# shiv-vignesh/T5-Resnet-VQA

Measured on AMD Instinct MI355X. Metric: question-image pairs/sec, ResNet50+T5-base+SGA train step, 1/2/4/8 MI355X, higher is better.
Workload: dtype bf16; 1 GPU; ResNet50 + t5-base + 3xSGA train step (BASELINE configs[1]; configs[2] at N=8); model=resnet50+t5-base+3xSGA, global_batch=64, per_gpu_batch=64, seq_len=32, image_size=224, answers=170, parallelism=dp1, world_size=1, graph=True, resnet_pipelined=True

## Files before the change

include/vqa_hip.h:

```cpp
#ifndef VQA_HIP_H
#define VQA_HIP_H

#include <hip/hip_runtime.h>

#ifdef __cplusplus
extern "C" {
#endif

#define VQA_ABI_VERSION 20
#define VQA_OK 0
#define VQA_ERR_INVALID 1000

int vqa_abi_version(void);
const char* vqa_last_error(void);

typedef struct vqa_dropout {
  float p;
  unsigned site;
  const unsigned* rng;
} vqa_dropout;

int vqa_rng_advance(unsigned* rng, hipStream_t stream);
int vqa_dropout_mask(const vqa_dropout* d, float* out, long long n, hipStream_t stream);

typedef struct vqa_conv_geom {
  int n, h, w, c;
  int oh, ow;
  int kh, kw, stride, pad;
} vqa_conv_geom;

typedef struct vqa_gemm_desc {
  const void* a; long long lda; int a_trans;
  const void* b; long long ldb; int b_trans;
  int m, n, k;
  float* c32; long long ldc32;
  void* c16; long long ldc16;
  const float* bias;
  const float* res32; const void* res16; long long ldres;
  const void* mask16; long long ldmask;
  float alpha, beta; int relu;
  int a_conv; vqa_conv_geom ga;
  int b_conv; vqa_conv_geom gb;
  int batch; long long stride_a, stride_b, stride_c32, stride_c16, stride_res;
  int config;
  vqa_dropout drop;
  int splitk;
  void* workspace;
  long long workspace_bytes;
  long long stride_bias;
  int drop_site_stride;
  int fp8;
  const float* scale_a;
  const float* scale_b;
  long long stride_scale_a, stride_scale_b;
  int norm;
  const float* norm_w;
  const float* norm_b;
  float norm_eps;
  float* norm_y32;
  void* norm_y16;
  float* norm_mean;
  float* norm_rstd;
  long long stride_norm_w, stride_norm_y, stride_norm_stat;
  vqa_dropout norm_drop;
} vqa_gemm_desc;

#define VQA_GEMM_CONFIGS 28
#define VQA_GEMM_PATCH_FIRST 17
#define VQA_GEMM_PATCH_LAST 20
#define VQA_GEMM_PATCH_WIDE 25
int vqa_gemm(const vqa_gemm_desc* d, hipStream_t stream);
int vqa_quant_rows_fp8(const void* x, int x_bf16, long long ldx, int rows, int cols, void* q, long long ldq,
                       float* scale, hipStream_t stream);
int vqa_gemm_select(const vqa_gemm_desc* d);
long long vqa_gemm_workspace_bytes(const vqa_gemm_desc* d);
int vqa_gemm_pair(const vqa_gemm_desc* dx, const vqa_gemm_desc* dw, hipStream_t stream);

typedef struct vqa_attn_desc {
  const void* q; long long ldq;
  const void* k; long long ldk;
  const void* v; long long ldv;
  void* o; long long ldo;
  float* p;
  const float* bias;
  const long long* key_mask;
  int batch, heads, lq, lk, dh;
  float scale;
  const void* dout; long long lddo;
  void* dq; long long lddq;
  void* dk; long long lddk;
  void* dv; long long lddv;
  float* dbias;
  vqa_dropout drop;
  int groups;
  long long gstride_qkv, gstride_o, gstride_p, gstride_dout;
  int gdrop_site_stride;
} vqa_attn_desc;

int vqa_attn_fwd(const vqa_attn_desc* d, hipStream_t stream);
int vqa_attn_bwd(const vqa_attn_desc* d, hipStream_t stream);
#define VQA_ATTN_MFMA 0
#define VQA_ATTN_LONG 1
#define VQA_ATTN_VALU 2
int vqa_attn_path(const vqa_attn_desc* d, int backward);
int vqa_attn_probs(const vqa_attn_desc* d, hipStream_t stream);

int vqa_rmsnorm_fwd(const float* x, const float* w, float* y32, void* y16, float* rstd, int rows, int d, float eps,
                    const vqa_dropout* drop, hipStream_t stream);
int vqa_rmsnorm_bwd(const float* dy, const float* x, const float* rstd, const float* w, const float* dres,
                    float* dx32, void* dx16, float* dw, float dw_beta, float* ws, int rows, int d,
                    const vqa_dropout* drop_dy, const vqa_dropout* drop_dx32, const vqa_dropout* drop_dx16,
                    hipStream_t stream);
int vqa_layernorm_fwd(const float* x, const float* gamma, const float* beta, float* y32, void* y16, float* mean,
                      float* rstd, int rows, int d, float eps, hipStream_t stream);
int vqa_layernorm_bwd(const float* dy, const float* x, const float* mean, const float* rstd, const float* gamma,
                      const float* dres, float* dx32, void* dx16, float* dgamma, float* dbeta, float* ws, int rows,
                      int d, const vqa_dropout* drop_dx16, float* dsum, hipStream_t stream);
int vqa_norm_bwd_workspace_floats(int rows, int d);
int vqa_colsum_partials(const float* ws, int parts, long long stride, int cols, float* out, float beta,
                        hipStream_t stream);
typedef struct vqa_colsum_job {
  const float* ws; float* out; long long stride; int parts; int cols; float beta; int first_block;
} vqa_colsum_job;
int vqa_norm_bwd_parts(int rows);
int vqa_colsum_parts(int rows);
int vqa_colsum_batched(const vqa_colsum_job* jobs, int njobs, int nblocks, hipStream_t stream);

int vqa_image_to_nhwc8(const float* img, void* out, int n, int h, int w, hipStream_t stream);
int vqa_image_to_s2d16(const float* img, void* out, int n, int h, int w, hipStream_t stream);
int vqa_maxpool3x3s2_nhwc(const void* x, void* y, int n, int h, int w, int c, int oh, int ow, hipStream_t stream);
int vqa_subsample_nhwc(const void* x, int n, int h, int w, int c, int stride, void* y, long long ldy,
                       hipStream_t stream);
int vqa_stem_s2d_conv(const void* z, const void* w, const float* bias, void* y, int n, int hz, int oh,
                      hipStream_t stream);
int vqa_stem_pool_s2d(const void* z, const void* w, const float* bias, void* y, int n, int hz, int oh,
                      hipStream_t stream);
int vqa_stem_pool_img(const float* img, const void* w, const float* bias, void* y, int n, int h, hipStream_t stream);
int vqa_colsum(const void* x, int x_bf16, int rows, int cols, long long ld, float* out, float beta, float* ws,
               hipStream_t stream);
int vqa_colsum_workspace_floats(int rows, int cols);
int vqa_embedding_fwd(const long long* ids, const float* table, float* out, int tokens, int d, int vocab,
                      const vqa_dropout* drop, hipStream_t stream);
typedef struct {
  long long offset;
  int h, w;
} vqa_image_desc;
int vqa_resize_linear_u8(const void* src, const vqa_image_desc* desc, int batch, int oh, int ow, float* out,
                         hipStream_t stream);
int vqa_embedding_bwd(const long long* ids, const float* dh, float* dtable, int tokens, int d, int vocab, int* ws,
                      hipStream_t stream);
int vqa_embedding_zero_rows(long long* ids_prev, const long long* ids_cur, int tokens, float* dtable, int d,
                            int vocab, hipStream_t stream);
int vqa_t5_relbias_fwd(const float* table, const int* bucket, float* out, int heads, int lq, int lk,
                       hipStream_t stream);
int vqa_t5_relbias_bwd(const float* dbias, const int* bucket, float* dtable, int heads, int lq, int lk,
                       int nbuckets, hipStream_t stream);
int vqa_batch_sum(const float* x, int batch, long long n, float* out, float beta, hipStream_t stream);
int vqa_cast_f32_bf16(const float* x, void* y, long long n, hipStream_t stream);
int vqa_zero(void* p, long long bytes, hipStream_t stream);
int vqa_copy(void* dst, const void* src, long long bytes, hipStream_t stream);
int vqa_tap_shift(const void* in, void* out, int n, int h, int w, int c, int kh, int kw, int pad,
                  hipStream_t stream);

int vqa_vit_patchify(const float* img, void* out, int n, int h, int w, int patch, hipStream_t stream);
int vqa_gather_rows(const void* src, long long lds, const long long* idx, long long stride, long long offset,
                    void* dst, long long ldd, int rows, int cols, int esz, hipStream_t stream);
int vqa_scatter_rows(const void* src, long long lds, const long long* idx, long long stride, long long offset,
                     void* dst, long long ldd, int rows, int cols, int esz, hipStream_t stream);
int vqa_last_index(const long long* mask, int batch, int len, long long* out, hipStream_t stream);
int vqa_xattn1_fwd(const void* v, long long ldv, void* out, long long ldo, int batch, int len, int heads, int dh,
                   const vqa_dropout* drop, hipStream_t stream);
int vqa_xattn1_bwd(const void* dctx, long long ldd, float* dv32, void* dv16, long long lddv, int batch, int len,
                   int heads, int dh, const vqa_dropout* drop, hipStream_t stream);

int vqa_head_fwd(const float* x, const float* wp, const float* bp, const float* wc, const float* bc,
                 const long long* targets, float* att, float* pooled, float* logp, float* nll, float* loss,
                 int batch, int seq, int d, int answers, hipStream_t stream);
int vqa_head_bwd(const float* x, const float* att, const float* pooled, const float* logp, const long long* targets,
                 const float* wp, const float* wc, float* dx32, void* dx16, float* dwp, float* dbp, float* dwc,
                 float* dbc, float* ws, int batch, int seq, int d, int answers, const float* nll, float* loss,
                 const float* row_total, float row_scale, hipStream_t stream);
int vqa_head_workspace_floats(int batch, int seq, int d, int answers);
int vqa_count_targets(const long long* targets, int batch, float* out, hipStream_t stream);

typedef struct vqa_eval_desc {
  const float* logp;
  const long long* targets;
  const float* nll;
  const float* loss;
  const float* similarity;
  int batch, answers, k;
  int* topk_idx;
  float* topk_logp;
  void* acc;
  int* pred_log; int* tgt_log;
  long long capacity;
} vqa_eval_desc;

int vqa_eval_rows(const vqa_eval_desc* d, hipStream_t stream);

#define VQA_MAX_GROUPS 8
#define VQA_ST_STEP 0
#define VQA_ST_GRAD_NORM 1
#define VQA_ST_CLIP_COEF 2
#define VQA_ST_LR_SCALE 3
#define VQA_ST_BC1 4
#define VQA_ST_BC2_SQRT 5
#define VQA_ST_PENDING 8

typedef struct vqa_adamw_desc {
  float* param; const float* grad;
  float* exp_avg; float* exp_avg_sq; float* max_exp_avg_sq;
  void* param16;
  long long n;
  int ngroups;
  long long group_end[VQA_MAX_GROUPS];
  float group_lr[VQA_MAX_GROUPS];
  float beta1, beta2, eps, weight_decay, grad_scale;
  const float* state;
} vqa_adamw_desc;

int vqa_grad_sqnorm(const float* g, long long n, double* ws, int parts, hipStream_t stream);
int vqa_optim_finalize(const double* ws, int parts, float grad_scale, float max_norm, int warmup, int total,
                       float beta1, float beta2, float* state, hipStream_t stream);
int vqa_adamw_amsgrad(const vqa_adamw_desc* d, hipStream_t stream);
int vqa_embed_mark(const long long* ids, int n, int rows, int* mark, const float* state, hipStream_t stream);
int vqa_adamw_rows(const vqa_adamw_desc* d, const int* mark, int rows, int cols, int touched, int warmup, int total,
                   hipStream_t stream);

#ifdef __cplusplus
}
#endif
#endif
```

t5-resnet-vqa_amd/csrc/elementwise.hip:

```cpp
#include "common.h"

namespace {

__global__ __launch_bounds__(256) void image_to_nhwc8_kernel(const float* __restrict__ img, bf16_t* __restrict__ out,
                                                             int n, int hw) {
  const long i = (long)blockIdx.x * 256 + threadIdx.x;
  if (i >= (long)n * hw) return;
  const long b = i / hw, p = i - b * hw;
  const float* src = img + b * 3 * hw + p;
  uint4 u;
  u.x = (uint32_t)f2bf(src[0]) | ((uint32_t)f2bf(src[hw]) << 16);
  u.y = (uint32_t)f2bf(src[2 * hw]);
  u.z = 0; u.w = 0;
  reinterpret_cast<uint4*>(out)[i] = u;
}

__global__ __launch_bounds__(256) void image_to_s2d16_kernel(const float* __restrict__ img, bf16_t* __restrict__ out,
                                                             int n, int h, int w, int hz, int wz) {
  const long i = (long)blockIdx.x * 256 + threadIdx.x;
  if (i >= (long)n * hz * wz) return;
  const int v = (int)(i % wz);
  const long t = i / wz;
  const int u = (int)(t % hz), b = (int)(t / hz);
  const float* src = img + (long)b * 3 * h * w;
  float z[16];
#pragma unroll
  for (int p = 0; p < 2; ++p)
#pragma unroll
    for (int q = 0; q < 2; ++q) {
      const int y = 2 * u + p - 1, x = 2 * v + q - 1;
      const bool ok = y >= 0 && y < h && x >= 0 && x < w;
      const long o = ok ? (long)y * w + x : 0;
#pragma unroll
      for (int c = 0; c < 3; ++c) z[(2 * p + q) * 3 + c] = ok ? src[(long)c * h * w + o] : 0.f;
    }
#pragma unroll
  for (int c = 12; c < 16; ++c) z[c] = 0.f;
  uint4 lo, hi;
  lo.x = (uint32_t)f2bf(z[0]) | ((uint32_t)f2bf(z[1]) << 16);
  lo.y = (uint32_t)f2bf(z[2]) | ((uint32_t)f2bf(z[3]) << 16);
  lo.z = (uint32_t)f2bf(z[4]) | ((uint32_t)f2bf(z[5]) << 16);
  lo.w = (uint32_t)f2bf(z[6]) | ((uint32_t)f2bf(z[7]) << 16);
  hi.x = (uint32_t)f2bf(z[8]) | ((uint32_t)f2bf(z[9]) << 16);
  hi.y = (uint32_t)f2bf(z[10]) | ((uint32_t)f2bf(z[11]) << 16);
  hi.z = 0; hi.w = 0;
  reinterpret_cast<uint4*>(out)[2 * i] = lo;
  reinterpret_cast<uint4*>(out)[2 * i + 1] = hi;
}

__global__ __launch_bounds__(256) void maxpool3s2_kernel(const bf16_t* __restrict__ x, bf16_t* __restrict__ y, int n,
                                                         int h, int w, int c, int oh, int ow) {
  const int c8 = c / 8;
  const long i = (long)blockIdx.x * 256 + threadIdx.x;
  if (i >= (long)n * oh * ow * c8) return;
  const int cc = (int)(i % c8);
  long t = i / c8;
  const int ox = (int)(t % ow); t /= ow;
  const int oy = (int)(t % oh);
  const int b = (int)(t / oh);
  float m[8];
#pragma unroll
  for (int j = 0; j < 8; ++j) m[j] = -INFINITY;
  for (int dy = 0; dy < 3; ++dy) {
    const int iy = oy * 2 - 1 + dy;
    if (iy < 0 || iy >= h) continue;
    for (int dx = 0; dx < 3; ++dx) {
      const int ix = ox * 2 - 1 + dx;
      if (ix < 0 || ix >= w) continue;
      uint4 u = reinterpret_cast<const uint4*>(x + (((long)b * h + iy) * w + ix) * c)[cc];
      const uint32_t wds[4] = {u.x, u.y, u.z, u.w};
#pragma unroll
      for (int j = 0; j < 4; ++j) {
        m[2 * j] = fmaxf(m[2 * j], bf2f((bf16_t)(wds[j] & 0xffff)));
        m[2 * j + 1] = fmaxf(m[2 * j + 1], bf2f((bf16_t)(wds[j] >> 16)));
      }
    }
  }
  uint4 o;
  o.x = (uint32_t)f2bf(m[0]) | ((uint32_t)f2bf(m[1]) << 16);
  o.y = (uint32_t)f2bf(m[2]) | ((uint32_t)f2bf(m[3]) << 16);
  o.z = (uint32_t)f2bf(m[4]) | ((uint32_t)f2bf(m[5]) << 16);
  o.w = (uint32_t)f2bf(m[6]) | ((uint32_t)f2bf(m[7]) << 16);
  reinterpret_cast<uint4*>(y)[i] = o;
}

constexpr int COLSUM_ROWS = 64;
template <bool BF16>
__global__ __launch_bounds__(256) void colsum_part_kernel(const void* __restrict__ xv, int rows, int cols, long ld,
                                                          float* __restrict__ ws) {
  const int tx = threadIdx.x & 63, ty = threadIdx.x >> 6;
  const int c = blockIdx.x * 256 + tx * 4;
  const int r0 = blockIdx.y * COLSUM_ROWS;
  float s[4] = {0.f, 0.f, 0.f, 0.f};
  constexpr int RPT = COLSUM_ROWS / 4;
  const int cl = min(c, cols - 4);
  float4 v[RPT];
#pragma unroll
  for (int q = 0; q < RPT; ++q) {
    const int r = min(r0 + ty + 4 * q, rows - 1);
    if constexpr (BF16) {
      const uint2 u = *reinterpret_cast<const uint2*>((const bf16_t*)xv + (long)r * ld + cl);
      v[q] = make_float4(bf2f(u.x & 0xffff), bf2f(u.x >> 16), bf2f(u.y & 0xffff), bf2f(u.y >> 16));
    } else {
      v[q] = *reinterpret_cast<const float4*>((const float*)xv + (long)r * ld + cl);
    }
  }
#pragma unroll
  for (int q = 0; q < RPT; ++q) {
    const float m = (c < cols && r0 + ty + 4 * q < rows) ? 1.f : 0.f;
    s[0] += v[q].x * m; s[1] += v[q].y * m; s[2] += v[q].z * m; s[3] += v[q].w * m;
  }
  __shared__ float red[4][256];
#pragma unroll
  for (int j = 0; j < 4; ++j) red[ty][tx * 4 + j] = s[j];
  __syncthreads();
  const int cc = blockIdx.x * 256 + threadIdx.x;
  if (cc < cols)
    ws[(long)blockIdx.y * cols + cc] = red[0][threadIdx.x] + red[1][threadIdx.x] + red[2][threadIdx.x] +
                                       red[3][threadIdx.x];
}

__global__ __launch_bounds__(256) void embedding_fwd_kernel(const long long* __restrict__ ids,
                                                            const float* __restrict__ table, float* __restrict__ out,
                                                            int tokens, int d4, int vocab, vqa_dropout drop) {
  const long i = (long)blockIdx.x * 256 + threadIdx.x;
  if (i >= (long)tokens * d4) return;
  const int t = (int)(i / d4), j = (int)(i - (long)t * d4);
  long long id = ids[t];
  id = id < 0 ? 0 : (id >= vocab ? vocab - 1 : id);
  float4 v = reinterpret_cast<const float4*>(table + id * (long)d4 * 4)[j];
  const DropK dk = drop_init(drop);
  if (dk.on) {
    const uint32_t e = (uint32_t)i * 4u;
    v.x *= drop_mul(dk, e); v.y *= drop_mul(dk, e + 1); v.z *= drop_mul(dk, e + 2); v.w *= drop_mul(dk, e + 3);
  }
  reinterpret_cast<float4*>(out)[i] = v;
}

__global__ void rng_advance_kernel(unsigned* rng) { rng[1] += 1u; }

__global__ __launch_bounds__(256) void dropout_mask_kernel(vqa_dropout d, float* __restrict__ out, long n) {
  const long i = (long)blockIdx.x * 256 + threadIdx.x;
  if (i >= n) return;
  const DropK dk = drop_init(d);
  out[i] = drop_mul(dk, (uint32_t)i);
}

__global__ __launch_bounds__(256) void embedding_zero_rows_kernel(long long* __restrict__ prev,
                                                                  const long long* __restrict__ cur,
                                                                  float* __restrict__ dtable, int d, int vocab) {
  const int t = blockIdx.x;
  long long id = prev[t];
  id = id < 0 ? 0 : (id >= vocab ? vocab - 1 : id);
  float4* row = reinterpret_cast<float4*>(dtable + id * (long long)d);
  for (int c = threadIdx.x; c < d / 4; c += 256) row[c] = make_float4(0.f, 0.f, 0.f, 0.f);
  __syncthreads();
  if (cur && threadIdx.x == 0) prev[t] = cur[t];
}

__device__ __forceinline__ unsigned long long shfl_xor64(unsigned long long v, int m) {
  const int lo = __shfl_xor((int)(unsigned)(v & 0xffffffffu), m, 64);
  const int hi = __shfl_xor((int)(unsigned)(v >> 32), m, 64);
  return ((unsigned long long)(unsigned)hi << 32) | (unsigned)lo;
}
template <int E>
__global__ __launch_bounds__(1024) void embedding_sort_kernel(const long long* __restrict__ ids, int tokens, int vocab,
                                                              int* __restrict__ ws) {
  __shared__ unsigned long long key[E * 1024];
  constexpr int n = E * 1024;
  const int t = threadIdx.x;
  unsigned long long v[E];
#pragma unroll
  for (int q = 0; q < E; ++q) {
    const int i = q * 1024 + t;
    long long id = ids[min(i, tokens - 1)];
    id = id < 0 ? 0 : (id >= vocab ? vocab - 1 : id);
    v[q] = i < tokens ? (((unsigned long long)id << 16) | (unsigned long long)i) : ~0ull;
  }
  for (int k = 2; k <= n; k <<= 1) {
    for (int j = k >> 1; j > 0; j >>= 1) {
      if (j >= 1024) {
        const int qj = j >> 10;
#pragma unroll
        for (int q = 0; q < E; ++q) {
          if (q & qj) continue;
          const int i = q * 1024 + t;
          const bool up = (i & k) == 0;
          const unsigned long long a = v[q], c = v[q | qj];
          v[q] = up ? (a < c ? a : c) : (a < c ? c : a);
          v[q | qj] = up ? (a < c ? c : a) : (a < c ? a : c);
        }
      } else if (j >= 64) {
#pragma unroll
        for (int q = 0; q < E; ++q) key[q * 1024 + t] = v[q];
        __syncthreads();
#pragma unroll
        for (int q = 0; q < E; ++q) {
          const int i = q * 1024 + t;
          const unsigned long long c = key[i ^ j];
          const bool keep_min = ((i & j) == 0) == ((i & k) == 0);
          v[q] = keep_min ? (v[q] < c ? v[q] : c) : (v[q] < c ? c : v[q]);
        }
        __syncthreads();
      } else {
#pragma unroll
        for (int q = 0; q < E; ++q) {
          const int i = q * 1024 + t;
          const unsigned long long c = shfl_xor64(v[q], j);
          const bool keep_min = ((i & j) == 0) == ((i & k) == 0);
          v[q] = keep_min ? (v[q] < c ? v[q] : c) : (v[q] < c ? c : v[q]);
        }
      }
    }
  }
#pragma unroll
  for (int q = 0; q < E; ++q) key[q * 1024 + t] = v[q];
  __syncthreads();
#pragma unroll
  for (int q = 0; q < E; ++q) {
    const int i = q * 1024 + t;
    if (i >= tokens) continue;
    const unsigned long long kt = v[q];
    const unsigned id = (unsigned)(kt >> 16);
    ws[i] = (int)(kt & 0xffff);
    ws[tokens + i] = (int)id;
    if (i == 0 || (unsigned)(key[i - 1] >> 16) != id) {
      int lo = i + 1, hi = tokens;
      while (lo < hi) {
        const int mid = (lo + hi) >> 1;
        if ((unsigned)(key[mid] >> 16) == id) lo = mid + 1; else hi = mid;
      }
      ws[2 * tokens + i] = lo;
    }
  }
}

constexpr int EMB_RL = 16, EMB_CL = 32;
__global__ __launch_bounds__(EMB_RL * EMB_CL) void embedding_bwd_kernel(const float* __restrict__ dh,
                                                                        float* __restrict__ dtable,
                                                                        const int* __restrict__ ws, int tokens,
                                                                        int d) {
  const int s0 = blockIdx.x;
  const int* pos = ws;
  const int* sid = ws + tokens;
  const int id = sid[s0];
  if (s0 > 0 && sid[s0 - 1] == id) return;
  const int s1 = ws[2 * tokens + s0];
  const int tx = threadIdx.x % EMB_CL, ty = threadIdx.x / EMB_CL;
  const int c4 = blockIdx.y * EMB_CL + tx;
  const bool act = c4 * 4 < d;
  float4 acc = make_float4(0.f, 0.f, 0.f, 0.f);
  if (act) {
    constexpr int U = 8;
    for (int u0 = s0 + ty; u0 < s1; u0 += EMB_RL * U) {
      int pp[U];
#pragma unroll
      for (int q = 0; q < U; ++q) pp[q] = pos[min(u0 + q * EMB_RL, s1 - 1)];
      float4 v[U];
#pragma unroll
      for (int q = 0; q < U; ++q) v[q] = reinterpret_cast<const float4*>(dh + (long)pp[q] * d)[c4];
#pragma unroll
      for (int q = 0; q < U; ++q) {
        if (u0 + q * EMB_RL < s1) { acc.x += v[q].x; acc.y += v[q].y; acc.z += v[q].z; acc.w += v[q].w; }
      }
    }
  }
  __shared__ float4 red[EMB_RL][EMB_CL];
  red[ty][tx] = acc;
  __syncthreads();
  if (ty == 0 && act) {
    float4 t = red[0][tx];
#pragma unroll
    for (int r = 1; r < EMB_RL; ++r) {
      const float4 v = red[r][tx];
      t.x += v.x; t.y += v.y; t.z += v.z; t.w += v.w;
    }
    float4* dst = reinterpret_cast<float4*>(dtable + (long)id * d) + c4;
    const float4 o = *dst;
    t.x += o.x; t.y += o.y; t.z += o.z; t.w += o.w;
    *dst = t;
  }
}

__global__ __launch_bounds__(256) void relbias_fwd_kernel(const float* __restrict__ table,
                                                          const int* __restrict__ bucket, float* __restrict__ out,
                                                          int heads, int lqk) {
  const int i = blockIdx.x * 256 + threadIdx.x;
  if (i >= heads * lqk) return;
  const int h = i / lqk, p = i - h * lqk;
  const int bk = bucket[p];
  out[i] = bk < 0 ? -3.4028234663852886e38f : table[bk * heads + h];
}

__global__ __launch_bounds__(256) void relbias_bwd_kernel(const float* __restrict__ dbias,
                                                          const int* __restrict__ bucket, float* __restrict__ dtable,
                                                          int heads, int lqk) {
  __shared__ float red[4];
  const int bk = blockIdx.x / heads, h = blockIdx.x - bk * heads;
  float s = 0.f;
  for (int p = threadIdx.x; p < lqk; p += 256)
    if (bucket[p] == bk) s += dbias[(long)h * lqk + p];
  s = block_sum<256>(s, red);
  if (threadIdx.x == 0) dtable[bk * heads + h] = s;
}

__global__ __launch_bounds__(256) void cast_f32_bf16_kernel(const float* __restrict__ x, bf16_t* __restrict__ y,
                                                            long n) {
  const long i = ((long)blockIdx.x * 256 + threadIdx.x) * 4;
  if (i + 3 < n) {
    float4 v = *reinterpret_cast<const float4*>(x + i);
    uint2 u;
    u.x = (uint32_t)f2bf(v.x) | ((uint32_t)f2bf(v.y) << 16);
    u.y = (uint32_t)f2bf(v.z) | ((uint32_t)f2bf(v.w) << 16);
    *reinterpret_cast<uint2*>(y + i) = u;
  } else {
    for (long j = i; j < n; ++j) y[j] = f2bf(x[j]);
  }
}

__global__ __launch_bounds__(256) void zero_kernel(uint4* __restrict__ p, long n16) {
  for (long i = (long)blockIdx.x * 256 + threadIdx.x; i < n16; i += (long)gridDim.x * 256)
    p[i] = make_uint4(0, 0, 0, 0);
}

__global__ __launch_bounds__(256) void copy_kernel(uint4* __restrict__ dst, const uint4* __restrict__ src, long n16) {
  for (long i = (long)blockIdx.x * 256 + threadIdx.x; i < n16; i += (long)gridDim.x * 256) dst[i] = src[i];
}

}

extern "C" int vqa_image_to_s2d16(const float* img, void* out, int n, int h, int w, hipStream_t s) {
  VQA_REQUIRE(img && out && n > 0 && h > 1 && w > 1 && h % 2 == 0 && w % 2 == 0,
              "vqa_image_to_s2d16: bad arguments (H and W must be even)");
  const int hz = h / 2 + 1, wz = w / 2 + 1;
  const long total = (long)n * hz * wz;
  hipLaunchKernelGGL(image_to_s2d16_kernel, dim3(vqa::cdiv(total, 256)), dim3(256), 0, s, img, (bf16_t*)out, n, h, w,
                     hz, wz);
  return vqa::check_launch("vqa_image_to_s2d16");
}

extern "C" int vqa_image_to_nhwc8(const float* img, void* out, int n, int h, int w, hipStream_t s) {
  VQA_REQUIRE(img && out && n > 0 && h > 0 && w > 0, "vqa_image_to_nhwc8: bad arguments");
  const long total = (long)n * h * w;
  hipLaunchKernelGGL(image_to_nhwc8_kernel, dim3(vqa::cdiv(total, 256)), dim3(256), 0, s, img, (bf16_t*)out, n, h * w);
  return vqa::check_launch("vqa_image_to_nhwc8");
}

extern "C" int vqa_maxpool3x3s2_nhwc(const void* x, void* y, int n, int h, int w, int c, int oh, int ow,
                                     hipStream_t s) {
  VQA_REQUIRE(x && y && c % 8 == 0, "vqa_maxpool3x3s2_nhwc: bad arguments");
  const long total = (long)n * oh * ow * (c / 8);
  hipLaunchKernelGGL(maxpool3s2_kernel, dim3(vqa::cdiv(total, 256)), dim3(256), 0, s, (const bf16_t*)x, (bf16_t*)y, n,
                     h, w, c, oh, ow);
  return vqa::check_launch("vqa_maxpool3x3s2_nhwc");
}

namespace {
__global__ __launch_bounds__(256) void subsample_kernel(const uint4* __restrict__ x, uint4* __restrict__ y, int h,
                                                        int w, int c8, int s, int oh, int ow, long ldy8, long total) {
  const long i = (long)blockIdx.x * 256 + threadIdx.x;
  if (i >= total) return;
  const int cc = (int)(i % c8);
  const long r = i / c8;
  const int ox = (int)(r % ow);
  const long t = r / ow;
  const int oy = (int)(t % oh);
  const long b = t / oh;
  y[r * ldy8 + cc] = x[((b * h + (long)oy * s) * w + (long)ox * s) * c8 + cc];
}
}

extern "C" int vqa_subsample_nhwc(const void* x, int n, int h, int w, int c, int stride, void* y, long long ldy,
                                  hipStream_t s) {
  VQA_REQUIRE(x && y && n > 0 && h > 0 && w > 0 && stride >= 1 && c % 8 == 0 && ldy % 8 == 0 && ldy >= c &&
                  ((uintptr_t)y & 15) == 0 && ((uintptr_t)x & 15) == 0,
              "vqa_subsample_nhwc: bad arguments (c, ldy multiples of 8, 16-B aligned buffers)");
  const int oh = (h - 1) / stride + 1, ow = (w - 1) / stride + 1;
  const long total = (long)n * oh * ow * (c / 8);
  hipLaunchKernelGGL(subsample_kernel, dim3(vqa::cdiv(total, 256)), dim3(256), 0, s, (const uint4*)x, (uint4*)y, h, w,
                     c / 8, stride, oh, ow, (long)(ldy / 8), total);
  return vqa::check_launch("vqa_subsample_nhwc");
}

extern "C" int vqa_colsum_workspace_floats(int rows, int cols) { return vqa::cdiv(rows, COLSUM_ROWS) * cols; }
extern "C" int vqa_colsum_parts(int rows) { return vqa::cdiv(rows, COLSUM_ROWS); }

extern "C" int vqa_colsum(const void* x, int x_bf16, int rows, int cols, long long ld, float* out, float beta,
                          float* ws, hipStream_t s) {
  VQA_REQUIRE(x && ws && cols % 4 == 0 && ld % 4 == 0, "vqa_colsum: bad arguments");
  const int parts = vqa::cdiv(rows, COLSUM_ROWS);
  dim3 grid(vqa::cdiv(cols, 256), parts);
  if (x_bf16)
    hipLaunchKernelGGL(colsum_part_kernel<true>, grid, dim3(256), 0, s, x, rows, cols, (long)ld, ws);
  else
    hipLaunchKernelGGL(colsum_part_kernel<false>, grid, dim3(256), 0, s, x, rows, cols, (long)ld, ws);
  if (int rc = vqa::check_launch("vqa_colsum")) return rc;
  if (!out) return VQA_OK;
  return vqa_colsum_partials(ws, parts, cols, cols, out, beta, s);
}

extern "C" int vqa_embedding_fwd(const long long* ids, const float* table, float* out, int tokens, int d, int vocab,
                                 const vqa_dropout* drop, hipStream_t s) {
  VQA_REQUIRE(ids && table && out && d % 4 == 0, "vqa_embedding_fwd: bad arguments");
  VQA_REQUIRE(!drop || (drop->p >= 0.f && drop->p < 1.f), "vqa_embedding_fwd: dropout p must be in [0, 1)");
  const vqa_dropout dr = drop ? *drop : vqa_dropout{0.f, 0u, nullptr};
  const long total = (long)tokens * (d / 4);
  hipLaunchKernelGGL(embedding_fwd_kernel, dim3(vqa::cdiv(total, 256)), dim3(256), 0, s, ids, table, out, tokens,
                     d / 4, vocab, dr);
  return vqa::check_launch("vqa_embedding_fwd");
}

extern "C" int vqa_rng_advance(unsigned* rng, hipStream_t s) {
  VQA_REQUIRE(rng, "vqa_rng_advance: null state");
  hipLaunchKernelGGL(rng_advance_kernel, dim3(1), dim3(1), 0, s, rng);
  return vqa::check_launch("vqa_rng_advance");
}

extern "C" int vqa_dropout_mask(const vqa_dropout* d, float* out, long long n, hipStream_t s) {
  VQA_REQUIRE(d && out && n > 0 && n <= (1ll << 32), "vqa_dropout_mask: bad arguments");
  VQA_REQUIRE(d->p >= 0.f && d->p < 1.f, "vqa_dropout_mask: p must be in [0, 1)");
  hipLaunchKernelGGL(dropout_mask_kernel, dim3(vqa::cdiv(n, 256)), dim3(256), 0, s, *d, out, (long)n);
  return vqa::check_launch("vqa_dropout_mask");
}

extern "C" int vqa_embedding_zero_rows(long long* ids_prev, const long long* ids_cur, int tokens, float* dtable,
                                       int d, int vocab, hipStream_t s) {
  VQA_REQUIRE(ids_prev && dtable && tokens > 0 && d % 4 == 0 && vocab > 0, "vqa_embedding_zero_rows: bad arguments");
  hipLaunchKernelGGL(embedding_zero_rows_kernel, dim3(tokens), dim3(256), 0, s, ids_prev, ids_cur, dtable, d, vocab);
  return vqa::check_launch("vqa_embedding_zero_rows");
}

extern "C" int vqa_embedding_bwd(const long long* ids, const float* dh, float* dtable, int tokens, int d, int vocab,
                                 int* ws, hipStream_t s) {
  VQA_REQUIRE(ids && dh && dtable && ws && tokens > 0 && d % 4 == 0, "vqa_embedding_bwd: bad arguments");
  constexpr int SLICE = 16384;
  for (int t0 = 0; t0 < tokens; t0 += SLICE) {
    const int n = tokens - t0 < SLICE ? tokens - t0 : SLICE;
    const long long* sid = ids + t0;
    if (n <= 1024)
      hipLaunchKernelGGL(embedding_sort_kernel<1>, dim3(1), dim3(1024), 0, s, sid, n, vocab, ws);
    else if (n <= 2048)
      hipLaunchKernelGGL(embedding_sort_kernel<2>, dim3(1), dim3(1024), 0, s, sid, n, vocab, ws);
    else if (n <= 4096)
      hipLaunchKernelGGL(embedding_sort_kernel<4>, dim3(1), dim3(1024), 0, s, sid, n, vocab, ws);
    else if (n <= 8192)
      hipLaunchKernelGGL(embedding_sort_kernel<8>, dim3(1), dim3(1024), 0, s, sid, n, vocab, ws);
    else
      hipLaunchKernelGGL(embedding_sort_kernel<16>, dim3(1), dim3(1024), 0, s, sid, n, vocab, ws);
    if (int rc = vqa::check_launch("vqa_embedding_bwd/sort")) return rc;
    hipLaunchKernelGGL(embedding_bwd_kernel, dim3(n, vqa::cdiv(d, 4 * EMB_CL)), dim3(EMB_RL * EMB_CL), 0, s,
                       dh + (long long)t0 * d, dtable, ws, n, d);
    if (int rc = vqa::check_launch("vqa_embedding_bwd")) return rc;
  }
  return VQA_OK;
}

extern "C" int vqa_batch_sum(const float* x, int batch, long long n, float* out, float beta, hipStream_t s) {
  VQA_REQUIRE(x && out && batch > 0 && n > 0 && n < (1ll << 31), "vqa_batch_sum: bad arguments");
  return vqa_colsum_partials(x, batch, n, (int)n, out, beta, s);
}

extern "C" int vqa_t5_relbias_fwd(const float* table, const int* bucket, float* out, int heads, int lq, int lk,
                                  hipStream_t s) {
  VQA_REQUIRE(table && bucket && out, "vqa_t5_relbias_fwd: bad arguments");
  hipLaunchKernelGGL(relbias_fwd_kernel, dim3(vqa::cdiv(heads * lq * lk, 256)), dim3(256), 0, s, table, bucket, out,
                     heads, lq * lk);
  return vqa::check_launch("vqa_t5_relbias_fwd");
}

extern "C" int vqa_t5_relbias_bwd(const float* dbias, const int* bucket, float* dtable, int heads, int lq, int lk,
                                  int nbuckets, hipStream_t s) {
  VQA_REQUIRE(dbias && bucket && dtable, "vqa_t5_relbias_bwd: bad arguments");
  hipLaunchKernelGGL(relbias_bwd_kernel, dim3(heads * nbuckets), dim3(256), 0, s, dbias, bucket, dtable, heads,
                     lq * lk);
  return vqa::check_launch("vqa_t5_relbias_bwd");
}

extern "C" int vqa_cast_f32_bf16(const float* x, void* y, long long n, hipStream_t s) {
  VQA_REQUIRE(x && y && n >= 0, "vqa_cast_f32_bf16: bad arguments");
  if (n == 0) return VQA_OK;
  hipLaunchKernelGGL(cast_f32_bf16_kernel, dim3(vqa::cdiv(vqa::cdiv(n, 4), 256)), dim3(256), 0, s, x, (bf16_t*)y,
                     (long)n);
  return vqa::check_launch("vqa_cast_f32_bf16");
}

extern "C" int vqa_zero(void* p, long long bytes, hipStream_t s) {
  VQA_REQUIRE(p && bytes >= 0 && ((uintptr_t)p & 15) == 0 && bytes % 16 == 0,
              "vqa_zero: pointer and size must be 16-byte aligned");
  if (bytes == 0) return VQA_OK;
  const long n16 = (long)(bytes / 16);
  const int grid = (int)((n16 + 255) / 256 < 8192 ? (n16 + 255) / 256 : 8192);
  hipLaunchKernelGGL(zero_kernel, dim3(grid), dim3(256), 0, s, (uint4*)p, n16);
  return vqa::check_launch("vqa_zero");
}

extern "C" int vqa_copy(void* dst, const void* src, long long bytes, hipStream_t s) {
  VQA_REQUIRE(dst && src && bytes >= 0 && ((uintptr_t)dst & 15) == 0 && ((uintptr_t)src & 15) == 0 && bytes % 16 == 0,
              "vqa_copy: pointers and size must be 16-byte aligned");
  if (bytes == 0) return VQA_OK;
  const long n16 = (long)(bytes / 16);
  const int grid = (int)((n16 + 255) / 256 < 8192 ? (n16 + 255) / 256 : 8192);
  hipLaunchKernelGGL(copy_kernel, dim3(grid), dim3(256), 0, s, (uint4*)dst, (const uint4*)src, n16);
  return vqa::check_launch("vqa_copy");
}

__global__ __launch_bounds__(256) void tap_shift_kernel(const uint4* __restrict__ in, uint4* __restrict__ out, int h,
                                                        int w, int c8, int kw, int pad, int per_tap) {
  const int i = blockIdx.x * 256 + threadIdx.x;
  if (i >= per_tap) return;
  const int t = blockIdx.y, ky = t / kw, kx = t - ky * kw;
  const int pos = i / c8, ch = i - pos * c8;
  const int hw = h * w, b = pos / hw, yx = pos - b * hw;
  const int y = yx / w, x = yx - y * w;
  const int sy = y - ky + pad, sx = x - kx + pad;
  uint4 v = make_uint4(0u, 0u, 0u, 0u);
  if (sy >= 0 && sy < h && sx >= 0 && sx < w) v = in[(b * hw + sy * w + sx) * c8 + ch];
  out[(long)t * per_tap + i] = v;
}

extern "C" int vqa_tap_shift(const void* in, void* out, int n, int h, int w, int c, int kh, int kw, int pad,
                             hipStream_t s) {
  VQA_REQUIRE(in && out && n > 0 && h > 0 && w > 0 && c > 0 && kh > 0 && kw > 0 && pad >= 0 && c % 8 == 0 &&
                  ((uintptr_t)in & 15) == 0 && ((uintptr_t)out & 15) == 0,
              "vqa_tap_shift: bad arguments (c a multiple of 8, 16-byte aligned maps)");
  const long per_tap = (long)n * h * w * (c / 8);
  VQA_REQUIRE(per_tap < (1l << 31) && kh * kw <= 65535, "vqa_tap_shift: map too large");
  hipLaunchKernelGGL(tap_shift_kernel, dim3((unsigned)((per_tap + 255) / 256), (unsigned)(kh * kw)), dim3(256), 0, s,
                     (const uint4*)in, (uint4*)out, h, w, c / 8, kw, pad, (int)per_tap);
  return vqa::check_launch("vqa_tap_shift");
}
```

t5-resnet-vqa_amd/csrc/optim.hip:

```cpp
#include "adamw.h"

namespace {

__global__ __launch_bounds__(256) void sqnorm_kernel(const float* __restrict__ g, long n4, double* __restrict__ ws) {
  const float4* g4 = reinterpret_cast<const float4*>(g);
  const long st = (long)gridDim.x * 256;
  double s = 0.0;
  long i = (long)blockIdx.x * 256 + threadIdx.x;
  for (; i + 3 * st < n4; i += 4 * st) {
    float4 v[4];
#pragma unroll
    for (int u = 0; u < 4; ++u) v[u] = g4[i + u * st];
#pragma unroll
    for (int u = 0; u < 4; ++u)
      s += (double)v[u].x * v[u].x + (double)v[u].y * v[u].y + (double)v[u].z * v[u].z + (double)v[u].w * v[u].w;
  }
  for (; i < n4; i += st) {
    const float4 v = g4[i];
    s += (double)v.x * v.x + (double)v.y * v.y + (double)v.z * v.z + (double)v.w * v.w;
  }
#pragma unroll
  for (int o = 32; o > 0; o >>= 1) s += __shfl_xor(s, o, 64);
  __shared__ double red[4];
  if ((threadIdx.x & 63) == 0) red[threadIdx.x >> 6] = s;
  __syncthreads();
  if (threadIdx.x == 0) ws[blockIdx.x] = red[0] + red[1] + red[2] + red[3];
}

__device__ __forceinline__ void schedule_at(double step, int warmup, int total, float beta1, float beta2,
                                            float& lam_f, float& bc1, float& bc2s) {
  double lam;
  if (step < warmup) lam = step / (double)(warmup > 1 ? warmup : 1);
  else lam = fmax(0.0, (double)(total - step) / (double)((total - warmup) > 1 ? (total - warmup) : 1));
  const double t = step + 1.0;
  lam_f = (float)lam;
  bc1 = (float)(1.0 - pow((double)beta1, t));
  bc2s = (float)sqrt(1.0 - pow((double)beta2, t));
}

__global__ void finalize_kernel(const double* __restrict__ ws, int parts, float grad_scale, float max_norm,
                                int warmup, int total, float beta1, float beta2, float* __restrict__ st) {
  __shared__ double red[256];
  double part = 0.0;
  for (int i = threadIdx.x; i < parts; i += 256) part += ws[i];
  red[threadIdx.x] = part;
  __syncthreads();
  if (threadIdx.x != 0) return;
  double ss = 0.0;
  for (int i = 0; i < 256; ++i) ss += red[i];
  const float norm = (float)(sqrt(ss) * (double)grad_scale);
  float coef = 1.f;
  if (max_norm > 0.f) coef = fminf(1.f, max_norm / (norm + 1e-6f));
  const double step = (double)st[VQA_ST_STEP];
  float lam, bc1, bc2s;
  schedule_at(step, warmup, total, beta1, beta2, lam, bc1, bc2s);
  st[VQA_ST_GRAD_NORM] = norm;
  st[VQA_ST_CLIP_COEF] = coef;
  st[VQA_ST_LR_SCALE] = lam;
  st[VQA_ST_BC1] = bc1;
  st[VQA_ST_BC2_SQRT] = bc2s;
  st[VQA_ST_STEP] = (float)(step + 1.0);
  st[VQA_ST_PENDING] = 1.f;
}

__global__ __launch_bounds__(256) void embed_mark_kernel(const long long* __restrict__ ids, int n, int rows,
                                                         int* __restrict__ mark, const float* __restrict__ st) {
  const int i = blockIdx.x * 256 + threadIdx.x;
  if (i >= n) return;
  const long long id = ids[i];
  if (id >= 0 && id < rows) mark[id] = (int)st[VQA_ST_STEP];
}

template <int MODE>
__global__ __launch_bounds__(192) void adamw_rows_kernel(AdamArgs A, const int* __restrict__ mark, int rows, int d4,
                                                         int warmup, int total) {
  const int step = (int)A.st[VQA_ST_STEP];
  float coef, lam, bc1, bc2s;
  if (MODE == 0) {
    coef = 1.f;
    schedule_at((double)A.st[VQA_ST_STEP], warmup, total, A.b1, A.b2, lam, bc1, bc2s);
  } else {
    if (A.st[VQA_ST_PENDING] == 0.f) return;
    coef = A.st[VQA_ST_CLIP_COEF];
    lam = A.st[VQA_ST_LR_SCALE];
    bc1 = A.st[VQA_ST_BC1];
    bc2s = A.st[VQA_ST_BC2_SQRT];
  }
  for (int row = blockIdx.x; row < rows; row += gridDim.x) {
  const bool touched = mark[row] == (MODE == 0 ? step : step - 1);
  if (MODE == 0 ? touched : !touched) continue;
  for (int c = threadIdx.x; c < d4; c += 192) {
    const long i = (long)row * d4 + c;
    f32x4_t p = __builtin_nontemporal_load(reinterpret_cast<const f32x4_t*>(A.p) + i);
    f32x4_t g4 = {0.f, 0.f, 0.f, 0.f};
    if (MODE == 1) g4 = __builtin_nontemporal_load(reinterpret_cast<const f32x4_t*>(A.g) + i);
    f32x4_t m = __builtin_nontemporal_load(reinterpret_cast<const f32x4_t*>(A.m) + i);
    f32x4_t v = __builtin_nontemporal_load(reinterpret_cast<const f32x4_t*>(A.v) + i);
    f32x4_t vm = __builtin_nontemporal_load(reinterpret_cast<const f32x4_t*>(A.vm) + i);
    adamw_update4_with(A, i, p, g4, m, v, vm, coef, lam, bc1, bc2s);
    __builtin_nontemporal_store(p, reinterpret_cast<f32x4_t*>(A.p) + i);
    __builtin_nontemporal_store(m, reinterpret_cast<f32x4_t*>(A.m) + i);
    __builtin_nontemporal_store(v, reinterpret_cast<f32x4_t*>(A.v) + i);
    __builtin_nontemporal_store(vm, reinterpret_cast<f32x4_t*>(A.vm) + i);
    if (A.p16) {
      uint2 u;
      u.x = (uint32_t)f2bf(p[0]) | ((uint32_t)f2bf(p[1]) << 16);
      u.y = (uint32_t)f2bf(p[2]) | ((uint32_t)f2bf(p[3]) << 16);
      reinterpret_cast<uint2*>(A.p16)[i] = u;
    }
  }
  }
}

__global__ __launch_bounds__(256) void adamw_kernel(AdamArgs A) {
  const long i = (long)blockIdx.x * 256 + threadIdx.x;
  if (i >= A.n4 || A.st[VQA_ST_PENDING] == 0.f) return;
  f32x4_t p = __builtin_nontemporal_load(reinterpret_cast<const f32x4_t*>(A.p) + i);
  const f32x4_t g4 = __builtin_nontemporal_load(reinterpret_cast<const f32x4_t*>(A.g) + i);
  f32x4_t m = __builtin_nontemporal_load(reinterpret_cast<const f32x4_t*>(A.m) + i);
  f32x4_t v = __builtin_nontemporal_load(reinterpret_cast<const f32x4_t*>(A.v) + i);
  f32x4_t vm = __builtin_nontemporal_load(reinterpret_cast<const f32x4_t*>(A.vm) + i);
  adamw_update4(A, i, p, g4, m, v, vm);
  __builtin_nontemporal_store(p, reinterpret_cast<f32x4_t*>(A.p) + i);
  __builtin_nontemporal_store(m, reinterpret_cast<f32x4_t*>(A.m) + i);
  __builtin_nontemporal_store(v, reinterpret_cast<f32x4_t*>(A.v) + i);
  __builtin_nontemporal_store(vm, reinterpret_cast<f32x4_t*>(A.vm) + i);
  if (A.p16) {
    uint2 u;
    u.x = (uint32_t)f2bf(p[0]) | ((uint32_t)f2bf(p[1]) << 16);
    u.y = (uint32_t)f2bf(p[2]) | ((uint32_t)f2bf(p[3]) << 16);
    reinterpret_cast<uint2*>(A.p16)[i] = u;
  }
}

int grid_for(long n4) {
  long b = (n4 + 255) / 256;
  return (int)(b < 4096 ? b : 4096);
}

}

extern "C" int vqa_grad_sqnorm(const float* g, long long n, double* ws, int parts, hipStream_t s) {
  VQA_REQUIRE(g && ws && n % 4 == 0 && parts > 0, "vqa_grad_sqnorm: bad arguments (n %% 4 == 0)");
  hipLaunchKernelGGL(sqnorm_kernel, dim3(parts), dim3(256), 0, s, g, (long)(n / 4), ws);
  return vqa::check_launch("vqa_grad_sqnorm");
}

extern "C" int vqa_optim_finalize(const double* ws, int parts, float grad_scale, float max_norm, int warmup, int total,
                                  float beta1, float beta2, float* state, hipStream_t s) {
  VQA_REQUIRE(ws && state && parts > 0, "vqa_optim_finalize: bad arguments");
  hipLaunchKernelGGL(finalize_kernel, dim3(1), dim3(256), 0, s, ws, parts, grad_scale, max_norm, warmup, total, beta1,
                     beta2, state);
  return vqa::check_launch("vqa_optim_finalize");
}

extern "C" int vqa_adamw_amsgrad(const vqa_adamw_desc* d, hipStream_t s) {
  AdamArgs A;
  if (int rc = adam_args(d, A)) return rc;
  hipLaunchKernelGGL(adamw_kernel, dim3(vqa::cdiv(A.n4, 256)), dim3(256), 0, s, A);
  return vqa::check_launch("vqa_adamw_amsgrad");
}

extern "C" int vqa_embed_mark(const long long* ids, int n, int rows, int* mark, const float* state, hipStream_t s) {
  VQA_REQUIRE(ids && mark && state && n > 0 && rows > 0, "vqa_embed_mark: bad arguments");
  hipLaunchKernelGGL(embed_mark_kernel, dim3(vqa::cdiv(n, 256)), dim3(256), 0, s, ids, n, rows, mark, state);
  return vqa::check_launch("vqa_embed_mark");
}

extern "C" int vqa_adamw_rows(const vqa_adamw_desc* d, const int* mark, int rows, int cols, int touched, int warmup,
                              int total, hipStream_t s) {
  AdamArgs A;
  if (int rc = adam_args(d, A)) return rc;
  VQA_REQUIRE(mark && rows > 0 && cols > 0 && cols % 4 == 0 && (long long)rows * cols == d->n,
              "vqa_adamw_rows: rows x cols must be the descriptor's n (cols %% 4 == 0)");
  const int grid = touched > 1 && touched < rows ? touched : rows;
  if (touched == 1)
    hipLaunchKernelGGL(adamw_rows_kernel<1>, dim3(rows), dim3(192), 0, s, A, mark, rows, cols / 4, warmup, total);
  else
    hipLaunchKernelGGL(adamw_rows_kernel<0>, dim3(grid), dim3(192), 0, s, A, mark, rows, cols / 4, warmup, total);
  return vqa::check_launch("vqa_adamw_rows");
}
```

t5-resnet-vqa_amd/dp.py:

```python
from __future__ import annotations

import os

import numpy as np
import torch

from . import lib as L
from . import ops
from . import synthetic as S
from .engine_base import _after, no_gc_capture


DP_T5_DW_GROUPS = (4, 4, 3, 1)


def dp_t5_dw_groups(layers=12):
    if layers == 12:
        return DP_T5_DW_GROUPS
    g = [layers // 3, layers // 3, layers // 4]
    return tuple(g + [layers - sum(g)])


def plan_buckets(ready_marks, end, min_bytes=24 << 20):
    out, start = [], 0
    for i, (ci, stop) in enumerate(ready_marks):
        stop = min(stop, end)
        last = i == len(ready_marks) - 1
        if stop - start >= min_bytes // 4 or (last and stop > start):
            if last and out and stop - start < min_bytes // 32:
                out[-1] = (ci, out[-1][1], stop)
            else:
                out.append((ci, start, stop))
            start = stop
    return out


def plan_shards(buckets, world, align=64):
    out = []
    for _, a, b in buckets:
        chunk = (b - a) // (world * align) * align
        out.append((a, chunk, b))
    return out


def _wait_only(w):
    return w.wait_only() if hasattr(w, "wait_only") else w.wait()


COMM_ON_STREAM = True


class _OnStream:
    def __init__(self):
        self.ev = torch.cuda.Event()
        self.ev.record(torch.cuda.current_stream())

    def wait(self):
        torch.cuda.current_stream().wait_event(self.ev)
        return True

    wait_only = wait


class _Done:
    def wait(self):
        return True

    wait_only = wait


class _Then:
    def __init__(self, work, then):
        self.work, self.then = work, then

    def wait(self):
        self.work.wait()
        self.then()
        return True

    def wait_only(self):
        return self.work.wait()


class _All:
    def __init__(self, works):
        self.works = works

    def wait(self):
        for w in self.works:
            w.wait()
        return True

    def wait_only(self):
        for w in self.works:
            _wait_only(w)
        return True


def _staged(t, group):
    import torch.distributed as dist
    return t.is_cuda and dist.get_backend(group) == "gloo"


def allreduce_buckets(flat, buckets, group=None):
    import torch.distributed as dist
    if _staged(flat, group):
        for _, a, b in buckets:
            h = flat[a:b].cpu()
            dist.all_reduce(h, group=group)
            flat[a:b].copy_(h)
        return [_Done() for _ in buckets]
    if COMM_ON_STREAM and flat.is_cuda:
        for _, a, b in buckets:
            dist.all_reduce(flat[a:b], group=group, async_op=False)
        return [_OnStream()]
    return [dist.all_reduce(flat[a:b], group=group, async_op=True) for _, a, b in buckets]


def gather_rows(ids, rows, out_ids, out_rows, group=None):
    import torch.distributed as dist
    if dist.get_backend(group) == "gloo":
        w = dist.get_world_size(group)
        if _staged(rows, group):
            hi, hr = torch.empty(out_ids.shape, dtype=out_ids.dtype), torch.empty(out_rows.shape, dtype=out_rows.dtype)
            dist.all_gather(list(hi.chunk(w)), ids.reshape(-1).cpu(), group=group)
            dist.all_gather(list(hr.chunk(w)), rows.cpu(), group=group)
            out_ids.copy_(hi)
            out_rows.copy_(hr)
            return [_Done(), _Done()]
        w1 = dist.all_gather(list(out_ids.chunk(w)), ids.reshape(-1), group=group, async_op=True)
        w2 = dist.all_gather(list(out_rows.chunk(w)), rows, group=group, async_op=True)
        return [w1, w2]
    if COMM_ON_STREAM:
        dist.all_gather_into_tensor(out_ids, ids.reshape(-1), group=group, async_op=False)
        dist.all_gather_into_tensor(out_rows, rows, group=group, async_op=False)
        return [_OnStream()]
    w1 = dist.all_gather_into_tensor(out_ids, ids.reshape(-1), group=group, async_op=True)
    w2 = dist.all_gather_into_tensor(out_rows, rows, group=group, async_op=True)
    return [w1, w2]


def gather_tensor(x, out, group=None):
    import torch.distributed as dist
    w = dist.get_world_size(group)
    if dist.get_backend(group) == "gloo":
        if x.is_cuda:
            h = torch.empty(out.shape, dtype=out.dtype)
            dist.all_gather(list(h.chunk(w)), x.reshape(-1, *out.shape[1:]).cpu(), group=group)
            out.copy_(h)
            return [_Done()]
        dist.all_gather(list(out.chunk(w)), x.reshape(-1, *out.shape[1:]), group=group)
        return [_Done()]
    if COMM_ON_STREAM:
        dist.all_gather_into_tensor(out, x.reshape(-1, *out.shape[1:]), group=group, async_op=False)
        return [_OnStream()]
    return [dist.all_gather_into_tensor(out, x.reshape(-1, *out.shape[1:]), group=group, async_op=True)]


RES_SPLIT = 1.0


def plan_stages(segments, scaler, dw_stream=True):
    stages, ops, fin, pend, pend_b, prev = [], [], [], [], [], 0
    for k, seg in enumerate(segments):
        lo, hi = prev, prev + len(seg)
        prev = hi
        if (lo, hi) == tuple(scaler):
            chain, dw = [], list(seg)
        elif dw_stream:
            chain, dw = [c for c in seg if not c.side], [c for c in seg if c.side]
        else:
            chain, dw = list(seg), []
        if chain:
            if pend:
                ops.append(("fork", pend))
                fin, pend, pend_b = fin + pend_b, [], []
            ops.append(("main", chain))
        if dw:
            pend, pend_b = pend + dw, pend_b + [k]
        else:
            fin = fin + [k]
        if chain and fin:
            stages.append({"ops": ops, "final": fin})
            ops, fin = [], []
    if pend:
        if ops or not stages:
            ops.append(("fork", pend))
            fin = fin + pend_b
        else:
            stages[-1]["ops"].append(("fork", pend))
            stages[-1]["final"] = stages[-1]["final"] + pend_b
    if ops or fin:
        stages.append({"ops": ops, "final": fin})
    rows = max(j for j, st in enumerate(stages) if any(kd == "main" for kd, _ in st["ops"]))
    return stages, rows


class DataParallelStep:
    def __init__(self, engine, group=None, bucket_mb=24, use_graph=True, shard_optimizer=False, res_split=RES_SPLIT):
        import torch.distributed as dist
        self.eng, self.group = engine, group
        self.world = dist.get_world_size(group)
        self.rank = dist.get_rank(group)
        self.shard = bool(shard_optimizer)
        e = engine
        e.set_grad_scale(1.0 / self.world)
        e.use_global_rows(self.world)
        emb = e.lay["t5.embed"]
        self.buckets = plan_buckets(e.ready_marks, emb.offset, bucket_mb << 20)
        calls = e.bwd_calls[:-1]
        assert e.bwd_calls[-1] is e.emb_call
        T, D = e.T, e.D
        dev = e.dev
        self.GIDS = torch.zeros(self.world * T, dtype=torch.int64, device=dev)
        self.GIDS_PREV = torch.zeros(self.world * T, dtype=torch.int64, device=dev)
        assert calls[0] is e.zero_calls[0]
        g = e.g32["t5.embed"]
        calls = [ops.Call("vqa_embedding_zero_rows", self.GIDS_PREV.data_ptr(), self.GIDS.data_ptr(), self.world * T,
                          g.data_ptr(), D, S.T5_VOCAB, keep=(self.GIDS_PREV, self.GIDS, g))] + calls[1:]
        self.segments, prev = [], 0
        for ci, _, _ in self.buckets:
            self.segments.append(calls[prev:ci])
            prev = ci
        self.tail = calls[prev:]
        self.GDH = torch.zeros(self.world * T, D, dtype=torch.float32, device=dev)
        self.WS = torch.empty(3 * min(self.world * T, 16384), dtype=torch.int32, device=dev)
        self.emb_call = ops.Call("vqa_embedding_bwd", self.GIDS.data_ptr(), self.GDH.data_ptr(),
                                 e.g32["t5.embed"].data_ptr(), self.world * T, D, S.T5_VOCAB, self.WS.data_ptr(),
                                 keep=(self.GIDS, self.GDH, self.WS, e.g32["t5.embed"]))
        if self.shard:
            self._plan_sharded_optimizer()
        self._plan_schedule()
        r1 = int(round(len(e.res_calls) * float(res_split))) if e.pipeline else 0
        self._res_a = list(e.res_calls[:r1]) if e.pipeline else []
        if e.pipeline and r1 < len(e.res_calls):
            self.stages[0]["ops"].insert(0, ("res", list(e.res_calls[r1:])))
        self.graphs = None
        self.timing = False
        self._ev = []
        if use_graph:
            self.capture()
        e.g32["t5.embed"].zero_()

    def _plan_sharded_optimizer(self):
        e = self.eng
        self.shards = plan_shards(self.buckets, self.world)
        n, emb = e.lay.total, e.lay["t5.embed"].offset
        r, N = self.rank, self.world
        own = [(a + r * c, a + (r + 1) * c) for a, c, b in self.shards if c > 0]
        rep = [(a + N * c, b) for a, c, b in self.shards if b > a + N * c] + [(emb, n)]
        K = e.SQ_PARTS
        ranges = own + rep
        self.WS_SQN = torch.zeros(len(ranges) * K, dtype=torch.float64, device=e.dev)
        sq = []
        for i, (lo, hi) in enumerate(ranges):
            if i < len(own) or r == 0:
                sq.append(ops.Call("vqa_grad_sqnorm", ops.addr(e.G32, lo), hi - lo, ops.addr(self.WS_SQN, i * K), K,
                                   keep=(e.G32, self.WS_SQN)))
        self.sq_calls = sq
        fin = []
        e._call(fin, "vqa_optim_finalize", self.WS_SQN, len(ranges) * K, float(e.grad_scale), float(e.max_norm),
                int(e.warmup), int(e.total), float(e.betas[0]), float(e.betas[1]), e.opt_state)
        self.finalize_call = fin[0]
        self.adam_calls = [e.adam_range_call(lo, hi) for lo, hi in ranges]
        offs = np.concatenate([[0], np.cumsum([c for _, c, _ in self.shards])]).astype(np.int64)
        self.rs_off = [int(o) for o in offs[:-1]]
        self.RS_OUT = torch.empty(max(int(offs[-1]), 1), dtype=torch.float32, device=e.dev)

    def _sharded_collectives_after(self, bk_index):
        import torch.distributed as dist
        e = self.eng
        a, c, b = self.shards[bk_index]
        N, r = self.world, self.rank
        works = []
        if c > 0:
            full, mine = e.G32[a:a + N * c], e.G32[a + r * c:a + (r + 1) * c]
            if _staged(full, self.group) or dist.get_backend(self.group) == "gloo":
                h = full.cpu()
                dist.all_reduce(h, group=self.group)
                mine.copy_(h[r * c:(r + 1) * c])
                works.append(_Done())
            else:
                out = self.RS_OUT[self.rs_off[bk_index]:self.rs_off[bk_index] + c]
                if COMM_ON_STREAM:
                    dist.reduce_scatter_tensor(out, full, group=self.group, async_op=False)
                    mine.copy_(out)
                    works.append(_OnStream())
                else:
                    works.append(_Then(dist.reduce_scatter_tensor(out, full, group=self.group, async_op=True),
                                       lambda out=out, mine=mine: mine.copy_(out)))
        if b > a + N * c:
            works += allreduce_buckets(e.G32, [(None, a + N * c, b)], self.group)
        return [_All(works)]

    def _sharded_optimizer(self):
        import torch.distributed as dist
        e = self.eng
        s = L.stream_handle()
        self.WS_SQN.zero_()
        for c in self.sq_calls:
            c(s)
        if _staged(self.WS_SQN, self.group):
            h = self.WS_SQN.cpu()
            dist.all_reduce(h, group=self.group)
            self.WS_SQN.copy_(h)
        else:
            dist.all_reduce(self.WS_SQN, group=self.group)
        self.finalize_call(s)
        for c in self.adam_calls:
            c(s)
        e.clear_pending(s)
        N, r = self.world, self.rank
        for a, c, b in self.shards:
            if c == 0:
                continue
            for t in (e.P32, e.P16):
                full, mine = t[a:a + N * c], t[a + r * c:a + (r + 1) * c]
                if _staged(full, self.group):
                    parts = [torch.empty(c, dtype=t.dtype) for _ in range(N)]
                    dist.all_gather(parts, mine.cpu(), group=self.group)
                    full.copy_(torch.cat(parts))
                else:
                    dist.all_gather_into_tensor(full, mine.clone(), group=self.group)
        if e.fp8 and not e.defer_opt:
            self._run(e.quant_all)

    def sync_optimizer_state(self):
        import torch.distributed as dist
        if not self.shard:
            return
        e = self.eng
        N, r = self.world, self.rank
        for a, c, b in self.shards:
            if c == 0:
                continue
            for t in (e.M, e.V, e.VMAX):
                full, mine = t[a:a + N * c], t[a + r * c:a + (r + 1) * c]
                if _staged(full, self.group):
                    parts = [torch.empty(c, dtype=t.dtype) for _ in range(N)]
                    dist.all_gather(parts, mine.cpu(), group=self.group)
                    full.copy_(torch.cat(parts))
                else:
                    dist.all_gather_into_tensor(full, mine.clone(), group=self.group)

    def _run(self, calls):
        s = L.stream_handle()
        for c in calls:
            c(s)

    def _plan_schedule(self):
        e = self.eng
        self.stages, self.rows_stage = plan_stages(self.segments, e._bsplit, e.dw_stream)
        assert sorted(k for st in self.stages for k in st["final"]) == list(range(len(self.buckets)))
        self.emb_pre = []
        self._sq0_stage = None
        opt = list(e.opt_calls)
        if not self.shard:
            if e.embed_split:
                self.emb_pre = [ops.Call("vqa_embed_mark", self.GIDS.data_ptr(), self.world * e.T, S.T5_VOCAB,
                                         e.EMB_MARK.data_ptr(), e.opt_state.data_ptr(),
                                         keep=(self.GIDS, e.EMB_MARK, e.opt_state)), e.emb_pre[1]]
                self.stages[0]["ops"].insert(0, ("emb", self.emb_pre))
                opt = opt[:2] + list(e.tail_calls)
            a = e._sq_split[1] if e._sq_split is not None else None
            if a is not None:
                done = 0
                for j, st in enumerate(self.stages):
                    if st["final"]:
                        done = max(done, max(self.buckets[k][2] for k in st["final"]))
                    if done >= a and st["final"]:
                        self._sq0_stage = j
                        break
            if self._sq0_stage is not None:
                assert opt[0].name == "vqa_grad_sqnorm"
                self._sq0_call = opt[0]
                opt = opt[1:]
        self.finish_calls = self.tail + [self.emb_call] + ([] if self.shard else opt)
        comm = os.environ.get("VQA_DP_COMM", "wside")
        self._comm = {"own": None, "side": e._side, "wside": e._wside}[comm] or torch.cuda.Stream(e.dev)
        self._tstream = torch.cuda.Stream(e.dev)

    def stage_plan(self):
        return [{"ops": [({"main": "chain", "fork": "dw_fork", "res": "resnet_fork", "emb": "embedding_rows_fork"}[kd],
                          len(c)) for kd, c in st["ops"]],
                 "final_buckets": st["final"]} for st in self.stages]

    def _run_stage(self, st):
        e = self.eng
        main = torch.cuda.current_stream(e.dev)
        forked = set()
        for kind, calls in st["ops"]:
            if kind == "main":
                self._run(calls)
            else:
                side = {"fork": e._wside, "res": e._rstream, "emb": e._side}[kind]
                _after(side, main)
                with torch.cuda.stream(side):
                    self._run(calls)
                forked.add(side)
        for side in forked:
            _after(main, side)

    def _backward_exchange(self):
        e = self.eng
        g = self.graphs
        main = torch.cuda.current_stream(e.dev)
        exchange = lambda i, bk: self._sharded_collectives_after(i)
        comm = self._comm
        tm = {"stage": {}, "done": {}} if self.timing else None
        works = {}

        def mark_done(key, ws):
            if tm is not None:
                with torch.cuda.stream(self._tstream):
                    for w in ws:
                        _wait_only(w)
                    tm["done"][key] = torch.cuda.Event(enable_timing=True)
                    tm["done"][key].record(self._tstream)
        for j, st in enumerate(self.stages):
            if g is not None:
                g[f"stage{j}"].replay()
            else:
                self._run_stage(st)
            if not (st["final"] or j == self.rows_stage):
                continue
            if tm is not None:
                tm["stage"][j] = torch.cuda.Event(enable_timing=True)
                tm["stage"][j].record(main)
            _after(comm, main)
            with torch.cuda.stream(comm):
                if j == self.rows_stage:
                    works["rows"] = gather_tensor(e.dH32, self.GDH, self.group)
                    mark_done("rows", works["rows"])
                if self.shard:
                    for k in st["final"]:
                        works[k] = exchange(k, self.buckets[k])
                        mark_done(k, works[k])
                else:
                    ks = st["final"]
                    assert ks == list(range(ks[0], ks[-1] + 1))
                    ws = allreduce_buckets(e.G32, [(None, self.buckets[ks[0]][1], self.buckets[ks[-1]][2])], self.group)
                    for k in ks:
                        works[k] = ws if k == ks[-1] else []
                        mark_done(k, ws)
                    if j == self._sq0_stage and (COMM_ON_STREAM or _staged(e.G32, self.group)):
                        self._sq0_call(L.stream_handle(comm))
        if tm is not None:
            tm["wait"] = (torch.cuda.Event(enable_timing=True), torch.cuda.Event(enable_timing=True))
            tm["wait"][0].record(main)
        for key, ws in works.items():
            for w in ws:
                w.wait()
        _after(main, comm)
        if tm is not None:
            tm["wait"][1].record(main)
        self._play("finish", self.finish_calls)
        return tm

    def _play(self, name, calls):
        if self.graphs is not None:
            self.graphs[name].replay()
        else:
            self._run(calls)

    def capture(self):
        e = self.eng
        e.flush_optimizer()
        e.ROWTOT.fill_(float(e.B * self.world))
        s = torch.cuda.Stream(e.dev)
        s.wait_stream(torch.cuda.current_stream(e.dev))
        saved_rng = e.RNG.clone()
        with torch.cuda.stream(s):
            e._run(e.fwd_calls)
            e.backward()
        torch.cuda.current_stream(e.dev).wait_stream(s)
        torch.cuda.synchronize(e.dev)
        e.RNG.copy_(saved_rng)
        with no_gc_capture():
            self.graphs = self._capture_all(s)

    def _capture_all(self, s):
        e = self.eng
        gs = {}

        def cap(name, fn):
            g = torch.cuda.CUDAGraph()
            with torch.cuda.graph(g, stream=s):
                fn()
            gs[name] = g
        cap("fwd", self._fwd)
        for j, st in enumerate(self.stages):
            cap(f"stage{j}", lambda st=st: self._run_stage(st))
        cap("finish", lambda: self._run(self.finish_calls))
        return gs

    def _fwd(self):
        e = self.eng
        main = torch.cuda.current_stream(e.dev)
        if self._res_a:
            _after(e._rstream, main)
            with torch.cuda.stream(e._rstream):
                self._run(self._res_a)
        e.run_forward_streams()
        if self._res_a:
            _after(main, e._rstream)

    def _exchange_step_start(self):
        e = self.eng
        main = torch.cuda.current_stream(e.dev)
        e.count_call(L.stream_handle(main))
        _after(self._comm, main)
        with torch.cuda.stream(self._comm):
            ws = allreduce_buckets(e.ROWTOT, [(None, 0, 1)], self.group)
            return ws + gather_tensor(e.IDS, self.GIDS, self.group)

    def step(self):
        e = self.eng
        rows = self._exchange_step_start()
        if e.pipeline:
            e.copy_f4(L.stream_handle(torch.cuda.current_stream(e.dev)))
        if self.graphs is not None:
            self.graphs["fwd"].replay()
        else:
            self._fwd()
        for w in rows:
            w.wait()
        _after(torch.cuda.current_stream(e.dev), self._comm)
        tev = self._backward_exchange()
        if self.shard:
            self._sharded_optimizer()
        if self.timing:
            self._ev.append(tev)

    def timing_report(self):
        torch.cuda.synchronize()
        if not self._ev:
            return None
        e = self.eng
        stage_of = {k: j for j, st in enumerate(self.stages) for k in st["final"]}
        stage_of["rows"] = self.rows_stage

        def mean(f):
            return round(float(np.mean([f(t) for t in self._ev])), 1)
        lag = {k: mean(lambda t, k=k: t["stage"][stage_of[k]].elapsed_time(t["done"][k]) * 1e3) for k in stage_of}
        return {"world_size": self.world, "steps": len(self._ev), "stages": self.stage_plan(),
                "embedding_rows_gather": {"bytes": int(self.world * e.T * (e.D * 4 + 8)),
                                          "done_us_after_stage": lag["rows"]},
                "buckets": [{"start": int(a), "stop": int(b), "bytes": int(4 * (b - a)), "stage": stage_of[k],
                             "done_us_after_stage": lag[k]} for k, (_, a, b) in enumerate(self.buckets)],
                "exposed_wait_us_total": mean(lambda t: t["wait"][0].elapsed_time(t["wait"][1]) * 1e3)}
```

t5-resnet-vqa_amd/engine.py:

```python
from __future__ import annotations

import ctypes
import os
import math

import numpy as np
import torch

from . import lib as L
from . import ops
from . import synthetic as S
from .engine_base import (BF16, F32, I64, IGNORE_INDEX, SITE_EMBED, SITE_FINAL, EngineBase, _after,
                          _check_attn_path, _h2d, _Seq, batch_rows, load_rows, no_gc_capture, t5_site)
from .layout import ParamLayout, fold_bn, t5_bucket_map


def sga_site(block, kind):
    return 128 + 8 * block + kind


def stem_s2d_weight(wf):
    co, kh, kw, ci = wf.shape
    w8 = np.zeros((co, 8, 8, ci), np.float32)
    w8[:, :kh, :kw] = wf
    w = w8.reshape(co, 4, 2, 4, 2, ci).transpose(0, 1, 3, 2, 4, 5).reshape(co, 4, 4, 4 * ci)
    return np.concatenate([w, np.zeros((co, 4, 4, 16 - 4 * ci), np.float32)], 3)


class VQAEngine(EngineBase):
    def __init__(self, state_dict, vision="resnet50", batch=64, seq_len=32, image_size=224, device="cuda:0",
                 warmup=10, total=100, num_blocks=3, answer_spaces=170, grad_scale=1.0, max_norm=1.0,
                 betas=(0.9, 0.999), eps=1e-8, weight_decay=0.1, dropout=0.1, seed=0, pipeline=False,
                 t5_dw_group=None, defer_optimizer=True, dw_stream=None, sga_dw_batch=True, pair_bwd=True,
                 language_model="t5-base", fp8=False, sga_attn_group=True, fuse_norm=None):
        super().__init__(device, dropout, seed, warmup, total, max_norm, betas, eps, weight_decay, grad_scale)
        self.fuse_norm = (os.environ.get("VQA_FUSE_NORM", "0") == "1") if fuse_norm is None else bool(fuse_norm)
        self.fuse_norm_kept = []
        self.pipeline = bool(pipeline)
        self.res_order, self.res_head = "first", 4
        self._res_feed = None
        self._keep_graph = False
        self._rstream_handle = None
        self._rstream_plain = None
        self.EMB_MARK = None
        self.vision, self.B, self.L, self.H = vision, batch, seq_len, image_size
        assert image_size % 2 == 0, "the space-to-depth stem needs an even image size"
        self.NB, self.A = num_blocks, answer_spaces
        self.dims = dm = S.lm_dims(language_model)
        self.D, self.nl, self.h5, self.dkv, self.dff = dm.d_model, dm.t5_layers, dm.t5_heads, dm.t5_dkv, dm.t5_dff
        self.sga_heads, self.sga_dh = dm.sga_heads, dm.sga_dhead
        assert self.h5 * self.dkv == self.D and self.sga_heads * self.sga_dh == self.D
        self.fp8 = bool(fp8)
        if not 1 <= answer_spaces <= 1024:
            raise ValueError(f"answer_spaces={answer_spaces}: the fused answer head supports 1..1024 answers")
        if not 1 <= seq_len <= 64:
            raise ValueError(f"seq_len={seq_len}: the attention / pooler kernels support 1..64 question tokens")
        self.pair_bwd = bool(pair_bwd)
        if t5_dw_group is None:
            t5_dw_group = (3 * self.nl // 4, self.nl - 3 * self.nl // 4)
        if isinstance(t5_dw_group, (list, tuple)):
            self.t5_dw_groups = [int(x) for x in t5_dw_group]
            self.t5_dw_group = self.nl
            assert sum(self.t5_dw_groups) == self.nl and min(self.t5_dw_groups) >= 1
        else:
            self.t5_dw_groups = None
            self.t5_dw_group = int(t5_dw_group)
        self.sga_dw_batch = bool(sga_dw_batch)
        self.sga_attn_group = bool(sga_attn_group)
        self.defer_opt = bool(defer_optimizer)
        self.dw_stream = True if dw_stream is None else bool(dw_stream)
        self.T = batch * seq_len
        self.rows = batch
        self.lay = ParamLayout(vision, answer_spaces, num_blocks, dm)
        sd = {k: np.asarray(v) for k, v in state_dict.items()}
        self._frozen = {k: v for k, v in sd.items() if k not in set(self.lay.trainable_keys)}
        with torch.cuda.device(self.dev):
            self._alloc_params(sd)
            self._plan_resnet(sd)
            self._alloc_activations()
            self.fwd_calls, self.bwd_calls, self.opt_calls, self.zero_calls = [], [], [], []
            self._plan_forward()
            self._plan_backward()
            self._plan_optimizer()
            self._run(self.quant_all)
        self.eval_call = None
        self.allreduce = None
        self._side = torch.cuda.Stream(self.dev)
        self._wside = torch.cuda.Stream(self.dev)
        self._rstream = torch.cuda.Stream(self.dev)
        self.res_external = False
        self.allow_empty_rows = False
        self._img_rows_next = None
        self.count_call = None

    @classmethod
    def from_state_dict(cls, sd, **kw):
        return cls(sd, **kw)

    def _alloc_params(self, sd):
        self._alloc_arenas(sd)
        self.bucket = torch.from_numpy(t5_bucket_map(self.L, self.L)).reshape(-1).to(self.dev)

    def _alloc_shadow_arenas(self):
        if self.fp8:
            self.W8 = torch.empty(self.lay.total, dtype=torch.uint8, device=self.dev)
            self.WSC = torch.ones(self.lay.total, dtype=F32, device=self.dev)
            self._xq = {}

    def _plan_resnet(self, sd):
        B, H = self.B, self.H
        vm = "vision_model."
        self.res_calls = []
        self._res_keep = []
        convs = []

        def conv_w(cname, bname, s2d=False):
            w = sd[vm + cname + ".weight"].astype(np.float32)
            wf, bf = fold_bn(w, sd[vm + bname + ".weight"], sd[vm + bname + ".bias"],
                             sd[vm + bname + ".running_mean"], sd[vm + bname + ".running_var"])
            wf = wf.transpose(0, 2, 3, 1)
            if s2d:
                wf = stem_s2d_weight(wf)
            w16 = torch.from_numpy(np.ascontiguousarray(wf)).to(self.dev).to(BF16)
            b32 = torch.from_numpy(bf).to(self.dev)
            self._res_keep += [w16, b32]
            return w16, b32

        layers = S.RESNET_LAYERS[self.vision]
        bottleneck = self.vision == "resnet50"
        h1 = (H + 2 * 3 - 7) // 2 + 1
        h2 = (h1 + 2 - 3) // 2 + 1
        plan = []
        maxel = B * h1 * h1 * 64
        hh, cin = h2, 64
        for li, (planes, nblk) in enumerate(zip((64, 128, 256, 512), layers)):
            for bi in range(nblk):
                stride = (1 if li == 0 else 2) if bi == 0 else 1
                out = planes * 4 if bottleneck else planes
                ho = (hh + 2 - 3) // stride + 1
                maxel = max(maxel, B * hh * hh * planes, B * ho * ho * out)
                if bottleneck and bi == 0:
                    maxel = max(maxel, B * ho * ho * (planes + cin))
                plan.append((li, bi, stride, hh, ho, cin, planes, out))
                hh, cin = ho, out
        self.fh, self.fc = hh, cin
        self.V_TOK = B * hh * hh
        self.IMG = self._t((B, 3, H, H))
        hz = H // 2 + 1
        bufs = [self._t(maxel, BF16) for _ in range(5)]
        self.res_bufs = bufs
        self.F4 = self._t((B, hh, hh, cin), BF16)
        self.F4N = self._t((B, hh, hh, cin), BF16) if self.pipeline else self.F4
        self.copy_f4 = ops.Call("vqa_copy", self.F4.data_ptr(), self.F4N.data_ptr(), self.F4.numel() * 2,
                                keep=(self.F4, self.F4N))

        w16, b32 = conv_w("conv1", "bn1", s2d=True)
        g = ops.conv_geom(B, hz, hz, 16, h1, h1, 4, 4, 1, 1)
        fused_img = H % 32 == 0
        self.IMG8 = None if fused_img else self._t((B, hz, hz, 16), BF16)
        if fused_img:
            self.res_calls.append(ops.Call("vqa_stem_pool_img", self.IMG.data_ptr(), w16.data_ptr(), b32.data_ptr(),
                                           bufs[1].data_ptr(), B, H, keep=(self.IMG, w16, b32, bufs[1])))
        else:
            self.res_calls.append(ops.Call("vqa_image_to_s2d16", self.IMG.data_ptr(), self.IMG8.data_ptr(), B, H, H,
                                           keep=(self.IMG, self.IMG8)))
            self._gemm(self.res_calls, self.IMG8, w16, B * h1 * h1, 64, 256, lda=256, ldb=256, ga=g,
                       c16=bufs[0], ldc16=64, bias=b32, relu=True)
            self.res_calls.append(ops.Call("vqa_maxpool3x3s2_nhwc", bufs[0].data_ptr(), bufs[1].data_ptr(), B, h1,
                                           h1, 64, h2, h2, keep=(bufs[0], bufs[1])))
        x = bufs[1]
        free = [bufs[0], bufs[2], bufs[3], bufs[4]]
        nblocks_total = len(plan)
        for idx, (li, bi, stride, hi, ho, ci, planes, out) in enumerate(plan):
            p = f"layer{li + 1}.{bi}."
            t1, t2, ds, y = free[0], free[1], free[2], free[3]
            if idx == nblocks_total - 1:
                y = self.F4N
            if bottleneck and (vm + p + "downsample.0.weight") in sd:
                kc = planes + ci
                w, b = conv_w(p + "conv1", p + "bn1")
                self._conv(x, (B, hi, hi, ci), w, b, 1, 0, t1, relu=True)
                w, b = conv_w(p + "conv2", p + "bn2")
                self._conv(t1, (B, hi, hi, planes), w, b, stride, 1, ds, relu=True, ldc16=kc)
                self.res_calls.append(ops.Call("vqa_subsample_nhwc", x.data_ptr(), B, hi, hi, ci, stride,
                                               ops.addr(ds, planes), kc, keep=(x, ds)))
                w3, b3 = conv_w(p + "conv3", p + "bn3")
                wd, bd = conv_w(p + "downsample.0", p + "downsample.1")
                wcat = torch.cat([w3.reshape(out, planes), wd.reshape(out, ci)], dim=1).contiguous()
                bcat = b3 + bd
                self._res_keep += [wcat, bcat]
                assert B * ho * ho * kc <= ds.numel(), "fused downsample: the [conv2 | x] rows exceed the buffer"
                self._gemm(self.res_calls, ds, wcat, B * ho * ho, out, kc, lda=kc, ldb=kc, c16=y, ldc16=out,
                           bias=bcat, relu=True)
                if y is not self.F4N:
                    free = [x, t1, t2, ds]
                    x = y
                continue
            if bottleneck:
                w, b = conv_w(p + "conv1", p + "bn1")
                self._conv(x, (B, hi, hi, ci), w, b, 1, 0, t1, relu=True)
                w, b = conv_w(p + "conv2", p + "bn2")
                self._conv(t1, (B, hi, hi, planes), w, b, stride, 1, t2, relu=True)
                last_in, last_c, last_h = t2, planes, ho
                w3, b3 = conv_w(p + "conv3", p + "bn3")
            else:
                w, b = conv_w(p + "conv1", p + "bn1")
                self._conv(x, (B, hi, hi, ci), w, b, stride, 1, t1, relu=True)
                last_in, last_c, last_h = t1, planes, ho
                w3, b3 = conv_w(p + "conv2", p + "bn2")
            res = x
            if (vm + p + "downsample.0.weight") in sd:
                w, b = conv_w(p + "downsample.0", p + "downsample.1")
                self._conv(x, (B, hi, hi, ci), w, b, stride, 0, ds, relu=False)
                res = ds
            k3 = 1 if bottleneck else 3
            self._conv(last_in, (B, last_h, last_h, last_c), w3, b3, 1, 1 if k3 == 3 else 0, y, relu=True,
                       res16=res)
            if y is not self.F4N:
                free = [x, t1, t2, ds]
                x = y

    def _conv(self, x, shape, w16, b32, stride, pad, out, relu, res16=None, ldc16=None):
        n, h, w, c = shape
        cout, kh, kw, _ = w16.shape
        oh = (h + 2 * pad - kh) // stride + 1
        g = ops.conv_geom(n, h, w, c, oh, oh, kh, kw, stride, pad)
        if kh == 1 and kw == 1 and stride == 1 and pad == 0:
            g = None
        patch = kh == 3 and kw == 3 and stride == 1 and pad == 1 and c % 64 == 0 and 14 <= w <= 64
        if patch:
            w16 = w16.reshape(cout, 9, c // 64, 64).permute(0, 2, 1, 3).contiguous().reshape(cout, kh, kw, c)
            self._res_keep.append(w16)
        self._gemm(self.res_calls, x, w16, n * oh * oh, cout, kh * kw * c, lda=kh * kw * c, ldb=kh * kw * c, ga=g,
                   c16=out, ldc16=ldc16 or cout, bias=b32, relu=relu, res16=res16, ldres=cout, a_patch=patch)

    def _alloc_activations(self):
        D = self.D
        B, Lq, T, NB, V = self.B, self.L, self.T, self.NB, self.V_TOK
        t = self._t
        self.IDS = t((B, Lq), I64, zero=True)
        self.IDS_PREV = t((B, Lq), I64, zero=True)
        self.MASK = t((B, Lq), I64, zero=True)
        self.TGT = t((B,), I64, zero=True)
        self.VIS32, self.VIS16 = t((V, D)), t((V, D), BF16)
        nl = self.nl
        self.PB = t((self.h5, Lq, Lq))
        self.HS = [t((T, D)) for _ in range(nl + 1)]
        self.N0S, self.OS, self.N1S = t((nl, T, D), BF16), t((nl, T, D), BF16), t((nl, T, D), BF16)
        self.FFS = t((nl, T, self.dff), BF16)
        self.N0 = [self.N0S[nl - 1 - i] for i in range(nl)]
        self.QKV = [t((T, 3 * D), BF16) for _ in range(nl)]
        self.PT = [t((B, self.h5, Lq, Lq)) for _ in range(nl)]
        self.O = [self.OS[nl - 1 - i] for i in range(nl)]
        self.HM = [t((T, D)) for _ in range(nl)]
        self.N1 = [self.N1S[nl - 1 - i] for i in range(nl)]
        self.FF = [self.FFS[nl - 1 - i] for i in range(nl)]
        self.R0 = [t(T) for _ in range(nl)]
        self.R1 = [t(T) for _ in range(nl)]
        self.RF = t(T)
        self.TXT32, self.TXT16 = t((T, D)), t((T, D), BF16)
        self.QKV1A = t((T, NB * 3 * D), BF16)
        self.O1A, self.S1A = t((NB, T, D), BF16), t((NB, T, D))
        self.P1A = t((NB, B, self.sga_heads, Lq, Lq))
        self.X1hS, self.O2S, self.X2hS, self.FFhS = (t((NB, T, D), BF16) for _ in range(4))
        self.Q2S = t((NB, T, D), BF16)
        if self.fuse_norm:
            self.X1S, self.MU1S, self.RS1S = t((NB, T, D)), t((NB, T)), t((NB, T))
            self.NORM_WS = [torch.zeros(65536 // 4, dtype=torch.int32, device=self.dev) for _ in range(2)]
        self.sga = []
        for n in range(NB):
            ly = V if n == 0 else T
            lk = self.fh * self.fh if n == 0 else Lq
            self.sga.append(dict(
                ly=ly, lk=lk,
                P1=self.P1A[n], O1=self.O1A[n], S1=self.S1A[n],
                X1=self.X1S[NB - 1 - n] if self.fuse_norm else t((T, D)), X1h=self.X1hS[NB - 1 - n],
                MU1=self.MU1S[n] if self.fuse_norm else t(T), RS1=self.RS1S[n] if self.fuse_norm else t(T),
                Q2=self.Q2S[NB - 1 - n], KV2=t((ly, 2 * D), BF16), P2=t((B, self.sga_heads, Lq, lk)),
                O2=self.O2S[NB - 1 - n], S2=t((T, D)), X2=t((T, D)), X2h=self.X2hS[NB - 1 - n], MU2=t(T), RS2=t(T),
                FFh=self.FFhS[NB - 1 - n], S3=t((T, D)), OUT=t((T, D)), OUTh=t((T, D), BF16), MU3=t(T), RS3=t(T)))
        self.ATT, self.POOLED = t((B, Lq)), t((B, D))
        self.LOGP, self.NLL, self.LOSS = t((B, self.A)), t(B), t(1)
        self.ROWTOT = t(1, zero=True)
        mx = max(T, V)
        self.dY = [t((T, D)), t((T, D))]
        self.dA32 = t((T, D))
        self._gbufs = {}
        self.dC32 = t((T, D))
        self.dTA = [t((T, D)), t((T, D))]
        self.dA1A, self.dO1A = t((NB, T, D), BF16), t((NB, T, D), BF16)
        self.dQKV1A = t((T, NB * 3 * D), BF16)
        self.dO16 = t((T, D), BF16)
        self.dTXT = t((T, D))
        self.dVIS32, self.dVIS16 = t((V, D)), t((V, D), BF16)
        self.dVIS9 = t((9, V, D), BF16)
        self.dH32 = t((T, D))
        self.dHM32 = t((T, D))
        self.dPB = t((self.h5, Lq, Lq), zero=True)
        self.dSB = t((self.nl, B, self.h5, Lq, Lq))
        self.WS_EMB = t(3 * T, torch.int32)
        lib = L.load()
        self.WS_COL2 = t(lib.vqa_colsum_workspace_floats(V, D))
        self.WS_HEAD = t(lib.vqa_head_workspace_floats(B, Lq, D, self.A))
        self.SQ_PARTS = 1024
        self.WS_SQ = t(3 * self.SQ_PARTS, torch.float64)

    def _sga_self_keep(self):
        names = [f"sga{n}.{w}" for w in ("qkv1_w", "qkv1_b", "m1_w", "m1_b") for n in range(self.NB)]
        for w in ("qkv1_w", "qkv1_b", "m1_w", "m1_b"):
            segs = [self.lay[f"sga{n}.{w}"] for n in range(self.NB)]
            assert all(b.offset == a.offset + a.numel for a, b in zip(segs, segs[1:])), w
        return tuple(self.p16[k] for k in names if k in self.p16) + tuple(self.p32[k] for k in names) + \
            tuple(self.g32[k] for k in names)

    def _sga_groups(self):
        T, D = self.B * self.L, self.D
        if not self.sga_attn_group or self.NB == 1:
            return dict(groups=1)
        return dict(groups=self.NB, gstride_qkv=3 * D, gstride_o=T * D, gstride_dout=T * D,
                    gstride_p=self.P1A[0].numel(), gdrop_site_stride=sga_site(1, 0) - sga_site(0, 0))

    FP8_T5 = ("qkv_w", "o_w", "wi", "wo")
    FP8_SGA = ("qkv1_w", "m1_w", "q2_w", "kv2_w", "m2_w", "fc1_w", "fc2_w")

    def _is_fp8(self, wname):
        return self.fp8 and wname.rsplit(".", 1)[-1] in (self.FP8_T5 + self.FP8_SGA)

    def _w8(self, wname):
        sg = self.lay[wname]
        n, k = sg.shape
        return self.W8[sg.offset:sg.offset + n * k].view(n, k), self.WSC[sg.offset:sg.offset + n]

    def _quant_weight(self, lst, wname, rows=None):
        sg = self.lay[wname]
        k = sg.shape[1]
        rows = sg.shape[0] if rows is None else rows
        self._call(lst, "vqa_quant_rows_fp8", ops.addr(self.P32, sg.offset), 0, k, rows, k, ops.addr(self.W8, sg.offset),
                   k, ops.addr(self.WSC, sg.offset), extra=(self.P32, self.W8, self.WSC))

    def _quant_act(self, lst, key, x16, rows):
        k = x16.shape[-1]
        if key not in self._xq:
            self._xq[key] = (torch.empty(rows, k, dtype=torch.uint8, device=self.dev), self._t(rows))
        x8, xs = self._xq[key]
        self._call(lst, "vqa_quant_rows_fp8", x16, 1, k, rows, k, x8, k, xs)
        return x8, xs

    def _rms_kw(self, w, y16, rstd, ws, y32=None, drop=None):
        kw = dict(norm=L.NORM_RMS, norm_w=w, norm_eps=1e-6, norm_y32=y32, norm_y16=y16, norm_rstd=rstd, workspace=ws)
        d = self._drop(drop) if drop is not None else None
        if d is not None:
            kw.update(norm_drop=d, keep=(self.RNG,))
        return kw

    def _ln_kw(self, g, b, y32, y16, mean, rstd, ws, **strides):
        return dict(norm=L.NORM_LAYER, norm_w=g, norm_b=b, norm_eps=1e-5, norm_y32=y32, norm_y16=y16, norm_mean=mean,
                    norm_rstd=rstd, workspace=ws, **strides)

    def _dxdw(self, lst, dy16, x16, wname, rows, bias_from=None, **dxkw):
        tmp = []
        self._dx(tmp, dy16, wname, rows, **dxkw)
        self._dw(tmp, dy16, x16, wname, rows, bias_from=bias_from)
        if not self.pair_bwd:
            lst.extend(tmp)
            return
        gx, gw = tmp[0], tmp[1]
        lst.append(ops.Call("vqa_gemm_pair", ctypes.byref(gx.desc), ctypes.byref(gw.desc), keep=gx.keep + gw.keep,
                            desc=(gx.desc, gw.desc)))
        lst.extend(tmp[2:])

    def _gbuf(self, name, shape):
        if name not in self._gbufs:
            self._gbufs[name] = self._t(shape, BF16)
        return self._gbufs[name]

    def _plan_forward(self):
        D = self.D
        f = self.fwd_calls
        B, Lq, T = self.B, self.L, self.T
        fuse = self.fuse_norm
        wt5, wsga = self.NORM_WS if fuse else (None, None)
        if self.p_drop > 0.0:
            self._call(f, "vqa_rng_advance", self.RNG)
        self._fsplit = [len(f)]
        if not self.pipeline:
            f += self.res_calls
        self._fvis_param = len(f)
        cin, fh = self.fc, self.fh
        g = ops.conv_geom(B, fh, fh, cin, fh, fh, 3, 3, 1, 1)
        self._gemm(f, self.F4, self.p16["scaler_w"], self.V_TOK, D, 9 * cin, lda=9 * cin, ldb=9 * cin, ga=g,
                   c32=self.VIS32, ldc32=D, c16=self.VIS16, ldc16=D, bias=self.p32["scaler_b"])
        self._linear(f, self.VIS16, "sga0.kv2_w", self.sga[0]["ly"], out16=self.sga[0]["KV2"])
        self.sga_vision_calls = [f[-1]]
        self._fsplit.append(len(f))
        kp = []
        self._call(f, "vqa_embedding_fwd", self.IDS, self.p32["t5.embed"], self.HS[0], T, D, S.T5_VOCAB,
                   self._dptr(SITE_EMBED, kp), extra=kp + [self.RNG])
        self._call(f, "vqa_t5_relbias_fwd", self.p32["t5.relbias"], self.bucket, self.PB, self.h5, Lq, Lq)
        self._t5_layer_start = []
        for i in range(self.nl):
            self._t5_layer_start.append(len(f))
            if i == 0 or not fuse:
                self._call(f, "vqa_rmsnorm_fwd", self.HS[i], self.p32[f"t5.{i}.ln0"], None, self.N0[i], self.R0[i],
                           T, D, 1e-6, None)
            self._linear(f, self.N0[i], f"t5.{i}.qkv_w", T, out16=self.QKV[i], bias=False)
            q = self.QKV[i]
            self._attn(f, "vqa_attn_fwd", q=q, ldq=3 * D, k=ops.addr(q, D), ldk=3 * D, v=ops.addr(q, 2 * D),
                       ldv=3 * D, o=self.O[i], ldo=D, p=self.PT[i], bias=self.PB, key_mask=self.MASK, batch=B,
                       heads=self.h5, lq=Lq, lk=Lq, dh=self.dkv, scale=1.0, drop=t5_site(i, 0))
            self._linear(f, self.O[i], f"t5.{i}.o_w", T, out32=self.HM[i], bias=False, res32=self.HS[i],
                         drop=t5_site(i, 1),
                         norm=self._rms_kw(self.p32[f"t5.{i}.ln1"], self.N1[i], self.R1[i], wt5) if fuse else None)
            if not fuse:
                self._call(f, "vqa_rmsnorm_fwd", self.HM[i], self.p32[f"t5.{i}.ln1"], None, self.N1[i], self.R1[i],
                           T, D, 1e-6, None)
            self._linear(f, self.N1[i], f"t5.{i}.wi", T, out16=self.FF[i], bias=False, relu=True,
                         drop=t5_site(i, 2))
            nrm = None
            if fuse and i + 1 < self.nl:
                nrm = self._rms_kw(self.p32[f"t5.{i + 1}.ln0"], self.N0[i + 1], self.R0[i + 1], wt5)
            elif fuse:
                nrm = self._rms_kw(self.p32["t5.final_ln"], self.TXT16, self.RF, wt5, y32=self.TXT32, drop=SITE_FINAL)
            self._linear(f, self.FF[i], f"t5.{i}.wo", T, out32=self.HS[i + 1], bias=False, res32=self.HM[i],
                         drop=t5_site(i, 3), norm=nrm)
        if not fuse:
            kp = []
            self._call(f, "vqa_rmsnorm_fwd", self.HS[-1], self.p32["t5.final_ln"], self.TXT32, self.TXT16, self.RF, T,
                       D, 1e-6, self._dptr(SITE_FINAL, kp), extra=kp + [self.RNG])
        self._fsplit.append(len(f))
        y16 = self.VIS16
        sc = 1.0 / math.sqrt(self.sga_dh)
        NB, W3 = self.NB, 3 * D
        if self.fp8:
            x8, xs = self._quant_act(f, ("sga.qkv1", "x"), self.TXT16, T)
            w8 = self.W8[self.lay["sga0.qkv1_w"].offset:]
            self._gemm(f, x8, w8, T, NB * W3, D, lda=D, ldb=D, c16=self.QKV1A, ldc16=NB * W3,
                       bias=self.p32["sga0.qkv1_b"], fp8=True, scale_a=xs,
                       scale_b=ops.addr(self.WSC, self.lay["sga0.qkv1_w"].offset),
                       keep=self._sga_self_keep() + (self.W8, self.WSC))
        else:
            self._gemm(f, self.TXT16, self.p16["sga0.qkv1_w"], T, NB * W3, D, lda=D, ldb=D, c16=self.QKV1A,
                       ldc16=NB * W3, bias=self.p32["sga0.qkv1_b"], keep=self._sga_self_keep())
        grp = self._sga_groups()
        for n in range(0, NB, grp["groups"]):
            s, c0 = self.sga[n], n * W3
            q = self.QKV1A
            self._attn(f, "vqa_attn_fwd", q=ops.addr(q, c0), ldq=NB * W3, k=ops.addr(q, c0 + D), ldk=NB * W3,
                       v=ops.addr(q, c0 + 2 * D), ldv=NB * W3, o=s["O1"], ldo=D, p=s["P1"], batch=B,
                       heads=self.sga_heads, lq=Lq, lk=Lq, dh=self.sga_dh, scale=sc, drop=sga_site(n, 0),
                       keep=(q, self.O1A, self.P1A), **grp)
        m1kw = dict(c32=self.S1A, ldc32=D, bias=self.p32["sga0.m1_b"], res32=self.TXT32, ldres=D, batch=NB,
                    stride_a=T * D, stride_b=D * D, stride_c32=T * D, stride_res=0, stride_bias=D,
                    drop_site_stride=sga_site(1, 1) - sga_site(0, 1))
        fuse1 = fuse
        if fuse and NB > 1:
            gs = [self.lay[f"sga{n}.ln1_g"].offset for n in range(NB)]
            bs = [self.lay[f"sga{n}.ln1_b"].offset for n in range(NB)]
            gst = gs[1] - gs[0]
            fuse1 = all(b_ - a_ == gst for a_, b_ in zip(gs, gs[1:])) and \
                all(b_ - a_ == gst for a_, b_ in zip(bs, bs[1:])) and gst % 4 == 0
            if not fuse1:
                self.fuse_norm_kept.append("sga ln1: gamma / beta of the blocks are not at one constant stride")
        if fuse1:
            gst = (self.lay["sga1.ln1_g"].offset - self.lay["sga0.ln1_g"].offset) if NB > 1 else 0
            m1kw.update(self._ln_kw(self.p32["sga0.ln1_g"], self.p32["sga0.ln1_b"], self.X1S[NB - 1], self.X1hS[NB - 1],
                                    self.MU1S, self.RS1S, wsga, stride_norm_w=gst, stride_norm_y=-T * D,
                                    stride_norm_stat=T))
            m1keep = (self.P32, self.X1S, self.X1hS)
        else:
            m1keep = ()
        if self.fp8:
            x8, xs = self._quant_act(f, ("sga.m1", "x"), self.O1A.view(NB * T, D), NB * T)
            o0 = self.lay["sga0.m1_w"].offset
            self._gemm(f, x8, self.W8[o0:], T, D, D, lda=D, ldb=D, fp8=True, scale_a=xs, stride_scale_a=T,
                       scale_b=ops.addr(self.WSC, o0), stride_scale_b=D * D,
                       keep=self._sga_self_keep() + (self.W8, self.WSC) + m1keep, **m1kw)
        else:
            self._gemm(f, self.O1A, self.p16["sga0.m1_w"], T, D, D, lda=D, ldb=D,
                       keep=self._sga_self_keep() + m1keep, **m1kw)
        self._set_drop(f[-1], sga_site(0, 1))
        for n in range(NB if not fuse1 else 0):
            s, p = self.sga[n], f"sga{n}."
            self._call(f, "vqa_layernorm_fwd", s["S1"], self.p32[p + "ln1_g"], self.p32[p + "ln1_b"], s["X1"],
                       s["X1h"], s["MU1"], s["RS1"], T, D, 1e-5)
        segs = [self.lay[f"sga{n}.q2_w"] for n in reversed(range(NB))]
        bsegs = [self.lay[f"sga{n}.q2_b"] for n in reversed(range(NB))]
        wst = segs[1].offset - segs[0].offset if NB > 1 else 0
        assert all(b_.offset - a_.offset == wst for a_, b_ in zip(segs, segs[1:]))
        assert all(b_.offset - a_.offset == wst for a_, b_ in zip(bsegs, bsegs[1:]))
        q2kw = dict(c16=self.Q2S, ldc16=D, bias=self.p32[f"sga{NB - 1}.q2_b"], batch=NB, stride_a=T * D,
                    stride_b=wst, stride_c16=T * D, stride_bias=wst)
        if self.fp8:
            x8, xs = self._quant_act(f, ("sga.q2", "x"), self.X1hS.view(NB * T, D), NB * T)
            o0 = self.lay[f"sga{NB - 1}.q2_w"].offset
            self._gemm(f, x8, self.W8[o0:], T, D, D, lda=D, ldb=D, fp8=True, scale_a=xs, stride_scale_a=T,
                       scale_b=ops.addr(self.WSC, o0), stride_scale_b=wst, keep=(self.P16, self.P32, self.W8, self.WSC),
                       **q2kw)
        else:
            self._gemm(f, self.X1hS, self.p16[f"sga{NB - 1}.q2_w"], T, D, D, lda=D, ldb=D, keep=(self.P16, self.P32),
                       **q2kw)
        for n in range(NB):
            s, p = self.sga[n], f"sga{n}."
            if n > 0:
                self._linear(f, y16, p + "kv2_w", s["ly"], out16=s["KV2"])
            kv = s["KV2"]
            self._attn(f, "vqa_attn_fwd", q=s["Q2"], ldq=D, k=kv, ldk=2 * D, v=ops.addr(kv, D), ldv=2 * D,
                       o=s["O2"], ldo=D, p=s["P2"], batch=B, heads=self.sga_heads, lq=Lq, lk=s["lk"], dh=self.sga_dh,
                       scale=sc, drop=sga_site(n, 2))
            self._linear(f, s["O2"], p + "m2_w", T, out32=s["S2"], res32=s["X1"], drop=sga_site(n, 3),
                         norm=self._ln_kw(self.p32[p + "ln2_g"], self.p32[p + "ln2_b"], s["X2"], s["X2h"], s["MU2"],
                                          s["RS2"], wsga) if fuse else None)
            if not fuse:
                self._call(f, "vqa_layernorm_fwd", s["S2"], self.p32[p + "ln2_g"], self.p32[p + "ln2_b"], s["X2"],
                           s["X2h"], s["MU2"], s["RS2"], T, D, 1e-5)
            self._linear(f, s["X2h"], p + "fc1_w", T, out16=s["FFh"], relu=True, drop=sga_site(n, 4))
            self._linear(f, s["FFh"], p + "fc2_w", T, out32=s["S3"], res32=s["X2"], drop=sga_site(n, 5),
                         norm=self._ln_kw(self.p32[p + "ln3_g"], self.p32[p + "ln3_b"], s["OUT"], s["OUTh"], s["MU3"],
                                          s["RS3"], wsga) if fuse else None)
            if not fuse:
                self._call(f, "vqa_layernorm_fwd", s["S3"], self.p32[p + "ln3_g"], self.p32[p + "ln3_b"], s["OUT"],
                           s["OUTh"], s["MU3"], s["RS3"], T, D, 1e-5)
            y16 = s["OUTh"]
        last = self.sga[-1]["OUT"]
        self._call(f, "vqa_head_fwd", last, self.p32["pool_w"], self.p32["pool_b"], self.p32["cls_w"],
                   self.p32["cls_b"], self.TGT, self.ATT, self.POOLED, self.LOGP, self.NLL, self.LOSS, B, Lq, D, self.A)

    def _plan_backward(self):
        D = self.D
        b = self.bwd_calls
        B, Lq, T, NB = self.B, self.L, self.T, self.NB
        nparts = L.load().vqa_norm_bwd_parts(T)
        z = self.g32["t5.embed"]
        self._call(self.zero_calls, "vqa_embedding_zero_rows", self.IDS_PREV, self.IDS, T, z, D, S.T5_VOCAB)
        b += self.zero_calls
        last = self.sga[-1]["OUT"]
        self._call(b, "vqa_head_bwd", last, self.ATT, self.POOLED, self.LOGP, self.TGT, self.p32["pool_w"],
                   self.p32["cls_w"], self.dY[(NB - 1) & 1], None, self.g32["pool_w"], self.g32["pool_b"],
                   self.g32["cls_w"], self.g32["cls_b"], self.WS_HEAD, B, Lq, D, self.A, self.NLL, self.LOSS,
                   None, 1.0)
        self.ready_marks = []
        self._sq_split = None

        def mark(seg):
            self._flush(b)
            sg = self.lay[seg]
            self.ready_marks.append((len(b), sg.offset + (sg.numel + 63) // 64 * 64))
        mark("pool_b")
        sc = 1.0 / math.sqrt(self.sga_dh)
        ks = self.drop_scale if self.p_drop > 0.0 else 1.0
        self.dA3S, self.dBS, self.dA2S, self.dQS = (self._t((NB, T, D), BF16) for _ in range(4))
        batched = self.sga_dw_batch
        dxdw = (lambda lst, dy, x, w, rows, **kw: self._dx(lst, dy, w, rows, **kw)) if batched else self._dxdw
        for n in reversed(range(NB)):
            s, p = self.sga[n], f"sga{n}."
            dy = self.dY[n & 1]
            y16 = self.VIS16 if n == 0 else self.sga[n - 1]["OUTh"]
            g = lambda nm, shape: self._gbuf(f"{p}{nm}", shape)
            slot = NB - 1 - n
            dA3, dA2, dB, dQ = self.dA3S[slot], self.dA2S[slot], self.dBS[slot], self.dQS[slot]
            dKV = g("dKV", (s["ly"], 2 * D))
            kp = []
            ws = self._norm_ws()
            self._call(b, "vqa_layernorm_bwd", dy, s["S3"], s["MU3"], s["RS3"], self.p32[p + "ln3_g"], None,
                       self.dA32, dA3, None, None, ws, T, D,
                       self._dptr(sga_site(n, 5), kp), self.g32[p + "fc2_b"], extra=kp + [self.RNG])
            for j, nm in enumerate(("ln3_g", "ln3_b", "fc2_b")):
                self._defer(ws, nparts, 3 * D, D, self.g32[p + nm], offset=j * D)
            dxdw(b, dA3, s["FFh"], p + "fc2_w", T, out16=dB, mask16=s["FFh"], alpha=ks)
            if batched:
                self._dx(b, dB, p + "fc1_w", T, out32=self.dC32, res32=self.dA32)
                self._bias_colsum(b, dB, T, p + "fc1_b")
            else:
                self._dxdw(b, dB, s["X2h"], p + "fc1_w", T, bias_from=dB, out32=self.dC32, res32=self.dA32)
            kp = []
            ws = self._norm_ws()
            self._call(b, "vqa_layernorm_bwd", self.dC32, s["S2"], s["MU2"], s["RS2"], self.p32[p + "ln2_g"], None,
                       self.dA32, dA2, None, None, ws, T, D,
                       self._dptr(sga_site(n, 3), kp), self.g32[p + "m2_b"], extra=kp + [self.RNG])
            for j, nm in enumerate(("ln2_g", "ln2_b", "m2_b")):
                self._defer(ws, nparts, 3 * D, D, self.g32[p + nm], offset=j * D)
            dxdw(b, dA2, s["O2"], p + "m2_w", T, out16=self.dO16)
            kv = s["KV2"]
            self._attn(b, "vqa_attn_bwd", q=s["Q2"], ldq=D, k=kv, ldk=2 * D, v=ops.addr(kv, D), ldv=2 * D,
                       p=s["P2"], batch=B, heads=self.sga_heads, lq=Lq, lk=s["lk"], dh=self.sga_dh, scale=sc,
                       dout=self.dO16, lddo=D, dq=dQ, lddq=D, dk=dKV, lddk=2 * D,
                       dv=ops.addr(dKV, D), lddv=2 * D, drop=sga_site(n, 2))
            if batched:
                self._dx(b, dQ, p + "q2_w", T, out32=self.dC32, res32=self.dA32)
                self._bias_colsum(b, dQ, T, p + "q2_b")
            else:
                self._dxdw(b, dQ, s["X1h"], p + "q2_w", T, bias_from=dQ, out32=self.dC32, res32=self.dA32)
            if n == 0:
                self._dxdw(b, dKV, y16, p + "kv2_w", s["ly"], bias_from=dKV, out32=self.dVIS32, out16=self.dVIS16)
            else:
                self._dxdw(b, dKV, y16, p + "kv2_w", s["ly"], bias_from=dKV, out32=self.dY[(n - 1) & 1])
            kp = []
            ws = self._norm_ws()
            self._call(b, "vqa_layernorm_bwd", self.dC32, s["S1"], s["MU1"], s["RS1"], self.p32[p + "ln1_g"],
                       None if n == NB - 1 else self.dTA[(n + 1) & 1], self.dTA[n & 1], self.dA1A[n], None, None,
                       ws, T, D, self._dptr(sga_site(n, 1), kp), self.g32[p + "m1_b"], extra=kp + [self.RNG])
            for j, nm in enumerate(("ln1_g", "ln1_b", "m1_b")):
                self._defer(ws, nparts, 3 * D, D, self.g32[p + nm], offset=j * D)
            if not batched:
                mark(f"sga{n}.ln3_b")
        if batched:
            for w, dys, xs in (("fc2_w", self.dA3S, self.FFhS), ("fc1_w", self.dBS, self.X2hS),
                               ("m2_w", self.dA2S, self.O2S), ("q2_w", self.dQS, self.X1hS)):
                segs = [self.lay[f"sga{n}.{w}"] for n in reversed(range(NB))]
                lstride = segs[1].offset - segs[0].offset if NB > 1 else 0
                assert all(b_.offset - a_.offset == lstride for a_, b_ in zip(segs, segs[1:])), w
                self._gemm(b, dys, xs, D, D, T, lda=D, ldb=D, a_trans=True, b_trans=True,
                           c32=self.g32[f"sga{NB - 1}.{w}"], ldc32=D, batch=NB, stride_a=T * D, stride_b=T * D,
                           stride_c32=lstride, keep=(self.G32,))
                b[-1].side = True
        W3 = 3 * D
        keep = self._sga_self_keep()
        self._gemm(b, self.dA1A, self.p16["sga0.m1_w"], T, D, D, lda=D, ldb=D, b_trans=True, c16=self.dO1A,
                   ldc16=D, batch=NB, stride_a=T * D, stride_b=D * D, stride_c16=T * D, keep=keep)
        self._gemm(b, self.dA1A, self.O1A, D, D, T, lda=D, ldb=D, a_trans=True, b_trans=True,
                   c32=self.g32["sga0.m1_w"], ldc32=D, batch=NB, stride_a=T * D, stride_b=T * D,
                   stride_c32=D * D, keep=keep)
        b[-1].side = True
        dq = self.dQKV1A
        grp = self._sga_groups()
        for n in reversed(range(0, NB, grp["groups"])):
            s, c0 = self.sga[n], n * W3
            q = self.QKV1A
            self._attn(b, "vqa_attn_bwd", q=ops.addr(q, c0), ldq=NB * W3, k=ops.addr(q, c0 + D), ldk=NB * W3,
                       v=ops.addr(q, c0 + 2 * D), ldv=NB * W3, p=s["P1"], batch=B, heads=self.sga_heads, lq=Lq, lk=Lq,
                       dh=self.sga_dh, scale=sc, dout=self.dO1A[n], lddo=D, dq=ops.addr(dq, c0), lddq=NB * W3,
                       dk=ops.addr(dq, c0 + D), lddk=NB * W3, dv=ops.addr(dq, c0 + 2 * D), lddv=NB * W3,
                       drop=sga_site(n, 0), keep=(q, dq, self.P1A, self.dO1A), **grp)
        tmp = []
        self._gemm(tmp, dq, self.p16["sga0.qkv1_w"], T, D, NB * W3, lda=NB * W3, ldb=D, b_trans=True,
                   c32=self.dTXT, ldc32=D, res32=self.dTA[0], ldres=D, keep=keep)
        self._gemm(tmp, dq, self.TXT16, NB * W3, D, T, lda=NB * W3, ldb=D, a_trans=True, b_trans=True,
                   c32=self.g32["sga0.qkv1_w"], ldc32=D, keep=keep)
        tmp[1].side = True
        b.extend(tmp)
        lib = L.load()
        ws = self._t(lib.vqa_colsum_workspace_floats(T, NB * W3))
        self._call(b, "vqa_colsum", dq, 1, T, NB * W3, NB * W3, None, 0.0, ws)
        self._defer(ws, lib.vqa_colsum_parts(T), NB * W3, NB * W3, self.g32["sga0.qkv1_b"])
        self._jobs[-1] = self._jobs[-1][:-1] + (self._jobs[-1][-1] + keep,)
        mark(f"sga{NB - 1}.m1_b")
        self._bsplit = [len(b)]
        cin, fh = self.fc, self.fh
        self._call(b, "vqa_tap_shift", self.dVIS16, self.dVIS9, B, fh, fh, D, 3, 3, 1)
        self._gemm(b, self.dVIS9, self.F4, D, cin, self.V_TOK, lda=D, ldb=cin, a_trans=True, b_trans=True,
                   c32=self.g32["scaler_w"], ldc32=9 * cin, batch=9, stride_a=self.V_TOK * D, stride_b=0,
                   stride_c32=cin, keep=(self.G32,))
        self.scaler_dw_call = b[-1]
        self._call(b, "vqa_colsum", self.dVIS32, 0, self.V_TOK, D, D, self.g32["scaler_b"], 0.0, self.WS_COL2)
        mark("scaler_b")
        self._bsplit.append(len(b))
        nl = self.nl
        self.dH16S, self.dHMS = self._t((nl, T, D), BF16), self._t((nl, T, D), BF16)
        self.dFS, self.dQKVS = self._t((nl, T, self.dff), BF16), self._t((nl, T, 3 * D), BF16)
        dH16 = [self.dH16S[nl - 1 - i] for i in range(nl)]
        G = self.t5_dw_group
        kp = []
        ws = self._norm_ws()
        self._call(b, "vqa_rmsnorm_bwd", self.dTXT, self.HS[-1], self.RF, self.p32["t5.final_ln"], None, self.dH32,
                   dH16[-1], None, 0.0, ws, T, D,
                   self._dptr(SITE_FINAL, kp), None, self._dptr(t5_site(self.nl - 1, 3), kp),
                   extra=kp + [self.RNG])
        self._defer(ws, nparts, D, D, self.g32["t5.final_ln"])
        mark("t5.final_ln")
        dxdw = self._dxdw if (G == 1 and not self.t5_dw_groups) else \
            (lambda lst, dy, x, w, rows, **kw: self._dx(lst, dy, w, rows, **kw))
        for i in reversed(range(nl)):
            dF, dHM, dQKV = self.dFS[nl - 1 - i], self.dHMS[nl - 1 - i], self.dQKVS[nl - 1 - i]
            dxdw(b, dH16[i], self.FF[i], f"t5.{i}.wo", T, out16=dF, mask16=self.FF[i], alpha=ks)
            dxdw(b, dF, self.N1[i], f"t5.{i}.wi", T, out32=self.dC32)
            kp = []
            ws = self._norm_ws()
            self._call(b, "vqa_rmsnorm_bwd", self.dC32, self.HM[i], self.R1[i], self.p32[f"t5.{i}.ln1"], self.dH32,
                       self.dHM32, dHM, None, 0.0, ws, T, D,
                       None, None, self._dptr(t5_site(i, 1), kp), extra=kp + [self.RNG])
            self._defer(ws, nparts, D, D, self.g32[f"t5.{i}.ln1"])
            dxdw(b, dHM, self.O[i], f"t5.{i}.o_w", T, out16=self.dO16)
            q = self.QKV[i]
            dq = dQKV
            self._attn(b, "vqa_attn_bwd", q=q, ldq=3 * D, k=ops.addr(q, D), ldk=3 * D, v=ops.addr(q, 2 * D),
                       ldv=3 * D, p=self.PT[i], bias=self.PB, key_mask=self.MASK, batch=B, heads=self.h5, lq=Lq,
                       lk=Lq, dh=self.dkv, scale=1.0, dout=self.dO16, lddo=D, dq=dq, lddq=3 * D,
                       dk=ops.addr(dq, D), lddk=3 * D, dv=ops.addr(dq, 2 * D), lddv=3 * D, dbias=self.dSB[i],
                       drop=t5_site(i, 0))
            dxdw(b, dq, self.N0[i], f"t5.{i}.qkv_w", T, out32=self.dC32)
            kp = []
            d32 = self._dptr(SITE_EMBED, kp) if i == 0 else None
            d16 = self._dptr(t5_site(i - 1, 3), kp) if i > 0 else None
            ws = self._norm_ws()
            self._call(b, "vqa_rmsnorm_bwd", self.dC32, self.HS[i], self.R0[i], self.p32[f"t5.{i}.ln0"], self.dHM32,
                       self.dH32, dH16[i - 1] if i > 0 else None, None, 0.0, ws, T, D,
                       None, d32, d16, extra=kp + [self.RNG])
            self._defer(ws, nparts, D, D, self.g32[f"t5.{i}.ln0"])
            done = nl - i
            ends = (np.cumsum(self.t5_dw_groups) if self.t5_dw_groups else None)
            if G == 1 and ends is None:
                mark(f"t5.{i}.ln1")
            elif ends is not None and done in ends:
                k = int(np.searchsorted(ends, done))
                self._t5_group_dw(b, i + self.t5_dw_groups[k] - 1, i)
                mark(f"t5.{i}.ln1")
                if self._sq_split is None and i > 0:
                    self._sq_split = self.ready_marks[-1]
            elif ends is None and (done % G == 0 or i == 0):
                self._t5_group_dw(b, i + (done - 1) % G, i)
                mark(f"t5.{i}.ln1")
                if self._sq_split is None and i > 0:
                    self._sq_split = self.ready_marks[-1]
        self._call(b, "vqa_batch_sum", self.dSB, self.nl * B, self.h5 * Lq * Lq, self.dPB, 0.0)
        self._call(b, "vqa_t5_relbias_bwd", self.dPB, self.bucket, self.g32["t5.relbias"], self.h5, Lq, Lq,
                   S.T5_BUCKETS)
        mark("t5.relbias")
        self._flush(b)
        self._call(b, "vqa_embedding_bwd", self.IDS, self.dH32, self.g32["t5.embed"], T, D, S.T5_VOCAB, self.WS_EMB)
        self.emb_call = b[-1]

    def _t5_group_dw(self, lst, i_hi, i_lo):
        nl, T = self.nl, self.T
        cnt, s0 = i_hi - i_lo + 1, nl - 1 - i_hi
        for w, dys, xs in (("wo", self.dH16S, self.FFS), ("wi", self.dFS, self.N1S), ("o_w", self.dHMS, self.OS),
                           ("qkv_w", self.dQKVS, self.N0S)):
            nout, kin = self.g32[f"t5.{i_hi}.{w}"].shape
            segs = [self.lay[f"t5.{i}.{w}"] for i in range(i_hi, i_lo - 1, -1)]
            lstride = segs[1].offset - segs[0].offset if cnt > 1 else 0
            assert all(b.offset - a.offset == lstride for a, b in zip(segs, segs[1:])), w
            self._gemm(lst, ops.addr(dys, s0 * T * nout), ops.addr(xs, s0 * T * kin), nout, kin, T, lda=nout,
                       ldb=kin, a_trans=True, b_trans=True, c32=self.g32[f"t5.{i_hi}.{w}"], ldc32=kin, batch=cnt,
                       stride_a=T * nout, stride_b=T * kin, stride_c32=lstride, keep=(dys, xs, self.G32))
            lst[-1].side = True

    def _plan_optimizer(self):
        o = self.opt_calls
        n = self.lay.total
        e0 = self.lay["t5.relbias"].offset
        a = self._sq_split[1] if self._sq_split is not None else e0
        assert a % 4 == 0 and e0 % 4 == 0 and (n - e0) % 4 == 0 and a <= e0
        K = self.SQ_PARTS
        self._call(o, "vqa_grad_sqnorm", self.G32, a, self.WS_SQ, K)
        self._call(o, "vqa_grad_sqnorm", ops.addr(self.G32, a), e0 - a, ops.addr(self.WS_SQ, K), K,
                   extra=[self.G32, self.WS_SQ])
        self._call(o, "vqa_grad_sqnorm", ops.addr(self.G32, e0), n - e0, ops.addr(self.WS_SQ, 2 * K), K,
                   extra=[self.G32, self.WS_SQ])
        self._call(o, "vqa_optim_finalize", self.WS_SQ, 3 * K, float(self.grad_scale), float(self.max_norm),
                   int(self.warmup), int(self.total), float(self.betas[0]), float(self.betas[1]), self.opt_state)
        self._adam_desc = self._adam_desc_full()
        self.adam_full = self._adam_call(self._adam_desc)
        lay = self.lay
        cuts = [("embed", lay["t5.relbias"].offset, n)]
        for i in range(self.nl):
            lo = lay[f"t5.{i}.qkv_w"].offset if i < self.nl - 1 else lay["t5.final_ln"].offset
            hi = lay[f"t5.{i - 1}.qkv_w"].offset if i > 0 else lay["t5.relbias"].offset
            cuts.append((f"t5.{i}", lo, hi))
        cuts.append(("scaler", lay["scaler_w"].offset, lay["t5.final_ln"].offset))
        cuts.append(("head", 0, lay["scaler_w"].offset))
        assert sum(hi - lo for _, lo, hi in cuts) == n
        self.adam_cuts = {name: (lo, hi) for name, lo, hi in cuts}
        quant = {name: [] for name, _, _ in cuts}
        self.quant_all = []
        if self.fp8:
            jobs = [(f"t5.{i}.{w}", None) for i in range(self.nl) for w in self.FP8_T5]
            jobs.append(("sga0.qkv1_w", self.NB * 3 * self.D))
            jobs += [(f"sga{n}.{w}", None) for n in range(self.NB) for w in self.FP8_SGA if w != "qkv1_w"]
            for wname, rows in jobs:
                off = self.lay[wname].offset
                nm = next(name for name, lo, hi in cuts if lo <= off < hi)
                self._quant_weight(quant[nm], wname, rows)
                self.quant_all += quant[nm][-1:]
        self.adam_segs = []
        self.adam_embed = None
        for name, lo, hi in cuts:
            c = self.adam_range_call(lo, hi)
            if quant[name]:
                c = _Seq([c] + quant[name])
            if name == "embed":
                self.adam_embed = c
            else:
                self.adam_segs.append((name, c))
        lst = []
        self._call(lst, "vqa_zero", ops.addr(self.opt_state, L.ST_PENDING), 16, extra=[self.opt_state])
        self.clear_pending = lst[0]
        if not self.defer_opt:
            o.append(self.adam_full)
            o += self.quant_all
        elif self.adam_embed is not None:
            o.append(self.adam_embed)
        self.embed_split = self.defer_opt
        self.tail_calls = o[2:]
        self.emb_pre = []
        if self.embed_split:
            emb = lay["t5.embed"]
            assert emb.offset + emb.numel == n and self.adam_embed is o[-1]
            if self.EMB_MARK is None:
                self.EMB_MARK = torch.full((S.T5_VOCAB,), -1, dtype=torch.int32, device=self.dev)
            lo = emb.offset
            self._emb_desc = dt = self._adam_range_desc(lo, n)
            keep = self._adam_keep() + (self.EMB_MARK,)
            rows_call = lambda touched: ops.Call("vqa_adamw_rows", ctypes.byref(dt), self.EMB_MARK.data_ptr(),
                                                 S.T5_VOCAB, self.D, touched, int(self.warmup), int(self.total),
                                                 desc=dt, keep=keep)
            self.emb_pre = [ops.Call("vqa_embed_mark", self.IDS.data_ptr(), self.T, S.T5_VOCAB,
                                     self.EMB_MARK.data_ptr(), self.opt_state.data_ptr(),
                                     keep=(self.IDS, self.EMB_MARK, self.opt_state)),
                            rows_call(256)]
            self.tail_calls = o[2:-1] + [self.adam_range_call(lay["t5.relbias"].offset, lo), rows_call(1)]

    def _adam_groups(self):
        ends, lrs = self.lay.group_of_element()
        return ends, [self.group_lr.get(g, lr) for g, lr in zip(self.lay.groups, lrs)]

    def flush_optimizer(self):
        if self.defer_opt:
            self._run([c for _, c in self.adam_segs] + [self.clear_pending])

    def set_grad_scale(self, s):
        self.grad_scale = float(s)
        self.opt_calls = []
        self._plan_optimizer()
        self.graph = None

    def load_batch(self, batch, next_images=None):
        ae = self.allow_empty_rows
        n = batch_rows(batch, "question_input_ids", self.B, ae)
        if self.pipeline:
            if self._img_rows_next is not None and self._img_rows_next != n:
                raise ValueError(f"pipelined engine: this batch has {n} question rows but its images "
                                 f"(loaded one step earlier) had {self._img_rows_next}")
            if next_images is not None:
                ni = batch_rows({"image_tensors": next_images}, "image_tensors", self.B, ae)
                load_rows(self.IMG, next_images, ni)
                self._img_rows_next = ni
            else:
                self._img_rows_next = None
        else:
            load_rows(self.IMG, batch["image_tensors"], n)
        self.rows = n
        load_rows(self.IDS, batch["question_input_ids"], n)
        load_rows(self.MASK, batch["question_attention_masks"], n, empty_fill=1)
        load_rows(self.TGT, batch.get("annotation_ids"), n, fill=IGNORE_INDEX)

    def prime(self, images):
        assert self.pipeline, "prime() is for pipelined engines"
        ni = batch_rows({"image_tensors": images}, "image_tensors", self.B, self.allow_empty_rows)
        load_rows(self.IMG, images, ni)
        self._img_rows_next = ni
        self._run(self.res_calls)

    def use_global_rows(self, world):
        i = next(k for k, c in enumerate(self.bwd_calls) if c.name == "vqa_head_bwd")
        old = self.bwd_calls[i]
        if self.count_call is not None:
            assert old.args[-1] == float(world), "use_global_rows: already set for another world size"
            return
        new = ops.Call("vqa_head_bwd", *old.args[:-2], ops.addr(self.ROWTOT), float(world),
                       keep=tuple(old.keep) + (self.ROWTOT,))
        new.side = old.side
        self.bwd_calls[i] = new
        self.count_call = ops.Call("vqa_count_targets", ops.addr(self.TGT), self.B, ops.addr(self.ROWTOT),
                                   keep=(self.TGT, self.ROWTOT))
        self.allow_empty_rows = True
        self.graph = None

    def forward(self):
        self.flush_optimizer()
        super().forward()

    def _run_step_streams(self, optimizer=True):
        self.run_forward_streams()
        if optimizer:
            self.run_backward_streams(sq_overlap=True)
            self._run(self.tail_calls)
        else:
            self.run_backward_streams()

    def run_forward_streams(self):
        main = torch.cuda.current_stream(self.dev)
        side = self._side
        f = self.fwd_calls
        p0, p1, p2 = self._fsplit
        self._run(f[:p0])
        _after(side, main)
        vis, txt = f[p0:p1], f[p1:p2]
        if self.defer_opt:
            self._forward_branches_deferred(main, side, vis, txt)
        else:
            self._forward_branches(main, side, vis, txt)
        self._run(f[p2:])

    def _forward_branches(self, main, side, vis, txt):
        hm, hs = L.stream_handle(main), L.stream_handle(side)
        j = 0
        for i, c in enumerate(vis):
            c(hm)
            upto = (i + 1) * len(txt) // len(vis)
            while j < upto:
                txt[j](hs)
                j += 1
        for c in txt[j:]:
            c(hs)
        _after(main, side)

    def _t5_waits(self, i):
        w = [f"t5.{i}"]
        if self.fuse_norm and i + 1 < self.nl:
            w.append(f"t5.{i + 1}")
        return w

    def _forward_branches_deferred(self, main, side, vis, txt):
        hm, hs = L.stream_handle(main), L.stream_handle(side)
        ost = main
        hs_o = L.stream_handle(ost)
        segs = dict(self.adam_segs)
        order = [n for n, _ in self.adam_segs]
        ev = {}

        def issue(name):
            segs[name](hs_o)
            ev[name] = torch.cuda.Event()
            ev[name].record(ost)
        p0, p1 = self._fsplit[0], self._fsplit[1]
        starts = [at - p1 for at in self._t5_layer_start]
        nl = len(starts)
        ahead = 2
        for i in range(min(ahead, nl)):
            issue(f"t5.{i}")
        issue("scaler")
        issue("head")
        vpre = vis[:self._fvis_param - p0]
        vpost = vis[self._fvis_param - p0:]
        bounds = starts + [len(txt)]
        j = 0
        feed = self._res_feed
        nres = len(feed[0]) if feed else 0
        head = min(nres, self.res_head)

        def res_upto(n):
            while feed and feed[0] and nres - len(feed[0]) < n:
                feed[0].pop(0)(feed[1])
        res_upto(head)
        for t in range(bounds[0]):
            txt[t](hs)
        for i in range(nl):
            if i + ahead < nl:
                issue(f"t5.{i + ahead}")
            for name in self._t5_waits(i):
                side.wait_event(ev[name])
            for t in range(bounds[i], bounds[i + 1]):
                txt[t](hs)
            res_upto(head + (i + 1) * (nres - head) // nl)
            while j < (i + 1) * len(vpre) // nl:
                vpre[j](hm)
                j += 1
            if j == len(vpre) and vpost:
                main.wait_event(ev["scaler"])
                main.wait_event(ev["head"])
                for c in vpost:
                    c(hm)
                vpost = []
        _after(main, side)
        main.wait_event(ev[f"t5.{nl - 1}"])
        self.clear_pending(hm)
        assert set(ev) == set(order)

    def run_backward_streams(self, sq_overlap=False):
        main = torch.cuda.current_stream(self.dev)
        side, wside = self._side, self._wside
        b = self.bwd_calls
        q0, q1 = self._bsplit
        self._run_tagged(b[:q0], main, wside)
        _after(side, main)
        with torch.cuda.stream(side):
            self._run(b[q0:q1])
            if sq_overlap:
                self._run(self.emb_pre)
        if sq_overlap:
            assert b[-1] is self.emb_call

            def to_side(calls):
                for st in ((main, wside) if self.dw_stream else (main,)):
                    _after(side, st)
                with torch.cuda.stream(side):
                    self._run(calls)
            m1 = self._sq_split[0] if self._sq_split is not None else None
            if m1 is not None and q1 < m1 < len(b) - 1:
                self._run_tagged(b[q1:m1], main, wside)
                to_side(self.opt_calls[:1])
                self._run_tagged(b[m1:-1], main, wside)
                to_side(self.opt_calls[1:2])
            else:
                self._run_tagged(b[q1:-1], main, wside)
                to_side(self.opt_calls[:2])
            self._run(b[-1:])
        else:
            self._run_tagged(b[q1:], main, wside)
        for st in (side, wside):
            _after(main, st)

    def _run_tagged(self, calls, main, wside):
        if not self.dw_stream:
            self._run(calls)
            return
        i, n = 0, len(calls)
        while i < n:
            j = i
            while j < n and calls[j].side == calls[i].side:
                j += 1
            if calls[i].side:
                _after(wside, main)
                with torch.cuda.stream(wside):
                    self._run(calls[i:j])
            else:
                self._run(calls[i:j])
            i = j

    def set_res_cumask(self, words):
        hip = L.hip_runtime()
        s = ctypes.c_void_p()
        arr = (ctypes.c_uint32 * len(words))(*words)
        with torch.cuda.device(self.dev):
            rc = hip.hipExtStreamCreateWithCUMask(ctypes.byref(s), ctypes.c_uint32(len(words)), arr)
        if rc != 0:
            raise RuntimeError(f"hipExtStreamCreateWithCUMask failed ({rc})")
        self.reset_res_cumask()
        self._rstream_plain = self._rstream
        self._rstream_handle = s
        self._rstream = torch.cuda.ExternalStream(s.value, device=self.dev)
        self.res_external = True

    def reset_res_cumask(self, destroy=True):
        h = self._rstream_handle
        if h is None:
            return None
        torch.cuda.synchronize(self.dev)
        masked = self._rstream
        self._rstream = self._rstream_plain
        self._rstream_handle = None
        if self.res_external:
            self.res_external = False
            self.graph = None
        if destroy:
            rc = L.hip_runtime().hipStreamDestroy(h)
            if rc != 0:
                raise RuntimeError(f"hipStreamDestroy failed ({rc})")
            return None
        return masked, h

    def _res_external_step(self):
        main = torch.cuda.current_stream(self.dev)
        self.copy_f4(L.stream_handle(main))
        _after(self._rstream, main)
        for g in self.graph:
            g.replay()
        with torch.cuda.stream(self._rstream):
            self._run(self.res_calls)
        _after(main, self._rstream)

    def _step_pipelined(self):
        main = torch.cuda.current_stream(self.dev)
        if self.res_external:
            self.run_forward_streams()
            self.run_backward_streams(sq_overlap=True)
            self._run(self.tail_calls)
            return
        if not (torch.cuda.is_current_stream_capturing() and self.res_order == "root"):
            self.copy_f4(L.stream_handle(main))
        _after(self._rstream, main)

        last = self.res_order == "last"
        inter = self.res_order == "interleave"
        if inter:
            self._res_feed = [list(self.res_calls), L.stream_handle(self._rstream)]
        elif not last:
            with torch.cuda.stream(self._rstream):
                self._run(self.res_calls)
        self.run_forward_streams()
        if inter:
            assert not self._res_feed[0], "every ResNet call issued"
            self._res_feed = None
        self.run_backward_streams(sq_overlap=True)
        self._run(self.tail_calls)
        if last:
            with torch.cuda.stream(self._rstream):
                self._run(self.res_calls)
        _after(main, self._rstream)

    def train_step(self):
        if self.graph is not None and self.res_external:
            self._res_external_step()
            return
        if self.graph is not None and self.pipeline and self.res_order == "root":
            self.copy_f4(L.stream_handle(torch.cuda.current_stream(self.dev)))
        if self.graph is not None:
            for g in self.graph:
                if callable(g):
                    g()
                else:
                    g.replay()
            return
        if self.pipeline:
            assert self.allreduce is None, "pipelined DP steps go through dp.DataParallelStep"
            self._step_pipelined()
            return
        self.forward()
        self.backward()
        if self.allreduce is not None:
            self.allreduce(self.G32)
        self.optimizer_step()

    def capture(self, warm=True, keep_graph=False):
        self._keep_graph = bool(keep_graph)
        self.flush_optimizer()
        s = torch.cuda.Stream(self.dev)
        s.wait_stream(torch.cuda.current_stream(self.dev))
        saved, saved_rng = self.opt_state.clone(), self.RNG.clone()
        with torch.cuda.stream(s):
            if warm:
                self._run(self.fwd_calls)
                self.backward()
        torch.cuda.current_stream(self.dev).wait_stream(s)
        torch.cuda.synchronize(self.dev)
        with no_gc_capture():
            parts = self._capture_parts(s)
        self.opt_state.copy_(saved)
        self.RNG.copy_(saved_rng)
        for g in parts:
            if self._keep_graph and not callable(g):
                g.instantiate()
        self.graph = parts

    def _new_graph(self):
        return torch.cuda.CUDAGraph(keep_graph=self._keep_graph)

    def _capture_parts(self, s):
        if self.allreduce is None:
            g = self._new_graph()
            with torch.cuda.graph(g, stream=s):
                if self.pipeline:
                    self._step_pipelined()
                else:
                    self._run_step_streams()
            parts = [g]
        else:
            g1, g2 = self._new_graph(), self._new_graph()
            with torch.cuda.graph(g1, stream=s):
                self.forward()
                self.backward()
            with torch.cuda.graph(g2, stream=s):
                self.optimizer_step()
            ar = self.allreduce
            parts = [g1, lambda: ar(self.G32), g2]
        return parts

    EVAL_CAPACITY = 1 << 16

    def eval_plan(self, topk=5, similarity=None, capacity=None):
        if self.pipeline:
            raise ValueError("pipelined engines take their images a step early; evaluation has no next batch: "
                             "build the engine with pipeline=False to evaluate")
        if not 1 <= int(topk) <= L.EVAL_MAX_K:
            raise ValueError(f"topk={topk}: vqa_eval_rows supports 1..{L.EVAL_MAX_K}")
        capacity = self.EVAL_CAPACITY if capacity is None else int(capacity)
        if capacity < 0:
            raise ValueError(f"capacity={capacity} must be >= 0")
        from .metrics import check_similarity
        sim = check_similarity(similarity, self.A)
        k = int(topk)
        with torch.cuda.device(self.dev):
            self.TOPK_IDX, self.TOPK_LOGP = self._t((self.B, k), torch.int32, zero=True), self._t((self.B, k), zero=True)
            self.EVAL_BUF = self._t(16 + 2 * capacity, torch.int32, zero=True)
            self.EVAL_SIM = None if sim is None else torch.from_numpy(sim).to(self.dev)
        d = L.EvalDesc()
        d.logp, d.targets, d.nll, d.loss = (ops.addr(t) for t in (self.LOGP, self.TGT, self.NLL, self.LOSS))
        d.similarity = ops.addr(self.EVAL_SIM)
        d.batch, d.answers, d.k = self.B, self.A, k
        d.topk_idx, d.topk_logp = ops.addr(self.TOPK_IDX), ops.addr(self.TOPK_LOGP)
        d.acc = ops.addr(self.EVAL_BUF)
        d.pred_log, d.tgt_log = ops.addr(self.EVAL_BUF, 16), ops.addr(self.EVAL_BUF, 16 + capacity)
        d.capacity = capacity
        keep = (self.LOGP, self.TGT, self.NLL, self.LOSS, self.TOPK_IDX, self.TOPK_LOGP, self.EVAL_BUF) + \
            (() if self.EVAL_SIM is None else (self.EVAL_SIM,))
        self.eval_call = ops.Call("vqa_eval_rows", ctypes.byref(d), keep=keep, desc=d)
        self.eval_k, self.eval_capacity = k, capacity
        self.eval_graph = None

    def eval_prepare(self, topk=5, similarity=None, capacity=None, graph=True):
        from .metrics import check_similarity
        sim = check_similarity(similarity, self.A)
        if capacity is None:
            capacity = self.eval_capacity if self.eval_call is not None else self.EVAL_CAPACITY
        cap = int(capacity)
        same = (self.eval_call is not None and self.eval_k == int(topk) and self.eval_capacity == cap
                and (sim is None) == (self.EVAL_SIM is None))
        if not same:
            self.eval_plan(topk, sim, cap)
        elif sim is not None:
            _h2d(self.EVAL_SIM, sim)
        if graph and self.eval_graph is None:
            self.eval_capture_graph()

    def _run_eval_streams(self):
        main = torch.cuda.current_stream(self.dev)
        side = self._side
        f = self.fwd_calls
        p0, p1, p2 = self._fsplit
        _after(side, main)
        self._forward_branches(main, side, f[p0:p1], f[p1:p2])
        self._run(f[p2:])
        self.eval_call(L.stream_handle(main))

    def eval_capture(self, topk=5, similarity=None, capacity=None):
        self.eval_plan(topk, similarity, capacity)
        self.eval_capture_graph()

    def eval_capture_graph(self):
        self.flush_optimizer()
        s = torch.cuda.Stream(self.dev)
        s.wait_stream(torch.cuda.current_stream(self.dev))
        saved = (self.opt_state.clone(), self.RNG.clone(), self.EVAL_BUF.clone())
        with torch.cuda.stream(s):
            self._run_eval_streams()
        torch.cuda.current_stream(self.dev).wait_stream(s)
        torch.cuda.synchronize(self.dev)
        g = self._new_graph()
        with no_gc_capture():
            with torch.cuda.graph(g, stream=s):
                self._run_eval_streams()
        for dst, src in zip((self.opt_state, self.RNG, self.EVAL_BUF), saved):
            dst.copy_(src)
        if self._keep_graph:
            g.instantiate()
        self.eval_graph = g

    def eval_step(self, use_graph=True):
        if self.eval_call is None or (use_graph and self.eval_graph is None):
            raise RuntimeError("eval_step: call eval_capture() (or eval_plan() for use_graph=False) first")
        self.flush_optimizer()
        flag = self.RNG[2:3]
        was = flag.clone()
        flag.zero_()
        if use_graph:
            self.eval_graph.replay()
        else:
            self._run_eval_streams()
        flag.copy_(was)

    def eval_reset(self):
        self.EVAL_BUF[:16].zero_()

    def eval_result(self):
        h = self.EVAL_BUF.cpu().numpy()
        out = {n: int(v) for n, v in zip(L.EVAL_ACC_INTS, h[:10].view(np.int64))}
        out.update({n: float(v) for n, v in zip(L.EVAL_ACC_F64, h[10:16].view(np.float64))})
        n, cap = min(out["cursor"], self.eval_capacity), self.eval_capacity
        out["predictions"] = h[16:16 + n].tolist()
        out["targets"] = h[16 + cap:16 + cap + n].tolist()
        return out

    def _model_specs(self):
        return S.model_specs(self.vision, self.A, self.NB, self.dims)

    def _tune_calls(self):
        return (self.res_calls if self.pipeline else []) + super()._tune_calls()

    def log_probs(self):
        return self.LOGP[:self.rows]

    def loss(self):
        return self.LOSS

    def segment_grad(self, name):
        return self.g32[name]

    def refresh_shadow(self):
        super().refresh_shadow()
        self._run(self.quant_all)

    def layer4_features(self):
        return self.F4[:self.rows].permute(0, 3, 1, 2).float()
```

t5-resnet-vqa_amd/engine_base.py:

```python
from __future__ import annotations

import contextlib
import ctypes
import gc

import numpy as np
import torch

from . import lib as L
from . import ops
from . import tune

BF16, F32, I64 = torch.bfloat16, torch.float32, torch.int64

SITE_EMBED, SITE_FINAL = 1, 2


def t5_site(layer, kind):
    return 16 + 4 * layer + kind


class _Seq:
    def __init__(self, calls):
        self.calls = calls

    def __call__(self, stream):
        for c in self.calls:
            c(stream)


@contextlib.contextmanager
def no_gc_capture():
    was = gc.isenabled()
    gc.collect()
    gc.disable()
    try:
        yield
    finally:
        if was:
            gc.enable()


def _after(stream, other):
    if stream is other:
        return
    ev = torch.cuda.Event()
    ev.record(other)
    stream.wait_event(ev)


_WARNED_ATTN = set()


def _check_attn_path(d, fn):
    path = L.load().vqa_attn_path(ctypes.byref(d), int(fn == "vqa_attn_bwd"))
    if path == L.ATTN_VALU:
        key = (fn, d.lq, d.lk, d.dh, bool(d.key_mask))
        if key not in _WARNED_ATTN:
            _WARNED_ATTN.add(key)
            import warnings
            warnings.warn(f"{fn}: lq={d.lq} lk={d.lk} dh={d.dh} key_mask={bool(d.key_mask)} runs the scalar VALU "
                          "attention kernel (no MFMA kernel covers this shape)", RuntimeWarning, stacklevel=3)
    return path


def _h2d(dst, src):
    src = torch.as_tensor(src).to(dst.dtype).reshape(dst.shape)
    dst.copy_(src, non_blocking=src.is_cuda or src.is_pinned())


IGNORE_INDEX = -100


def batch_rows(batch, key, planned, allow_empty=False):
    n = int(torch.as_tensor(batch[key]).shape[0])
    if not (0 if allow_empty else 1) <= n <= planned:
        lo = 0 if allow_empty else 1
        raise ValueError(f"{key}: batch of {n} rows; this engine is planned for {lo}..{planned} rows")
    return n


def load_rows(dst, src, n, fill=None, empty_fill=0):
    if src is None:
        return
    B = dst.shape[0]
    if n == 0:
        dst.fill_(fill if fill is not None else empty_fill)
        return
    _h2d(dst[:n] if n < B else dst, src)
    if n == B:
        return
    if fill is not None:
        dst[n:].fill_(fill)
        return
    i = n
    while i < B:
        k = min(i, B - i)
        dst[i:i + k].copy_(dst[:k])
        i += k


class EngineBase:
    TIED = {}

    def __init__(self, device, dropout, seed, warmup, total, max_norm, betas, eps, weight_decay, grad_scale=1.0,
                 group_lr=None):
        L.load()
        self.dev = torch.device(device)
        self.p_drop, self.seed = float(dropout), int(seed)
        self.warmup, self.total, self.max_norm = warmup, total, max_norm
        self.betas, self.eps, self.wd = betas, eps, weight_decay
        self.grad_scale = grad_scale
        self.group_lr = dict(group_lr or {})
        self.fp8 = False
        self.graph = None
        self.eval_graph = None
        self._scratch = None
        self._jobs = []

    def _model_specs(self):
        raise NotImplementedError

    def _trainable_keys(self):
        return [k for s in self.lay.segments.values() for k in s.parts]

    def _adam_groups(self):
        raise NotImplementedError

    def _tune_calls(self):
        return self.fwd_calls + self.bwd_calls

    def _alloc_shadow_arenas(self):
        """Parameter shadows beyond the bf16 one, allocated between G32 and the AdamW moments."""

    def flush_optimizer(self):
        """Apply a deferred AdamW update now (nothing is deferred unless an engine says so)."""

    def _t(self, shape, dtype=F32, zero=False):
        f = torch.zeros if zero else torch.empty
        return f(shape, dtype=dtype, device=self.dev)

    def _alloc_arenas(self, sd):
        lay = self.lay
        self.P32 = torch.from_numpy(lay.pack(sd)).to(self.dev)
        self.P16 = self.P32.to(BF16)
        self.G32 = self._t(lay.total, zero=True)
        self._alloc_shadow_arenas()
        self.M, self.V, self.VMAX = (self._t(lay.total, zero=True) for _ in range(3))
        self.p32, self.p16, self.g32 = {}, {}, {}
        for s in lay.segments.values():
            sl = slice(s.offset, s.offset + s.numel)
            self.p32[s.name] = self.P32[sl].view(s.shape)
            self.p16[s.name] = self.P16[sl].view(s.shape)
            self.g32[s.name] = self.G32[sl].view(s.shape)
        self.opt_state = self._t(L.ST_FLOATS, zero=True)
        self.RNG = torch.from_numpy(np.array([self.seed & 0xFFFFFFFF, 0, 1, 0], np.uint32).view(np.int32)).to(self.dev)

    def _gemm(self, lst, a, b, m, n, k, keep=(), **kw):
        ts = [a, b] + [v for v in kw.values() if isinstance(v, torch.Tensor)] + list(keep)
        lst.append(ops.gemm_call(ops.gemm_desc(a, b, m, n, k, **kw), [t for t in ts if isinstance(t, torch.Tensor)]))

    def _call(self, lst, name, *args, extra=()):
        ts = tuple(a for a in args if isinstance(a, torch.Tensor)) + tuple(extra)
        lst.append(ops.Call(name, *[ops.addr(a) if isinstance(a, torch.Tensor) else a for a in args], keep=ts))

    def _attn(self, lst, fn, drop=None, keep=(), **kw):
        d = L.AttnDesc()
        for k, v in kw.items():
            setattr(d, k, ops.addr(v) if isinstance(v, torch.Tensor) else v)
        ts = tuple(v for v in kw.values() if isinstance(v, torch.Tensor)) + tuple(keep)
        dd = self._drop(drop) if drop is not None else None
        if dd is not None:
            d.drop = dd
            ts = ts + (self.RNG,)
        _check_attn_path(d, fn)
        lst.append(ops.Call(fn, ctypes.byref(d), keep=ts, desc=d))

    def _drop(self, site):
        if self.p_drop <= 0.0:
            return None
        return L.Dropout(self.p_drop, site, self.RNG.data_ptr())

    def _dptr(self, site, keep):
        d = self._drop(site)
        if d is None:
            return None
        keep.append(d)
        return ctypes.addressof(d)

    def _set_drop(self, call, site):
        d = self._drop(site) if site is not None else None
        if d is not None:
            call.desc.drop = d
            call.keep = call.keep + (self.RNG,)

    @property
    def drop_scale(self):
        p = np.float32(self.p_drop)
        return float(np.float32(1.0) / (np.float32(1.0) - p))

    def _linear(self, lst, x16, wname, m, out32=None, out16=None, bias=True, relu=False, res32=None, drop=None,
                norm=None):
        nkw = dict(norm or {})
        nkeep = tuple(nkw.pop("keep", ()))
        if self.fp8 and self._is_fp8(wname):
            x8, xs = self._quant_act(lst, (wname, "x"), x16, m)
            w8, ws = self._w8(wname)
            n, k = w8.shape
            self._gemm(lst, x8, w8, m, n, k, lda=k, ldb=k, c32=out32, ldc32=n, c16=out16, ldc16=n,
                       bias=self.p32[wname[:-1] + "b"] if bias else None, relu=relu, res32=res32, ldres=n, fp8=True,
                       scale_a=xs, scale_b=ws, keep=(self.W8, self.WSC) + nkeep, **nkw)
        else:
            w = self.p16[wname]
            n, k = w.shape
            self._gemm(lst, x16, w, m, n, k, lda=k, ldb=k, c32=out32, ldc32=n, c16=out16, ldc16=n,
                       bias=self.p32[wname[:-1] + "b"] if bias else None, relu=relu, res32=res32, ldres=n, keep=nkeep,
                       **nkw)
        self._set_drop(lst[-1], drop)

    def _dx(self, lst, dy16, wname, m, out32=None, out16=None, res32=None, mask16=None, beta=0.0, alpha=1.0):
        w = self.p16[wname]
        n, k = w.shape
        self._gemm(lst, dy16, w, m, k, n, lda=n, ldb=k, b_trans=True, c32=out32, ldc32=k, c16=out16, ldc16=k,
                   res32=res32, ldres=k, mask16=mask16, ldmask=k, beta=beta, alpha=alpha)

    def _dw(self, lst, dy16, x16, wname, rows, bias_from=None):
        g = self.g32[wname]
        n, k = g.shape
        self._gemm(lst, dy16, x16, n, k, rows, lda=n, ldb=k, a_trans=True, b_trans=True, c32=g, ldc32=k)
        lst[-1].side = True
        if bias_from is not None:
            assert bias_from.shape[-1] == n
            self._bias_colsum(lst, bias_from, rows, wname[:-1] + "b")

    def _bias_colsum(self, lst, dy16, rows, bname):
        lib = L.load()
        n = dy16.shape[-1]
        ws = self._t(lib.vqa_colsum_workspace_floats(rows, n))
        self._call(lst, "vqa_colsum", dy16, 1, rows, n, n, None, 0.0, ws)
        self._defer(ws, lib.vqa_colsum_parts(rows), n, n, self.g32[bname])

    def _defer(self, ws, parts, stride, cols, out, beta=0.0, offset=0):
        self._jobs.append((ops.addr(ws) + 4 * offset, ops.addr(out), stride, parts, cols, beta, (ws, out)))

    def _flush(self, lst):
        if not self._jobs:
            return
        arr = (L.ColsumJob * len(self._jobs))()
        blk = 0
        keep = []
        for j, (ws, out, stride, parts, cols, beta, k) in enumerate(self._jobs):
            arr[j] = L.ColsumJob(ws, out, stride, parts, cols, beta, blk)
            blk += -(-cols // 64)
            keep += list(k)
        raw = torch.frombuffer(bytearray(bytes(arr)), dtype=torch.uint8).to(self.dev)
        lst.append(ops.Call("vqa_colsum_batched", raw.data_ptr(), len(self._jobs), blk, keep=tuple(keep) + (raw,)))
        self._jobs = []

    def _norm_ws(self, rows=None):
        return self._t(L.load().vqa_norm_bwd_workspace_floats(self.T if rows is None else rows, self.D))

    def _run(self, calls):
        s = L.stream_handle()
        for c in calls:
            c(s)

    def _adam_desc_full(self):
        d = L.AdamWDesc()
        d.param, d.grad = self.P32.data_ptr(), self.G32.data_ptr()
        d.exp_avg, d.exp_avg_sq, d.max_exp_avg_sq = self.M.data_ptr(), self.V.data_ptr(), self.VMAX.data_ptr()
        d.param16 = self.P16.data_ptr()
        d.n = self.lay.total
        ends, lrs = self._adam_groups()
        d.ngroups = len(ends)
        for i, (e, lr) in enumerate(zip(ends, lrs)):
            d.group_end[i], d.group_lr[i] = e, lr
        d.beta1, d.beta2, d.eps, d.weight_decay = self.betas[0], self.betas[1], self.eps, self.wd
        d.grad_scale = self.grad_scale
        d.state = self.opt_state.data_ptr()
        return d

    def _adam_range_desc(self, lo, hi):
        d = self._adam_desc
        ds = L.AdamWDesc()
        ctypes.memmove(ctypes.addressof(ds), ctypes.addressof(d), ctypes.sizeof(d))
        ds.param, ds.grad = ops.addr(self.P32, lo), ops.addr(self.G32, lo)
        ds.exp_avg, ds.exp_avg_sq = ops.addr(self.M, lo), ops.addr(self.V, lo)
        ds.max_exp_avg_sq, ds.param16 = ops.addr(self.VMAX, lo), ops.addr(self.P16, lo)
        ds.n = hi - lo
        for i in range(d.ngroups):
            ds.group_end[i] = d.group_end[i] - lo
        return ds

    def _adam_keep(self):
        return (self.P32, self.G32, self.M, self.V, self.VMAX, self.P16, self.opt_state)

    def _adam_call(self, d):
        return ops.Call("vqa_adamw_amsgrad", ctypes.byref(d), desc=d, keep=self._adam_keep())

    def adam_range_call(self, lo, hi):
        return self._adam_call(self._adam_range_desc(lo, hi))

    def configure_optimizer(self, group_lr=None, warmup=None, total=None, max_norm=None, weight_decay=None,
                            betas=None, eps=None):
        if group_lr:
            self.group_lr.update(group_lr)
        if warmup is not None:
            self.warmup = int(warmup)
        if total is not None:
            self.total = int(total)
        if max_norm is not None:
            self.max_norm = float(max_norm)
        if weight_decay is not None:
            self.wd = float(weight_decay)
        if betas is not None:
            self.betas = tuple(betas)
        if eps is not None:
            self.eps = float(eps)
        self.opt_calls = []
        self._plan_optimizer()
        self.graph = None

    def set_training(self, mode=True):
        self.RNG[2].fill_(1 if mode else 0)

    def forward(self):
        self._run(self.fwd_calls)

    def backward(self):
        self._run(self.bwd_calls)

    def optimizer_step(self):
        self._run(self.opt_calls)

    def autotune(self, reps=5, table=None, save=None, cold=False):
        chosen = tune.autotune(self, self._tune_calls(), reps=reps, table=table, save=save, cold=cold)
        self.graph = None
        self.eval_graph = None
        return chosen

    def forward_backward(self, batch):
        self.load_batch(batch)
        self.forward()
        self.backward()
        torch.cuda.synchronize(self.dev)
        return self.LOGP[:self.rows].cpu().numpy(), float(self.LOSS.item())

    def grad_norm(self):
        return float(self.G32.double().norm()) * self.grad_scale

    def group_grad_norms(self):
        return {g: float(self.G32[a:e].double().norm()) * self.grad_scale for g, (a, e) in self.lay.groups.items()}

    def last_grad_norm(self):
        return float(self.opt_state[L.ST_GRAD_NORM].item())

    def state_dict(self):
        self.flush_optimizer()
        sd = dict(self._frozen)
        sd.update(self.lay.unpack(self.P32.cpu().numpy()))
        return {k: sd[k] for k in self._model_specs()}

    def optimizer_state(self):
        self.flush_optimizer()
        torch.cuda.synchronize(self.dev)
        unpack = lambda t: {k: v for k, v in self.lay.unpack(t.cpu().numpy()).items() if k not in self.TIED}
        return (unpack(self.M), unpack(self.V), unpack(self.VMAX), float(self.opt_state[L.ST_STEP].item()),
                self.RNG.cpu().numpy().copy())

    def load_optimizer_state(self, exp_avg, exp_avg_sq, max_exp_avg_sq, step, rng=None):
        self.flush_optimizer()
        specs = self._model_specs()
        zeros = {k: np.zeros(specs[k], np.float32) for k in self._trainable_keys()}
        for arena, st in ((self.M, exp_avg), (self.V, exp_avg_sq), (self.VMAX, max_exp_avg_sq)):
            full = dict(zeros)
            full.update({k: np.asarray(v, np.float32) for k, v in st.items() if k in full})
            arena.copy_(torch.from_numpy(self.lay.pack(full)))
        self.opt_state.zero_()
        self.opt_state[L.ST_STEP] = float(step)
        if rng is not None:
            self.RNG.copy_(torch.as_tensor(np.asarray(rng).astype(np.uint32).view(np.int32)))
        torch.cuda.synchronize(self.dev)

    def param_view(self, key):
        specs = self._model_specs()
        key = self.TIED.get(key, key)
        for sg in self.lay.segments.values():
            if key not in sg.parts:
                continue
            p32, g32 = self.p32[sg.name], self.g32[sg.name]
            if sg.kind == "convT":
                return p32, g32
            if sg.kind == "flat":
                return p32.view(specs[key]), g32.view(specs[key])
            row = 0
            for part in sg.parts:
                n = specs[part][0]
                if part == key:
                    return p32[row:row + n].view(specs[key]), g32[row:row + n].view(specs[key])
                row += n
        return None

    def refresh_shadow(self):
        self.P16.copy_(self.P32)
```

t5-resnet-vqa_amd/lib.py:

```python
from __future__ import annotations

import ctypes
import os
import re

import torch

PKG_DIR = os.path.dirname(os.path.abspath(__file__))
LIB_PATH = os.path.join(PKG_DIR, "lib", "libvqa_hip.so")
HEADER = os.path.join(os.path.dirname(PKG_DIR), "include", "vqa_hip.h")

c_void_p, c_int, c_float, c_ll = ctypes.c_void_p, ctypes.c_int, ctypes.c_float, ctypes.c_longlong


class ConvGeom(ctypes.Structure):
    _fields_ = [(n, c_int) for n in ("n", "h", "w", "c", "oh", "ow", "kh", "kw", "stride", "pad")]


class Dropout(ctypes.Structure):
    _fields_ = [("p", c_float), ("site", ctypes.c_uint), ("rng", c_void_p)]


class GemmDesc(ctypes.Structure):
    _fields_ = [
        ("a", c_void_p), ("lda", c_ll), ("a_trans", c_int),
        ("b", c_void_p), ("ldb", c_ll), ("b_trans", c_int),
        ("m", c_int), ("n", c_int), ("k", c_int),
        ("c32", c_void_p), ("ldc32", c_ll),
        ("c16", c_void_p), ("ldc16", c_ll),
        ("bias", c_void_p),
        ("res32", c_void_p), ("res16", c_void_p), ("ldres", c_ll),
        ("mask16", c_void_p), ("ldmask", c_ll),
        ("alpha", c_float), ("beta", c_float), ("relu", c_int),
        ("a_conv", c_int), ("ga", ConvGeom),
        ("b_conv", c_int), ("gb", ConvGeom),
        ("batch", c_int), ("stride_a", c_ll), ("stride_b", c_ll), ("stride_c32", c_ll),
        ("stride_c16", c_ll), ("stride_res", c_ll), ("config", c_int),
        ("drop", Dropout),
        ("splitk", c_int), ("workspace", c_void_p), ("workspace_bytes", c_ll),
        ("stride_bias", c_ll), ("drop_site_stride", c_int),
        ("fp8", c_int), ("scale_a", c_void_p), ("scale_b", c_void_p),
        ("stride_scale_a", c_ll), ("stride_scale_b", c_ll),
        ("norm", c_int), ("norm_w", c_void_p), ("norm_b", c_void_p), ("norm_eps", c_float),
        ("norm_y32", c_void_p), ("norm_y16", c_void_p), ("norm_mean", c_void_p), ("norm_rstd", c_void_p),
        ("stride_norm_w", c_ll), ("stride_norm_y", c_ll), ("stride_norm_stat", c_ll),
        ("norm_drop", Dropout),
    ]


class ImageDesc(ctypes.Structure):
    _fields_ = [("offset", c_ll), ("h", c_int), ("w", c_int)]


class ColsumJob(ctypes.Structure):
    _fields_ = [("ws", c_void_p), ("out", c_void_p), ("stride", c_ll), ("parts", c_int), ("cols", c_int),
                ("beta", c_float), ("first_block", c_int)]


class AttnDesc(ctypes.Structure):
    _fields_ = [
        ("q", c_void_p), ("ldq", c_ll), ("k", c_void_p), ("ldk", c_ll), ("v", c_void_p), ("ldv", c_ll),
        ("o", c_void_p), ("ldo", c_ll), ("p", c_void_p), ("bias", c_void_p), ("key_mask", c_void_p),
        ("batch", c_int), ("heads", c_int), ("lq", c_int), ("lk", c_int), ("dh", c_int), ("scale", c_float),
        ("dout", c_void_p), ("lddo", c_ll), ("dq", c_void_p), ("lddq", c_ll), ("dk", c_void_p), ("lddk", c_ll),
        ("dv", c_void_p), ("lddv", c_ll), ("dbias", c_void_p),
        ("drop", Dropout),
        ("groups", c_int), ("gstride_qkv", c_ll), ("gstride_o", c_ll), ("gstride_p", c_ll), ("gstride_dout", c_ll),
        ("gdrop_site_stride", c_int),
    ]


GEMM_TILES = {1: (128, 128, 3), 2: (128, 64, 4), 3: (64, 64, 4), 4: (64, 64, 2), 5: (64, 64, 3), 6: (128, 64, 2),
              7: (64, 128, 2), 8: (128, 128, 2), 9: (256, 128, 2), 10: (128, 256, 2), 11: (256, 256, 2),
              12: (256, 128, 3), 13: (64, 192, 2), 14: (128, 192, 2), 15: (64, 192, 3), 16: (128, 192, 3),
              17: (128, 64, 2), 18: (128, 128, 2), 19: (64, 64, 2), 20: (64, 128, 2),
              21: (64, 64, 2), 22: (64, 128, 2), 23: (128, 64, 2), 24: (64, 128, 2), 25: (128, 128, 3),
              26: (64, 128, 1), 27: (128, 64, 1), 28: (64, 64, 1)}
GEMM_PATCH_ONLY = (17, 18, 19, 20, 25)
GEMM_KC_B_ONLY = (13, 14, 15, 16)
GEMM_BK128 = (21, 22, 23, 24)
GEMM_K64_ONLY = (26, 27, 28)
GEMM_FP8 = (1, 2, 3, 4, 5, 6, 7, 8, 9, 10, 12, 21, 22, 23)
GEMM_WAVES = {c: ((4, 2) if c in (9, 12, 25) else (2, 4) if c in (10, 11, 24) else (2, 2)) for c in GEMM_TILES}

GEMM_NORM = (3, 4, 5, 6, 7, 21)
NORM_LAYER, NORM_RMS = 1, 2

ATTN_MFMA, ATTN_LONG, ATTN_VALU = 0, 1, 2
MAX_GROUPS = 8
ST_STEP, ST_GRAD_NORM, ST_CLIP_COEF, ST_LR_SCALE, ST_BC1, ST_BC2_SQRT = range(6)
ST_PENDING, ST_FLOATS = 8, 16


class AdamWDesc(ctypes.Structure):
    _fields_ = [
        ("param", c_void_p), ("grad", c_void_p), ("exp_avg", c_void_p), ("exp_avg_sq", c_void_p),
        ("max_exp_avg_sq", c_void_p), ("param16", c_void_p), ("n", c_ll), ("ngroups", c_int),
        ("group_end", c_ll * MAX_GROUPS), ("group_lr", c_float * MAX_GROUPS),
        ("beta1", c_float), ("beta2", c_float), ("eps", c_float), ("weight_decay", c_float),
        ("grad_scale", c_float), ("state", c_void_p),
    ]


class EvalDesc(ctypes.Structure):
    _fields_ = [
        ("logp", c_void_p), ("targets", c_void_p), ("nll", c_void_p), ("loss", c_void_p), ("similarity", c_void_p),
        ("batch", c_int), ("answers", c_int), ("k", c_int),
        ("topk_idx", c_void_p), ("topk_logp", c_void_p), ("acc", c_void_p),
        ("pred_log", c_void_p), ("tgt_log", c_void_p), ("capacity", c_ll),
    ]


EVAL_MAX_K = 16
EVAL_ACC_INTS = ("steps", "rows", "top1", "topk", "cursor")
EVAL_ACC_F64 = ("loss_sum", "nll_sum", "sim_sum")

_lib = None


def header_symbols():
    txt = open(HEADER).read()
    return sorted(set(re.findall(r"^\s*(?:int|long long|const char\*)\s+(vqa_\w+)\s*\(", txt, re.M)))


def abi_version():
    return int(re.search(r"#define VQA_ABI_VERSION (\d+)", open(HEADER).read()).group(1))


def load():
    global _lib
    if _lib is not None:
        return _lib
    if not os.path.exists(LIB_PATH):
        raise RuntimeError(f"libvqa_hip.so not built at {LIB_PATH}: run `python __graft_entry__.py` "
                           "(make -C t5-resnet-vqa_amd/csrc)")
    lib = ctypes.CDLL(LIB_PATH)
    missing = [s for s in header_symbols() if not hasattr(lib, s)]
    if missing:
        raise RuntimeError(f"libvqa_hip.so lacks exported symbols {missing}")
    lib.vqa_last_error.restype = ctypes.c_char_p
    if lib.vqa_abi_version() != abi_version():
        raise RuntimeError(f"libvqa_hip.so ABI {lib.vqa_abi_version()} != header ABI {abi_version()}: rebuild it")
    lib.vqa_gemm.argtypes = [ctypes.POINTER(GemmDesc), c_void_p]
    lib.vqa_gemm_select.argtypes = [ctypes.POINTER(GemmDesc)]
    lib.vqa_gemm_workspace_bytes.argtypes = [ctypes.POINTER(GemmDesc)]
    lib.vqa_gemm_workspace_bytes.restype = c_ll
    lib.vqa_gemm_pair.argtypes = [ctypes.POINTER(GemmDesc), ctypes.POINTER(GemmDesc), c_void_p]
    lib.vqa_attn_fwd.argtypes = [ctypes.POINTER(AttnDesc), c_void_p]
    lib.vqa_attn_bwd.argtypes = [ctypes.POINTER(AttnDesc), c_void_p]
    lib.vqa_attn_path.argtypes = [ctypes.POINTER(AttnDesc), c_int]
    lib.vqa_attn_probs.argtypes = [ctypes.POINTER(AttnDesc), c_void_p]
    lib.vqa_adamw_amsgrad.argtypes = [ctypes.POINTER(AdamWDesc), c_void_p]
    lib.vqa_eval_rows.argtypes = [ctypes.POINTER(EvalDesc), c_void_p]
    lib.vqa_adamw_rows.argtypes = [ctypes.POINTER(AdamWDesc), c_void_p, c_int, c_int, c_int, c_int, c_int, c_void_p]
    for name in ("vqa_norm_bwd_workspace_floats", "vqa_colsum_workspace_floats"):
        getattr(lib, name).argtypes = [c_int, c_int]
    lib.vqa_head_workspace_floats.argtypes = [c_int] * 4
    lib.vqa_norm_bwd_parts.argtypes = [c_int]
    lib.vqa_colsum_parts.argtypes = [c_int]
    for name, argtypes in _SIGS.items():
        fn = getattr(lib, name)
        fn.argtypes = argtypes
        fn.restype = c_int
    _lib = lib
    return lib


_SIGS: dict = {}


def register(name, *argtypes):
    _SIGS[name] = list(argtypes) + [c_void_p]


P = c_void_p
register("vqa_rmsnorm_fwd", P, P, P, P, P, c_int, c_int, c_float, P)
register("vqa_rmsnorm_bwd", P, P, P, P, P, P, P, P, c_float, P, c_int, c_int, P, P, P)
register("vqa_layernorm_fwd", P, P, P, P, P, P, P, c_int, c_int, c_float)
register("vqa_layernorm_bwd", P, P, P, P, P, P, P, P, P, P, P, c_int, c_int, P, P)
register("vqa_rng_advance", P)
register("vqa_dropout_mask", P, P, c_ll)
register("vqa_colsum_partials", P, c_int, c_ll, c_int, P, c_float)
register("vqa_image_to_nhwc8", P, P, c_int, c_int, c_int)
register("vqa_image_to_s2d16", P, P, c_int, c_int, c_int)
register("vqa_resize_linear_u8", P, P, c_int, c_int, c_int, P)
register("vqa_maxpool3x3s2_nhwc", P, P, c_int, c_int, c_int, c_int, c_int, c_int)
register("vqa_subsample_nhwc", P, c_int, c_int, c_int, c_int, c_int, P, c_ll)
register("vqa_stem_s2d_conv", P, P, P, P, c_int, c_int, c_int)
register("vqa_stem_pool_s2d", P, P, P, P, c_int, c_int, c_int)
register("vqa_stem_pool_img", P, P, P, P, c_int, c_int)
register("vqa_colsum", P, c_int, c_int, c_int, c_ll, P, c_float, P)
register("vqa_embedding_fwd", P, P, P, c_int, c_int, c_int, P)
register("vqa_embedding_bwd", P, P, P, c_int, c_int, c_int, P)
register("vqa_embedding_zero_rows", P, P, c_int, P, c_int, c_int)
register("vqa_colsum_batched", P, c_int, c_int)
register("vqa_t5_relbias_fwd", P, P, P, c_int, c_int, c_int)
register("vqa_t5_relbias_bwd", P, P, P, c_int, c_int, c_int, c_int)
register("vqa_batch_sum", P, c_int, c_ll, P, c_float)
register("vqa_cast_f32_bf16", P, P, c_ll)
register("vqa_zero", P, c_ll)
register("vqa_copy", P, P, c_ll)
register("vqa_tap_shift", P, P, c_int, c_int, c_int, c_int, c_int, c_int, c_int)
register("vqa_quant_rows_fp8", P, c_int, c_ll, c_int, c_int, P, c_ll, P)
register("vqa_head_fwd", P, P, P, P, P, P, P, P, P, P, P, c_int, c_int, c_int, c_int)
register("vqa_head_bwd", P, P, P, P, P, P, P, P, P, P, P, P, P, P, c_int, c_int, c_int, c_int, P, P, P, c_float)
register("vqa_count_targets", P, c_int, P)
register("vqa_embed_mark", P, c_int, c_int, P, P)
register("vqa_grad_sqnorm", P, c_ll, P, c_int)
register("vqa_vit_patchify", P, P, c_int, c_int, c_int, c_int)
register("vqa_gather_rows", P, c_ll, P, c_ll, c_ll, P, c_ll, c_int, c_int, c_int)
register("vqa_scatter_rows", P, c_ll, P, c_ll, c_ll, P, c_ll, c_int, c_int, c_int)
register("vqa_last_index", P, c_int, c_int, P)
register("vqa_xattn1_fwd", P, c_ll, P, c_ll, c_int, c_int, c_int, c_int, P)
register("vqa_xattn1_bwd", P, c_ll, P, P, c_ll, c_int, c_int, c_int, c_int, P)
register("vqa_optim_finalize", P, c_int, c_float, c_float, c_int, c_int, c_float, c_float, P)


def check(rc, what):
    if rc != 0:
        raise RuntimeError(f"{what} failed ({rc}): {_lib.vqa_last_error().decode()}")


def ptr(t):
    return None if t is None else ctypes.c_void_p(t.data_ptr())


def hip_runtime():
    import torch
    torch.cuda.init()
    with open("/proc/self/maps") as f:
        paths = {ln.split()[-1] for ln in f if "libamdhip64.so" in ln}
    if not paths:
        raise RuntimeError("libamdhip64.so is not mapped in this process")
    return ctypes.CDLL(sorted(paths)[0])


def stream_handle(stream=None):
    s = stream if stream is not None else torch.cuda.current_stream()
    return ctypes.c_void_p(s.cuda_stream)


def call(name, *args, stream=None):
    lib = load()
    rc = getattr(lib, name)(*args, stream_handle(stream))
    check(rc, name)
```

Before: 9775 pairs/s.

## Fuse grad sqnorm with optimizer finalize, split embedding sort, batch input copies

```diff
diff --git a/include/vqa_hip.h b/include/vqa_hip.h
--- a/include/vqa_hip.h
+++ b/include/vqa_hip.h
@@ -7,7 +7,7 @@
 extern "C" {
 #endif
 
-#define VQA_ABI_VERSION 20
+#define VQA_ABI_VERSION 21
 #define VQA_OK 0
 #define VQA_ERR_INVALID 1000
 
@@ -149,6 +149,9 @@
                          hipStream_t stream);
 int vqa_embedding_bwd(const long long* ids, const float* dh, float* dtable, int tokens, int d, int vocab, int* ws,
                       hipStream_t stream);
+int vqa_embedding_sort(const long long* ids, int tokens, int vocab, int* ws, hipStream_t stream);
+int vqa_embedding_bwd_sorted(const float* dh, float* dtable, int tokens, int d, int vocab, const int* ws,
+                             hipStream_t stream);
 int vqa_embedding_zero_rows(long long* ids_prev, const long long* ids_cur, int tokens, float* dtable, int d,
                             int vocab, hipStream_t stream);
 int vqa_t5_relbias_fwd(const float* table, const int* bucket, float* out, int heads, int lq, int lk,
@@ -159,6 +162,11 @@
 int vqa_cast_f32_bf16(const float* x, void* y, long long n, hipStream_t stream);
 int vqa_zero(void* p, long long bytes, hipStream_t stream);
 int vqa_copy(void* dst, const void* src, long long bytes, hipStream_t stream);
+#define VQA_COPY_MAX_JOBS 8
+typedef struct vqa_copy_job {
+  void* dst; const void* src; long long bytes;
+} vqa_copy_job;
+int vqa_copy_multi(const vqa_copy_job* jobs, int njobs, hipStream_t stream);
 int vqa_tap_shift(const void* in, void* out, int n, int h, int w, int c, int kh, int kw, int pad,
                   hipStream_t stream);
 
@@ -223,6 +231,11 @@
 int vqa_grad_sqnorm(const float* g, long long n, double* ws, int parts, hipStream_t stream);
 int vqa_optim_finalize(const double* ws, int parts, float grad_scale, float max_norm, int warmup, int total,
                        float beta1, float beta2, float* state, hipStream_t stream);
+#define VQA_SQNORM_FINAL_COUNTER_WORDS 2112
+int vqa_grad_sqnorm_final(const float* g0, long long n0, const float* g1, long long n1, double* ws, int parts,
+                          int fin_parts, const int* mark, long long lead, int cols, unsigned* counter,
+                          float grad_scale, float max_norm, int warmup, int total, float beta1, float beta2,
+                          float* state, hipStream_t stream);
 int vqa_adamw_amsgrad(const vqa_adamw_desc* d, hipStream_t stream);
 int vqa_embed_mark(const long long* ids, int n, int rows, int* mark, const float* state, hipStream_t stream);
 int vqa_adamw_rows(const vqa_adamw_desc* d, const int* mark, int rows, int cols, int touched, int warmup, int total,
diff --git a/t5-resnet-vqa_amd/csrc/elementwise.hip b/t5-resnet-vqa_amd/csrc/elementwise.hip
--- a/t5-resnet-vqa_amd/csrc/elementwise.hip
+++ b/t5-resnet-vqa_amd/csrc/elementwise.hip
@@ -327,6 +327,36 @@
   for (long i = (long)blockIdx.x * 256 + threadIdx.x; i < n16; i += (long)gridDim.x * 256) dst[i] = src[i];
 }
 
+struct CopyMultiArgs {
+  uint4* dst[VQA_COPY_MAX_JOBS];
+  const uint4* src[VQA_COPY_MAX_JOBS];
+  long n16[VQA_COPY_MAX_JOBS];
+  int first_block[VQA_COPY_MAX_JOBS + 1];
+  int njobs;
+};
+__global__ __launch_bounds__(256) void copy_multi_kernel(CopyMultiArgs A) {
+  const int b = (int)blockIdx.x;
+  long n16 = A.n16[0];
+  int b0 = 0, b1 = A.first_block[1];
+  uint4* __restrict__ dst = A.dst[0];
+  const uint4* __restrict__ src = A.src[0];
+#pragma unroll
+  for (int j = 1; j < VQA_COPY_MAX_JOBS; ++j)
+    if (j < A.njobs && A.first_block[j] <= b) {
+      n16 = A.n16[j]; b0 = A.first_block[j]; b1 = A.first_block[j + 1]; dst = A.dst[j]; src = A.src[j];
+    }
+  const long st = (long)(b1 - b0) * 256;
+  long i = (long)(b - b0) * 256 + threadIdx.x;
+  for (; i + 3 * st < n16; i += 4 * st) {
+    uint4 v[4];
+#pragma unroll
+    for (int u = 0; u < 4; ++u) v[u] = src[i + u * st];
+#pragma unroll
+    for (int u = 0; u < 4; ++u) dst[i + u * st] = v[u];
+  }
+  for (; i < n16; i += st) dst[i] = src[i];
+}
+
 }
 
 extern "C" int vqa_image_to_s2d16(const float* img, void* out, int n, int h, int w, hipStream_t s) {
@@ -430,27 +460,50 @@
   return vqa::check_launch("vqa_embedding_zero_rows");
 }
 
+namespace {
+constexpr int EMB_SLICE = 16384;
+
+int launch_embedding_sort(const long long* ids, int n, int vocab, int* ws, hipStream_t s) {
+  if (n <= 1024)
+    hipLaunchKernelGGL(embedding_sort_kernel<1>, dim3(1), dim3(1024), 0, s, ids, n, vocab, ws);
+  else if (n <= 2048)
+    hipLaunchKernelGGL(embedding_sort_kernel<2>, dim3(1), dim3(1024), 0, s, ids, n, vocab, ws);
+  else if (n <= 4096)
+    hipLaunchKernelGGL(embedding_sort_kernel<4>, dim3(1), dim3(1024), 0, s, ids, n, vocab, ws);
+  else if (n <= 8192)
+    hipLaunchKernelGGL(embedding_sort_kernel<8>, dim3(1), dim3(1024), 0, s, ids, n, vocab, ws);
+  else
+    hipLaunchKernelGGL(embedding_sort_kernel<16>, dim3(1), dim3(1024), 0, s, ids, n, vocab, ws);
+  return vqa::check_launch("vqa_embedding_bwd/sort");
+}
+
+int launch_embedding_scatter(const float* dh, float* dtable, int n, int d, const int* ws, hipStream_t s) {
+  hipLaunchKernelGGL(embedding_bwd_kernel, dim3(n, vqa::cdiv(d, 4 * EMB_CL)), dim3(EMB_RL * EMB_CL), 0, s, dh, dtable,
+                     ws, n, d);
+  return vqa::check_launch("vqa_embedding_bwd");
+}
+}
+
+extern "C" int vqa_embedding_sort(const long long* ids, int tokens, int vocab, int* ws, hipStream_t s) {
+  VQA_REQUIRE(ids && ws && tokens > 0 && tokens <= EMB_SLICE && vocab > 0,
+              "vqa_embedding_sort: bad arguments (1 <= tokens <= 16384)");
+  return launch_embedding_sort(ids, tokens, vocab, ws, s);
+}
+
+extern "C" int vqa_embedding_bwd_sorted(const float* dh, float* dtable, int tokens, int d, int vocab, const int* ws,
+                                        hipStream_t s) {
+  VQA_REQUIRE(dh && dtable && ws && tokens > 0 && tokens <= EMB_SLICE && d % 4 == 0 && vocab > 0,
+              "vqa_embedding_bwd_sorted: bad arguments (1 <= tokens <= 16384)");
+  return launch_embedding_scatter(dh, dtable, tokens, d, ws, s);
+}
+
 extern "C" int vqa_embedding_bwd(const long long* ids, const float* dh, float* dtable, int tokens, int d, int vocab,
                                  int* ws, hipStream_t s) {
   VQA_REQUIRE(ids && dh && dtable && ws && tokens > 0 && d % 4 == 0, "vqa_embedding_bwd: bad arguments");
-  constexpr int SLICE = 16384;
-  for (int t0 = 0; t0 < tokens; t0 += SLICE) {
-    const int n = tokens - t0 < SLICE ? tokens - t0 : SLICE;
-    const long long* sid = ids + t0;
-    if (n <= 1024)
-      hipLaunchKernelGGL(embedding_sort_kernel<1>, dim3(1), dim3(1024), 0, s, sid, n, vocab, ws);
-    else if (n <= 2048)
-      hipLaunchKernelGGL(embedding_sort_kernel<2>, dim3(1), dim3(1024), 0, s, sid, n, vocab, ws);
-    else if (n <= 4096)
-      hipLaunchKernelGGL(embedding_sort_kernel<4>, dim3(1), dim3(1024), 0, s, sid, n, vocab, ws);
-    else if (n <= 8192)
-      hipLaunchKernelGGL(embedding_sort_kernel<8>, dim3(1), dim3(1024), 0, s, sid, n, vocab, ws);
-    else
-      hipLaunchKernelGGL(embedding_sort_kernel<16>, dim3(1), dim3(1024), 0, s, sid, n, vocab, ws);
-    if (int rc = vqa::check_launch("vqa_embedding_bwd/sort")) return rc;
-    hipLaunchKernelGGL(embedding_bwd_kernel, dim3(n, vqa::cdiv(d, 4 * EMB_CL)), dim3(EMB_RL * EMB_CL), 0, s,
-                       dh + (long long)t0 * d, dtable, ws, n, d);
-    if (int rc = vqa::check_launch("vqa_embedding_bwd")) return rc;
+  for (int t0 = 0; t0 < tokens; t0 += EMB_SLICE) {
+    const int n = tokens - t0 < EMB_SLICE ? tokens - t0 : EMB_SLICE;
+    if (int rc = launch_embedding_sort(ids + t0, n, vocab, ws, s)) return rc;
+    if (int rc = launch_embedding_scatter(dh + (long long)t0 * d, dtable, n, d, ws, s)) return rc;
   }
   return VQA_OK;
 }
@@ -502,6 +555,30 @@
   const int grid = (int)((n16 + 255) / 256 < 8192 ? (n16 + 255) / 256 : 8192);
   hipLaunchKernelGGL(copy_kernel, dim3(grid), dim3(256), 0, s, (uint4*)dst, (const uint4*)src, n16);
   return vqa::check_launch("vqa_copy");
+}
+
+extern "C" int vqa_copy_multi(const vqa_copy_job* jobs, int njobs, hipStream_t s) {
+  VQA_REQUIRE(jobs && njobs > 0 && njobs <= VQA_COPY_MAX_JOBS, "vqa_copy_multi: 1..8 jobs");
+  CopyMultiArgs A;
+  int nb = 0, k = 0;
+  for (int j = 0; j < njobs; ++j) {
+    const vqa_copy_job& J = jobs[j];
+    VQA_REQUIRE(J.bytes >= 0 && J.bytes % 16 == 0 && ((uintptr_t)J.dst & 15) == 0 && ((uintptr_t)J.src & 15) == 0 &&
+                    (J.bytes == 0 || (J.dst && J.src)),
+                "vqa_copy_multi: pointers and sizes must be 16-byte aligned");
+    if (J.bytes == 0) continue;
+    const long n16 = (long)(J.bytes / 16);
+    const long blocks = (n16 + 255) / 256 < 4096 ? (n16 + 255) / 256 : 4096;
+    A.dst[k] = (uint4*)J.dst; A.src[k] = (const uint4*)J.src; A.n16[k] = n16; A.first_block[k] = nb;
+    nb += (int)blocks;
+    ++k;
+  }
+  if (k == 0) return VQA_OK;
+  for (int j = k; j <= VQA_COPY_MAX_JOBS; ++j) A.first_block[j] = nb;
+  for (int j = k; j < VQA_COPY_MAX_JOBS; ++j) { A.dst[j] = nullptr; A.src[j] = nullptr; A.n16[j] = 0; }
+  A.njobs = k;
+  hipLaunchKernelGGL(copy_multi_kernel, dim3(nb), dim3(256), 0, s, A);
+  return vqa::check_launch("vqa_copy_multi");
 }
 
 __global__ __launch_bounds__(256) void tap_shift_kernel(const uint4* __restrict__ in, uint4* __restrict__ out, int h,
diff --git a/t5-resnet-vqa_amd/csrc/optim.hip b/t5-resnet-vqa_amd/csrc/optim.hip
--- a/t5-resnet-vqa_amd/csrc/optim.hip
+++ b/t5-resnet-vqa_amd/csrc/optim.hip
@@ -2,29 +2,59 @@
 
 namespace {
 
-__global__ __launch_bounds__(256) void sqnorm_kernel(const float* __restrict__ g, long n4, double* __restrict__ ws) {
+__device__ __forceinline__ double sq_term(const float4 v) {
+  return (double)v.x * v.x + (double)v.y * v.y + (double)v.z * v.z + (double)v.w * v.w;
+}
+
+__device__ __forceinline__ double sq_range(const float* __restrict__ g, long n4, int bid, int nblk) {
   const float4* g4 = reinterpret_cast<const float4*>(g);
-  const long st = (long)gridDim.x * 256;
+  const long st = (long)nblk * 256;
   double s = 0.0;
-  long i = (long)blockIdx.x * 256 + threadIdx.x;
+  long i = (long)bid * 256 + threadIdx.x;
   for (; i + 3 * st < n4; i += 4 * st) {
     float4 v[4];
 #pragma unroll
     for (int u = 0; u < 4; ++u) v[u] = g4[i + u * st];
 #pragma unroll
-    for (int u = 0; u < 4; ++u)
-      s += (double)v[u].x * v[u].x + (double)v[u].y * v[u].y + (double)v[u].z * v[u].z + (double)v[u].w * v[u].w;
-  }
-  for (; i < n4; i += st) {
-    const float4 v = g4[i];
-    s += (double)v.x * v.x + (double)v.y * v.y + (double)v.z * v.z + (double)v.w * v.w;
-  }
+    for (int u = 0; u < 4; ++u) s += sq_term(v[u]);
+  }
+  for (; i < n4; i += st) s += sq_term(g4[i]);
+  return s;
+}
+
+__device__ __forceinline__ double sq_range_rows(const float* __restrict__ g, long n4, int bid, int nblk,
+                                                const int* __restrict__ mark, int step, long lead4, unsigned d4) {
+  const float4* g4 = reinterpret_cast<const float4*>(g);
+  const long st = (long)nblk * 256;
+  double s = 0.0;
+  for (long i = (long)bid * 256 + threadIdx.x; i < n4; i += 8 * st) {
+    int mk[8];
+#pragma unroll
+    for (int u = 0; u < 8; ++u) {
+      const long j = i + u * st;
+      mk[u] = j >= n4 ? step - 1 : (j < lead4 ? step : mark[(unsigned)(j - lead4) / d4]);
+    }
+    float4 v[8];
+#pragma unroll
+    for (int u = 0; u < 8; ++u) v[u] = mk[u] == step ? g4[i + u * st] : make_float4(0.f, 0.f, 0.f, 0.f);
+#pragma unroll
+    for (int u = 0; u < 8; ++u) s += sq_term(v[u]);
+  }
+  return s;
+}
+
+__device__ __forceinline__ double sq_block_sum(double s, double* red) {
 #pragma unroll
   for (int o = 32; o > 0; o >>= 1) s += __shfl_xor(s, o, 64);
-  __shared__ double red[4];
   if ((threadIdx.x & 63) == 0) red[threadIdx.x >> 6] = s;
   __syncthreads();
-  if (threadIdx.x == 0) ws[blockIdx.x] = red[0] + red[1] + red[2] + red[3];
+  return red[0] + red[1] + red[2] + red[3];
+}
+
+__global__ __launch_bounds__(256) void sqnorm_kernel(const float* __restrict__ g, long n4, double* __restrict__ ws) {
+  __shared__ double red[4];
+  const double s = sq_block_sum(sq_range(g, n4, blockIdx.x, gridDim.x), red);
+  if (threadIdx.x == 0) ws[blockIdx.x] = s;
 }
 
 __device__ __forceinline__ void schedule_at(double step, int warmup, int total, float beta1, float beta2,
@@ -38,11 +68,32 @@
   bc2s = (float)sqrt(1.0 - pow((double)beta2, t));
 }
 
-__global__ void finalize_kernel(const double* __restrict__ ws, int parts, float grad_scale, float max_norm,
-                                int warmup, int total, float beta1, float beta2, float* __restrict__ st) {
-  __shared__ double red[256];
+typedef __attribute__((address_space(1))) unsigned gu32;
+typedef __attribute__((address_space(1))) unsigned long long gu64;
+
+template <bool SC1>
+__device__ __forceinline__ void finalize_body(const double* __restrict__ ws, int parts, float grad_scale,
+                                              float max_norm, int warmup, int total, float beta1, float beta2,
+                                              float* __restrict__ st, double* red) {
   double part = 0.0;
-  for (int i = threadIdx.x; i < parts; i += 256) part += ws[i];
+  for (int i0 = threadIdx.x; i0 < parts; i0 += 16 * 256) {
+    double v[16];
+#pragma unroll
+    for (int u = 0; u < 16; ++u) {
+      const int i = i0 + u * 256;
+      v[u] = 0.0;
+      if (i < parts) {
+        if (SC1)
+          v[u] = __longlong_as_double((long long)__hip_atomic_load((gu64*)(ws + i), __ATOMIC_RELAXED,
+                                                                   __HIP_MEMORY_SCOPE_AGENT));
+        else
+          v[u] = ws[i];
+      }
+    }
+#pragma unroll
+    for (int u = 0; u < 16; ++u)
+      if (i0 + u * 256 < parts) part += v[u];
+  }
   red[threadIdx.x] = part;
   __syncthreads();
   if (threadIdx.x != 0) return;
@@ -61,6 +112,58 @@
   st[VQA_ST_BC2_SQRT] = bc2s;
   st[VQA_ST_STEP] = (float)(step + 1.0);
   st[VQA_ST_PENDING] = 1.f;
+}
+
+__global__ __launch_bounds__(256) void finalize_kernel(const double* __restrict__ ws, int parts, float grad_scale,
+                                                       float max_norm, int warmup, int total, float beta1,
+                                                       float beta2, float* __restrict__ st) {
+  __shared__ double red[256];
+  finalize_body<false>(ws, parts, grad_scale, max_norm, warmup, total, beta1, beta2, st, red);
+}
+
+constexpr int SQ_NSUB = 32, SQ_CNT_STRIDE = 64;
+static_assert((1 + SQ_NSUB) * SQ_CNT_STRIDE == VQA_SQNORM_FINAL_COUNTER_WORDS, "counter block");
+struct SqFinalArgs {
+  const float* g0; long n4_0;
+  const float* g1; long n4_1;
+  double* ws; int parts, fin;
+  const int* mark; long lead4; unsigned d4;
+  unsigned* cnt;
+  float grad_scale, max_norm; int warmup, total; float beta1, beta2;
+  float* st;
+};
+
+__global__ __launch_bounds__(256) void sqnorm_final_kernel(SqFinalArgs A) {
+  __shared__ double red[256];
+  const int K = A.parts;
+  const int b = blockIdx.x;
+  double s;
+  if (b < K) s = sq_range(A.g0, A.n4_0, b, K);
+  else if (A.mark) s = sq_range_rows(A.g1, A.n4_1, b - K, K, A.mark, (int)A.st[VQA_ST_STEP], A.lead4, A.d4);
+  else s = sq_range(A.g1, A.n4_1, b - K, K);
+  s = sq_block_sum(s, red);
+  int* flag = reinterpret_cast<int*>(red + 8);
+  if (threadIdx.x == 0) {
+    __hip_atomic_store((gu64*)(A.ws + (A.fin - 2 * K) + b), (unsigned long long)__double_as_longlong(s),
+                       __ATOMIC_RELAXED, __HIP_MEMORY_SCOPE_AGENT);
+    asm volatile("s_waitcnt vmcnt(0)" ::: "memory");
+    const int nb = 2 * K, grp = b % SQ_NSUB;
+    const unsigned members = (unsigned)((nb - grp + SQ_NSUB - 1) / SQ_NSUB);
+    const unsigned groups = (unsigned)(nb < SQ_NSUB ? nb : SQ_NSUB);
+    gu32* sub = (gu32*)(A.cnt + (1 + grp) * SQ_CNT_STRIDE);
+    int last = 0;
+    if (__hip_atomic_fetch_add(sub, 1u, __ATOMIC_RELAXED, __HIP_MEMORY_SCOPE_AGENT) == members - 1) {
+      __hip_atomic_store(sub, 0u, __ATOMIC_RELAXED, __HIP_MEMORY_SCOPE_AGENT);
+      last = __hip_atomic_fetch_add((gu32*)A.cnt, 1u, __ATOMIC_RELAXED, __HIP_MEMORY_SCOPE_AGENT) == groups - 1;
+      if (last) __hip_atomic_store((gu32*)A.cnt, 0u, __ATOMIC_RELAXED, __HIP_MEMORY_SCOPE_AGENT);
+    }
+    *flag = last;
+  }
+  __syncthreads();
+  if (!*flag) return;
+  __syncthreads();
+  __builtin_amdgcn_fence(__ATOMIC_ACQUIRE, "wavefront");
+  finalize_body<true>(A.ws, A.fin, A.grad_scale, A.max_norm, A.warmup, A.total, A.beta1, A.beta2, A.st, red);
 }
 
 __global__ __launch_bounds__(256) void embed_mark_kernel(const long long* __restrict__ ids, int n, int rows,
@@ -154,6 +257,27 @@
   return vqa::check_launch("vqa_optim_finalize");
 }
 
+extern "C" int vqa_grad_sqnorm_final(const float* g0, long long n0, const float* g1, long long n1, double* ws,
+                                     int parts, int fin_parts, const int* mark, long long lead, int cols,
+                                     unsigned* counter, float grad_scale, float max_norm, int warmup, int total,
+                                     float beta1, float beta2, float* state, hipStream_t s) {
+  VQA_REQUIRE(g0 && g1 && ws && counter && state && parts > 0 && fin_parts >= 2 * parts && n0 >= 0 && n1 >= 0 &&
+                  n0 % 4 == 0 && n1 % 4 == 0 && ((uintptr_t)g0 & 15) == 0 && ((uintptr_t)g1 & 15) == 0,
+              "vqa_grad_sqnorm_final: bad arguments (n %% 4 == 0, 16-byte aligned ranges, fin_parts >= 2 parts)");
+  VQA_REQUIRE(!mark || (cols > 0 && cols % 4 == 0 && lead >= 0 && lead % 4 == 0 && lead <= n1 &&
+                        (n1 - lead) % cols == 0 && n1 / 4 < (1ll << 31)),
+              "vqa_grad_sqnorm_final: range 1 must be `lead` floats then whole rows of `cols` (both %% 4 == 0)");
+  SqFinalArgs A;
+  A.g0 = g0; A.n4_0 = (long)(n0 / 4); A.g1 = g1; A.n4_1 = (long)(n1 / 4);
+  A.ws = ws; A.parts = parts; A.fin = fin_parts;
+  A.mark = mark; A.lead4 = (long)(lead / 4); A.d4 = mark ? (unsigned)(cols / 4) : 1u;
+  A.cnt = counter;
+  A.grad_scale = grad_scale; A.max_norm = max_norm; A.warmup = warmup; A.total = total;
+  A.beta1 = beta1; A.beta2 = beta2; A.st = state;
+  hipLaunchKernelGGL(sqnorm_final_kernel, dim3(2 * parts), dim3(256), 0, s, A);
+  return vqa::check_launch("vqa_grad_sqnorm_final");
+}
+
 extern "C" int vqa_adamw_amsgrad(const vqa_adamw_desc* d, hipStream_t s) {
   AdamArgs A;
   if (int rc = adam_args(d, A)) return rc;
diff --git a/t5-resnet-vqa_amd/dp.py b/t5-resnet-vqa_amd/dp.py
--- a/t5-resnet-vqa_amd/dp.py
+++ b/t5-resnet-vqa_amd/dp.py
@@ -361,7 +361,7 @@
                                          e.EMB_MARK.data_ptr(), e.opt_state.data_ptr(),
                                          keep=(self.GIDS, e.EMB_MARK, e.opt_state)), e.emb_pre[1]]
                 self.stages[0]["ops"].insert(0, ("emb", self.emb_pre))
-                opt = opt[:2] + list(e.tail_calls)
+                opt = opt[:2] + list(e.tail_calls_unfused)
             a = e._sq_split[1] if e._sq_split is not None else None
             if a is not None:
                 done = 0
diff --git a/t5-resnet-vqa_amd/engine.py b/t5-resnet-vqa_amd/engine.py
--- a/t5-resnet-vqa_amd/engine.py
+++ b/t5-resnet-vqa_amd/engine.py
@@ -11,7 +11,8 @@
 from . import ops
 from . import synthetic as S
 from .engine_base import (BF16, F32, I64, IGNORE_INDEX, SITE_EMBED, SITE_FINAL, EngineBase, _after,
-                          _check_attn_path, _h2d, _Seq, batch_rows, load_rows, no_gc_capture, t5_site)
+                          _check_attn_path, _h2d, _Seq, batch_rows, load_rows, load_rows_multi, no_gc_capture,
+                          t5_site)
 from .layout import ParamLayout, fold_bn, t5_bucket_map
 
 
@@ -43,6 +44,7 @@
         self._rstream_handle = None
         self._rstream_plain = None
         self.EMB_MARK = None
+        self.SQ_CNT = None
         self.vision, self.B, self.L, self.H = vision, batch, seq_len, image_size
         assert image_size % 2 == 0, "the space-to-depth stem needs an even image size"
         self.NB, self.A = num_blocks, answer_spaces
@@ -807,6 +809,28 @@
                                      keep=(self.IDS, self.EMB_MARK, self.opt_state)),
                             rows_call(256)]
             self.tail_calls = o[2:-1] + [self.adam_range_call(lay["t5.relbias"].offset, lo), rows_call(1)]
+        self.tail_calls_unfused = self.tail_calls
+        T = self.T
+        self.fused_tail = self.embed_split and T <= 16384
+        self.emb_sort_call = self.emb_scatter_call = None
+        if self.fused_tail:
+            if self.SQ_CNT is None:
+                self.SQ_CNT = torch.zeros(L.SQNORM_FINAL_COUNTER_WORDS, dtype=torch.int32,
+                                          device=self.dev)
+            emb = lay["t5.embed"]
+            lead = emb.offset - e0
+            assert lead >= 0 and lead % 4 == 0 and emb.numel == S.T5_VOCAB * self.D and self.D % 4 == 0
+            fin = ops.Call("vqa_grad_sqnorm_final", ops.addr(self.G32, a), e0 - a, ops.addr(self.G32, e0), n - e0,
+                           self.WS_SQ.data_ptr(), K, 3 * K, self.EMB_MARK.data_ptr(), lead, self.D,
+                           self.SQ_CNT.data_ptr(), float(self.grad_scale), float(self.max_norm), int(self.warmup),
+                           int(self.total), float(self.betas[0]), float(self.betas[1]), self.opt_state.data_ptr(),
+                           keep=(self.G32[a:], self.WS_SQ, self.EMB_MARK, self.SQ_CNT, self.opt_state))
+            assert [c.name for c in self.tail_calls[:2]] == ["vqa_grad_sqnorm", "vqa_optim_finalize"]
+            self.tail_calls = [fin] + self.tail_calls[2:]
+            ids, dh, dtab, _, _, _, ws = self.emb_call.args
+            self.emb_sort_call = ops.Call("vqa_embedding_sort", ids, T, S.T5_VOCAB, ws, keep=(self.IDS, self.WS_EMB))
+            self.emb_scatter_call = ops.Call("vqa_embedding_bwd_sorted", dh, dtab, T, self.D, S.T5_VOCAB, ws,
+                                             keep=(self.dH32, self.G32, self.WS_EMB))
 
     def _adam_groups(self):
         ends, lrs = self.lay.group_of_element()
@@ -825,22 +849,27 @@
     def load_batch(self, batch, next_images=None):
         ae = self.allow_empty_rows
         n = batch_rows(batch, "question_input_ids", self.B, ae)
+        items = []
         if self.pipeline:
             if self._img_rows_next is not None and self._img_rows_next != n:
                 raise ValueError(f"pipelined engine: this batch has {n} question rows but its images "
                                  f"(loaded one step earlier) had {self._img_rows_next}")
             if next_images is not None:
                 ni = batch_rows({"image_tensors": next_images}, "image_tensors", self.B, ae)
-                load_rows(self.IMG, next_images, ni)
+                if ni == n:
+                    items.append((self.IMG, next_images, {}))
+                else:
+                    load_rows(self.IMG, next_images, ni)
                 self._img_rows_next = ni
             else:
                 self._img_rows_next = None
         else:
-            load_rows(self.IMG, batch["image_tensors"], n)
+            items.append((self.IMG, batch["image_tensors"], {}))
         self.rows = n
-        load_rows(self.IDS, batch["question_input_ids"], n)
-        load_rows(self.MASK, batch["question_attention_masks"], n, empty_fill=1)
-        load_rows(self.TGT, batch.get("annotation_ids"), n, fill=IGNORE_INDEX)
+        items += [(self.IDS, batch["question_input_ids"], {}),
+                  (self.MASK, batch["question_attention_masks"], {"empty_fill": 1}),
+                  (self.TGT, batch.get("annotation_ids"), {"fill": IGNORE_INDEX})]
+        load_rows_multi(items, n)
 
     def prime(self, images):
         assert self.pipeline, "prime() is for pipelined engines"
@@ -871,10 +900,13 @@
     def _run_step_streams(self, optimizer=True):
         self.run_forward_streams()
         if optimizer:
-            self.run_backward_streams(sq_overlap=True)
-            self._run(self.tail_calls)
+            self._backward_and_tail()
         else:
             self.run_backward_streams()
+
+    def _backward_and_tail(self):
+        self.run_backward_streams(sq_overlap=True, sorted_scatter=self.fused_tail)
+        self._run(self.tail_calls)
 
     def run_forward_streams(self):
         main = torch.cuda.current_stream(self.dev)
@@ -965,7 +997,8 @@
         self.clear_pending(hm)
         assert set(ev) == set(order)
 
-    def run_backward_streams(self, sq_overlap=False):
+    def run_backward_streams(self, sq_overlap=False, sorted_scatter=False):
+        assert sq_overlap or not sorted_scatter
         main = torch.cuda.current_stream(self.dev)
         side, wside = self._side, self._wside
         b = self.bwd_calls
@@ -974,6 +1007,10 @@
         _after(side, main)
         with torch.cuda.stream(side):
             self._run(b[q0:q1])
+            if sorted_scatter:
+                self.emb_sort_call(L.stream_handle(side))
+                sorted_ev = torch.cuda.Event()
+                sorted_ev.record(side)
             if sq_overlap:
                 self._run(self.emb_pre)
         if sq_overlap:
@@ -989,11 +1026,19 @@
                 self._run_tagged(b[q1:m1], main, wside)
                 to_side(self.opt_calls[:1])
                 self._run_tagged(b[m1:-1], main, wside)
-                to_side(self.opt_calls[1:2])
+                if sorted_scatter:
+                    main.wait_event(sorted_ev)
+                    self._run([self.emb_scatter_call])
+                else:
+                    to_side(self.opt_calls[1:2])
             else:
                 self._run_tagged(b[q1:-1], main, wside)
-                to_side(self.opt_calls[:2])
-            self._run(b[-1:])
+                if sorted_scatter:
+                    main.wait_event(sorted_ev)
+                    self._run([self.emb_scatter_call])
+                to_side(self.opt_calls[:1] if sorted_scatter else self.opt_calls[:2])
+            if not sorted_scatter:
+                self._run(b[-1:])
         else:
             self._run_tagged(b[q1:], main, wside)
         for st in (side, wside):
@@ -1062,8 +1107,7 @@
         main = torch.cuda.current_stream(self.dev)
         if self.res_external:
             self.run_forward_streams()
-            self.run_backward_streams(sq_overlap=True)
-            self._run(self.tail_calls)
+            self._backward_and_tail()
             return
         if not (torch.cuda.is_current_stream_capturing() and self.res_order == "root"):
             self.copy_f4(L.stream_handle(main))
@@ -1080,8 +1124,7 @@
         if inter:
             assert not self._res_feed[0], "every ResNet call issued"
             self._res_feed = None
-        self.run_backward_streams(sq_overlap=True)
-        self._run(self.tail_calls)
+        self._backward_and_tail()
         if last:
             with torch.cuda.stream(self._rstream):
                 self._run(self.res_calls)
diff --git a/t5-resnet-vqa_amd/engine_base.py b/t5-resnet-vqa_amd/engine_base.py
--- a/t5-resnet-vqa_amd/engine_base.py
+++ b/t5-resnet-vqa_amd/engine_base.py
@@ -98,6 +98,25 @@
         k = min(i, B - i)
         dst[i:i + k].copy_(dst[:k])
         i += k
+
+
+def _plain_device_copy(dst, src):
+    return (isinstance(src, torch.Tensor) and src.is_cuda and src.device == dst.device and src.dtype == dst.dtype
+            and src.numel() == dst.numel() and src.is_contiguous() and dst.is_contiguous()
+            and src.data_ptr() % 16 == 0 and dst.data_ptr() % 16 == 0 and (dst.numel() * dst.element_size()) % 16 == 0)
+
+
+def load_rows_multi(items, n):
+    jobs = []
+    for dst, src, kw in items:
+        if src is not None and n == dst.shape[0] and len(jobs) < L.COPY_MAX_JOBS and _plain_device_copy(dst, src):
+            jobs.append((dst, src))
+        else:
+            load_rows(dst, src, n, **kw)
+    if jobs:
+        arr = (L.CopyJob * len(jobs))(*[L.CopyJob(d.data_ptr(), s.data_ptr(), d.numel() * d.element_size())
+                                         for d, s in jobs])
+        L.call("vqa_copy_multi", arr, len(jobs))
 
 
 class EngineBase:
diff --git a/t5-resnet-vqa_amd/lib.py b/t5-resnet-vqa_amd/lib.py
--- a/t5-resnet-vqa_amd/lib.py
+++ b/t5-resnet-vqa_amd/lib.py
@@ -55,6 +55,14 @@
 class ColsumJob(ctypes.Structure):
     _fields_ = [("ws", c_void_p), ("out", c_void_p), ("stride", c_ll), ("parts", c_int), ("cols", c_int),
                 ("beta", c_float), ("first_block", c_int)]
+
+
+class CopyJob(ctypes.Structure):
+    _fields_ = [("dst", c_void_p), ("src", c_void_p), ("bytes", c_ll)]
+
+
+COPY_MAX_JOBS = 8
+SQNORM_FINAL_COUNTER_WORDS = 2112
 
 
 class AttnDesc(ctypes.Structure):
@@ -192,6 +200,8 @@
 register("vqa_colsum", P, c_int, c_int, c_int, c_ll, P, c_float, P)
 register("vqa_embedding_fwd", P, P, P, c_int, c_int, c_int, P)
 register("vqa_embedding_bwd", P, P, P, c_int, c_int, c_int, P)
+register("vqa_embedding_sort", P, c_int, c_int, P)
+register("vqa_embedding_bwd_sorted", P, P, c_int, c_int, c_int, P)
 register("vqa_embedding_zero_rows", P, P, c_int, P, c_int, c_int)
 register("vqa_colsum_batched", P, c_int, c_int)
 register("vqa_t5_relbias_fwd", P, P, P, c_int, c_int, c_int)
@@ -200,6 +210,7 @@
 register("vqa_cast_f32_bf16", P, P, c_ll)
 register("vqa_zero", P, c_ll)
 register("vqa_copy", P, P, c_ll)
+register("vqa_copy_multi", P, c_int)
 register("vqa_tap_shift", P, P, c_int, c_int, c_int, c_int, c_int, c_int, c_int)
 register("vqa_quant_rows_fp8", P, c_int, c_ll, c_int, c_int, P, c_ll, P)
 register("vqa_head_fwd", P, P, P, P, P, P, P, P, P, P, P, c_int, c_int, c_int, c_int)
@@ -207,6 +218,8 @@
 register("vqa_count_targets", P, c_int, P)
 register("vqa_embed_mark", P, c_int, c_int, P, P)
 register("vqa_grad_sqnorm", P, c_ll, P, c_int)
+register("vqa_grad_sqnorm_final", P, c_ll, P, c_ll, P, c_int, c_int, P, c_ll, c_int, P, c_float, c_float, c_int, c_int,
+         c_float, c_float, P)
 register("vqa_vit_patchify", P, P, c_int, c_int, c_int, c_int)
 register("vqa_gather_rows", P, c_ll, P, c_ll, c_ll, P, c_ll, c_int, c_int, c_int)
 register("vqa_scatter_rows", P, c_ll, P, c_ll, c_ll, P, c_ll, c_int, c_int, c_int)
```

Result: faster. 9928 pairs/s, median of 6 (+1.6%).
